# HicrestLaboratory/DLNetBench

Measured on AMD Instinct MI355X. Metric: proxy iter time (ms) + effective GB/s, Llama-3-8B DP/FSDP at 1/2/4/8 MI355X, lower is better.
Workload: dtype bf16

## Files before the change

### csrc/include/dlnb/comm.hpp

```cpp
#pragma once

#include <memory>
#include <string>
#include <vector>

#include "dlnb/bootstrap.hpp"
#include "dlnb/common.hpp"
#include "dlnb/device.hpp"

namespace dlnb {

enum class CollKind : int { AllReduce, AllGather, ReduceScatter, AllToAll, SendRecv };

class Communicator {
 public:
  virtual ~Communicator() = default;
  int rank() const { return rank_; }
  int size() const { return size_; }
  const std::vector<int>& members() const { return members_; }
  const std::string& name() const { return name_; }
  virtual std::string backend_name() const = 0;

  virtual void all_reduce(const void* send, void* recv, size_t count, DType t, Stream& s) = 0;
  virtual void all_gather(const void* send, void* recv, size_t send_count, DType t, Stream& s) = 0;
  virtual void reduce_scatter(const void* send, void* recv, size_t recv_count, DType t, Stream& s) = 0;
  virtual void all_to_all(const void* send, void* recv, size_t count, DType t, Stream& s) = 0;
  virtual void send(const void* buf, size_t count, DType t, int peer, Stream& s) = 0;
  virtual void recv(void* buf, size_t count, DType t, int peer, Stream& s) = 0;
  virtual void group_start() {}
  virtual void group_end() {}
  virtual bool wants_peer_buffers() const { return false; }
  virtual void register_buffer(void* p, size_t bytes) { (void)p, (void)bytes; }
  virtual std::string async_error() { return ""; }
  virtual void abort() {}
  virtual int library_nranks() { return -1; }

 protected:
  int rank_ = 0;
  int size_ = 1;
  std::vector<int> members_;
  std::string name_;
};

class CommFactory {
 public:
  virtual ~CommFactory() = default;
  virtual std::string backend_name() const = 0;
  virtual std::unique_ptr<Communicator> create(const std::string& name, const std::vector<int>& members,
                                               size_t capacity_bytes, bool need_p2p, int max_ctas = 0) = 0;
};

std::unique_ptr<CommFactory> make_rccl_factory(HostGroup& world, Device& dev);
std::unique_ptr<CommFactory> make_shm_factory(HostGroup& world, Device& dev);
std::unique_ptr<CommFactory> make_xgmi_factory(HostGroup& world, Device& dev);
std::unique_ptr<CommFactory> make_mixed_factory(HostGroup& world, Device& dev);

struct LoopbackHub;
std::shared_ptr<LoopbackHub> make_loopback_hub(int ranks, double timeout_s);
void loopback_abort(LoopbackHub& hub, const std::string& why);
AbortFlag loopback_cpu_abort_flag(LoopbackHub& hub);
void loopback_drained(LoopbackHub& hub, bool wait, double timeout_s);
std::unique_ptr<CommFactory> make_loopback_factory(HostGroup& world, Device& dev, std::shared_ptr<LoopbackHub> hub);

std::unique_ptr<CommFactory> wrap_comm_faults(std::unique_ptr<CommFactory> inner, Device& dev, int world_rank);

void host_reduce_sum(DType t, void* dst, const std::vector<const char*>& srcs, size_t count);
void host_copy(void* dst, const void* src, size_t bytes);

double busbw_factor(CollKind k, int n);

}
```

### csrc/include/dlnb/compute.hpp

```cpp
#pragma once

#include <memory>
#include <string>
#include <vector>

#include "dlnb/device.hpp"
#include "dlnb/json.hpp"
#include "dlnb/timers.hpp"

namespace dlnb {

enum class ComputeMode { Sleep, Spin, Gemm, GemmWork, Flops };

ComputeMode parse_compute_mode(const std::string& s, DeviceKind dev);
const char* compute_mode_name(ComputeMode m);

struct ComputeShape {
  int hidden = 4096;
  int ffn = 16384;
  DType dtype = DType::BF16;
  int comm_cus = 32;
  int ranks_on_device = 1;
};

class ComputeEngine {
 public:
  virtual ~ComputeEngine() = default;
  virtual void run(Stream& s, double us, double flops) = 0;
  virtual void run_stamped(Stream& s, double us, double flops, uint64_t* start) {
    (void)start;
    run(s, us, flops);
  }
  virtual bool stamps_task_start() const { return false; }
  virtual void run_chained(Stream& s, double us, double flops, uint64_t* start = nullptr, Event* done = nullptr) {
    run_stamped(s, us, flops, start);
    if (done) s.record(*done);
  }
  virtual uint64_t task_ticks(double us) const { (void)us; return 0; }
  virtual const uint64_t* last_task_end(Stream& s) { (void)s; return nullptr; }
  virtual bool gates_task(double us) const { (void)us; return false; }
  virtual int make_gate() { DLNB_THROW("this compute mode has no device gates"); }
  virtual void signal(Stream& s, int gate) { (void)s; (void)gate; DLNB_THROW("this compute mode has no device gates"); }
  virtual void wait_gate(Stream& s, int gate, double timeout_us) {
    (void)s; (void)gate; (void)timeout_us;
    DLNB_THROW("this compute mode has no device gates");
  }
  virtual void run_gated(Stream& s, double us, double flops, const std::vector<int>& gates, uint64_t* start,
                         bool chain, Event* done = nullptr) {
    (void)s; (void)us; (void)flops; (void)gates; (void)start; (void)chain; (void)done;
    DLNB_THROW("this compute mode has no device gates");
  }
  virtual void set_next_start_slot(uint64_t* slot) { (void)slot; }
  virtual void reset_clocks(Stream& s) { (void)s; }
  virtual void reset_slot(Stream& s) { (void)s; }
  virtual bool begin_program(Stream& s) { (void)s; return false; }
  virtual void end_program(Stream& s, bool join_ok) { (void)s; (void)join_ok; }
  virtual void after_capture() {}
  virtual long programs_on(Stream& s) { (void)s; return 0; }
  virtual bool program_split(Stream& s) { (void)s; return false; }
  virtual void set_lane_join(Stream& s, const std::vector<uint64_t*>& gates, uint32_t tag, uint64_t* host_done) {
    (void)s; (void)gates; (void)tag; (void)host_done;
  }
  virtual bool program_joined(Stream& s) { (void)s; return false; }
  virtual void set_gate_timeout(double s) { (void)s; }
  virtual double lane_task_us(Stream& s) { (void)s; return -1.0; }
  struct ChainCounters {
    double capped_tasks = 0, capped_s = 0, absorbed_tasks = 0, absorbed_s = 0;
    double wait_timeouts = 0, gate_timeouts = 0, aborted = 0, late_blocks = 0;
  };
  virtual void reset_capped(Stream& s) { (void)s; }
  virtual bool chain_counters(ChainCounters& c) { (void)c; return false; }
  virtual void set_task_timers(TimerSet* t) { (void)t; }
  virtual bool product(const void** c, size_t* count, DType* t) const {
    (void)c; (void)count; (void)t;
    return false;
  }
  virtual Json describe() const = 0;
  virtual ComputeMode mode() const = 0;
};

std::unique_ptr<ComputeEngine> make_compute_engine(Device& dev, ComputeMode mode, const ComputeShape& shape,
                                                   double time_scale);

struct TaskMark {
  const uint64_t* slot = nullptr;
  uint64_t ticks = 0;
};
inline TaskMark task_mark(ComputeEngine& ce, Stream& s, const uint64_t* start, double us) {
  if (const uint64_t* e = ce.last_task_end(s)) return {e, 0};
  return {start, ce.task_ticks(us)};
}

}
```

### csrc/include/dlnb/kernels.hpp

```cpp
#pragma once

#include <cstddef>
#include <cstdint>

#include "dlnb/common.hpp"

namespace dlnb {
namespace kernels {

void fill_random(void* p, size_t count, DType t, uint64_t seed, void* stream);

enum DlCounter : int {
  kCappedTasks = 0,
  kCappedTicks = 1,
  kWaitTimeouts = 2,
  kGateTimeouts = 3,
  kAbsorbedTicks = 4,
  kAbsorbedTasks = 5,
  kAborted = 6,
  kLateBlocks = 7,
  kNumCounters = 8
};
constexpr uint64_t kPoisonIter = ~0ull;
struct DlSync {
  uint64_t* tstart[2] = {nullptr, nullptr};
  const uint64_t* gate[2] = {nullptr, nullptr};
  uint32_t tag[2] = {0, 0};
  uint32_t chain = 0;
  uint64_t* counters = nullptr;
  const uint64_t* iter = nullptr;
  uint64_t gate_timeout = 0;
  uint64_t* done_gate = nullptr;
  uint32_t done_tag = 0;
  uint32_t pad = 0;
  const uint64_t* abort = nullptr;
};
constexpr uint32_t kTaskGateOnly = 1;
struct DlTask {
  DlSync sync;
  uint64_t ticks = 0;
  uint32_t epoch = 0;
  uint32_t work_rounds = 0;
  uint32_t tail_kt = 0;
  uint32_t flags = 0;
  uint64_t* tend = nullptr;
};
void gate_signal(uint64_t* gate, const uint64_t* iter, uint32_t tag, void* stream);
void fail_gate_signal(long index);
void gate_wait(const uint64_t* gate, const uint64_t* iter, uint32_t tag, uint64_t timeout_ticks, uint64_t* timeouts,
               void* stream, const uint64_t* abort = nullptr);
void set_word(uint64_t* word, uint64_t value, void* stream);
bool queues_independent(void* a, void* b, uint64_t timeout_ticks);

void idle_wait(uint64_t ticks, void* stream, uint64_t* start = nullptr, uint64_t* start2 = nullptr);
void busy_spin(uint64_t ticks, int blocks, void* stream, uint64_t* start = nullptr, uint64_t* start2 = nullptr);
double wallclock_hz(int device);
double wallclock_hz_nominal(int device);
double wallclock_uncertainty_ppm(int device);
void clock_cal_begin(int device);
void stamp(uint64_t* slot, void* stream);
void host_signal(uint64_t* word, uint64_t value, void* stream);
void lane_done(uint64_t* word, const uint64_t* iter, void* stream);
void host_wait(const uint64_t* word, uint64_t value, uint64_t timeout_ticks, uint64_t* timeouts, void* stream,
               uint64_t* iter_out = nullptr, uint64_t iter_value = 0, const uint64_t* abort = nullptr);
int num_cus(int device);

bool gemm_shape_ok(int M, int N, int K, DType in_t);
void gemm_tn(const void* A, const void* B, void* C, int M, int N, int K, int lda, int ldb, int ldc, DType in_t,
             void* stream, int variant = 0);
bool gemm_8phase_shape_ok(int M, int N, int K, DType in_t);
bool gemm_4wave_fp8_shape_ok(int M, int N, int K, DType in_t);
int gemm_group();
int gemm_narrow_nf(int M, int N, int cus);
bool gemm_tn_narrow(const void* A, const void* B, void* C, int M, int N, int K, int lda, int ldb, int ldc,
                    DType in_t, void* stream);
void gemm_tn_4wave_fp8(const void* A, const void* B, void* C, int M, int N, int K, int lda, int ldb, int ldc,
                       void* stream);
bool gemm_4wave_shape_ok(int M, int N, int K, DType in_t);
void gemm_tn_4wave_bf16(const void* A, const void* B, void* C, int M, int N, int K, int lda, int ldb, int ldc,
                        void* stream);
void gemm_tn_4wave_deadline(const void* A, const void* B, void* C, int M, int N, int K, DType in_t, uint64_t ticks,
                            uint64_t* slot, uint32_t epoch, int grid, void* stream, uint64_t slice_end,
                            const DlSync& sync);
void gemm_tn_4wave_fp8_deadline(const void* A, const void* B, void* C, int M, int N, int K, uint64_t ticks,
                                uint64_t* slot, uint32_t epoch, int grid, void* stream, uint64_t slice_end,
                                const DlSync& sync);
void gemm_tn_8phase(const void* A, const void* B, void* C, int M, int N, int K, int lda, int ldb, int ldc, DType in_t,
                    void* stream);
void gemm_tn_8phase_deadline(const void* A, const void* B, void* C, int M, int N, int K, DType in_t, uint64_t ticks,
                             uint64_t* slot, uint32_t epoch, int grid, void* stream, uint64_t slice_end,
                             const DlSync& sync);

void gemm_tn_deadline(const void* A, const void* B, void* C, int M, int N, int K, DType in_t, uint64_t ticks,
                      uint64_t* slot, uint32_t epoch, int grid, void* stream, uint64_t slice_end = 0,
                      const DlSync& sync = DlSync());

bool deadline_program_ok(int M, int N, int K, DType in_t);
void gemm_tn_deadline_program(const void* A, const void* B, void* C, int M, int N, int K, DType in_t,
                              const DlTask* tasks, int n, uint64_t* slot, int grid, void* stream,
                              uint32_t epoch = 0);
int program_ktiles(int M, int N, int K, DType in_t);
int program_tail_multiple(int M, int N, int K, DType in_t);

void sgd_momentum_bf16(void* param, void* mom, const void* grad, size_t n, float lr, float beta, void* stream,
                       uint64_t* end_stamp = nullptr, uint32_t* done = nullptr);

}
}
```

### csrc/include/dlnb/strategy.hpp

```cpp
#pragma once

#include <memory>
#include <string>
#include <vector>

#include "dlnb/bootstrap.hpp"
#include "dlnb/comm.hpp"
#include "dlnb/compute.hpp"
#include "dlnb/device.hpp"
#include "dlnb/json.hpp"
#include "dlnb/options.hpp"
#include "dlnb/timers.hpp"
#include "dlnb/timeline.hpp"
#include "dlnb/workload.hpp"

namespace dlnb {

struct CommRecord {
  std::string name;
  std::string backend;
  int nranks;
  int library_nranks;
};

struct Context {
  Options opt;
  std::unique_ptr<Bootstrap> boot;
  std::unique_ptr<Device> dev;
  std::unique_ptr<CommFactory> comms;
  std::vector<CommRecord> comm_log;
  std::vector<Communicator*> live_comms;
  std::unique_ptr<ComputeEngine> compute;
  ModelStats stats;
  bool have_arch = false;
  ModelArch arch;
  DType wire = DType::BF16;
  int lane_ctas = 0;
  int ranks_on_device = 1;
  std::unique_ptr<Timeline> timeline;
  int rank() const { return boot->info.rank; }
  int world() const { return boot->info.world_size; }
  HostGroup& hg() { return *boot->world; }
};

struct GridCoords {
  int inner_id, stage_id, dp_id;
};
GridCoords grid_coords(int rank, int inner, int stages);
std::vector<int> inner_group(int rank, int inner, int stages);
std::vector<int> pp_group(int rank, int inner, int stages);
std::vector<int> dp_group(int rank, int inner, int stages, int world);

struct OutputView {
  std::string name;
  const void* data;
  size_t count;
  DType dtype;
};

class Strategy {
 public:
  virtual ~Strategy() = default;
  virtual void setup(Context& ctx) = 0;
  virtual void enqueue_iteration() = 0;
  virtual void synchronize() = 0;
  virtual std::vector<Stream*> streams() = 0;
  virtual bool capturable() const = 0;
  virtual bool lanes_without_program() const { return true; }
  virtual std::string section_id() const = 0;
  virtual std::string section_title() const = 0;
  virtual const char* runtime_key() const { return "runtimes"; }
  virtual Json global_json() const = 0;
  virtual Json rank_json() const = 0;
  virtual Json comm_summary() const = 0;
  virtual double compute_floor_us(const Context& ctx) const {
    return ctx.stats.avg_forward_time_us + ctx.stats.avg_backward_time_us;
  }
  virtual std::string tail_collective_timer() const { return ""; }
  virtual std::vector<OutputView> outputs() const { return {}; }
  TimerSet* timers() { return timers_.get(); }

 protected:
  std::unique_ptr<TimerSet> timers_;
};

std::unique_ptr<Strategy> make_dp();
std::unique_ptr<Strategy> make_fsdp();
std::unique_ptr<Strategy> make_pipeline(StrategyKind kind);
std::unique_ptr<Strategy> make_cp();

int collective_lanes(const Options& o, int world);

std::string select_backend(Context& ctx, const std::string& requested, const std::string& devices);

int commtest_main(int argc, char** argv);
int info_main(int argc, char** argv);

Json run_benchmark(const Options& opt);

int main_for(StrategyKind kind, int argc, char** argv);

void sync_streams(const std::vector<Stream*>& streams, const std::vector<Communicator*>& comms, Device& dev);

void device_failure(const std::string& why);
bool process_poisoned();

class CompletionFlag {
 public:
  CompletionFlag(const uint64_t* flags, size_t n, uint64_t value);
  ~CompletionFlag();
  CompletionFlag(const CompletionFlag&) = delete;
  CompletionFlag& operator=(const CompletionFlag&) = delete;

 private:
  const uint64_t* prev_;
  size_t prev_n_;
  uint64_t prev_value_;
};

struct CommStat {
  std::string name;
  CollKind kind;
  int nranks;
  double bytes_per_op;
  std::string timer;
};
Json comm_stats_json(const std::vector<CommStat>& stats, const TimerSet& t);

void dump_outputs(Context& ctx, const Strategy& strat, const std::string& dir);

void print_topology(Context& ctx);

Json runtime_info();

Json comm_log_json(const std::vector<CommRecord>& log);

void optimizer_step(Context& ctx, Stream& s, void* param, void* mom, const void* grad, size_t n,
                    uint64_t* end_stamp = nullptr, uint32_t* done = nullptr);

}
```

### csrc/include/dlnb/timers.hpp

```cpp
#pragma once

#include <map>
#include <memory>
#include <string>
#include <vector>

#include "dlnb/device.hpp"
#include "dlnb/json.hpp"

namespace dlnb {

class TimerSet {
 public:
  explicit TimerSet(Device& dev);
  ~TimerSet();
  TimerSet(const TimerSet&) = delete;
  TimerSet& operator=(const TimerSet&) = delete;
  int begin(Stream& s);
  const uint64_t* at(int token) const { return token < 0 ? nullptr : stamps_ + token; }
  const uint64_t* end(int token, Stream& s, const std::string& name);
  void stall(Stream& s, Event& e, const std::string& name);
  uint64_t* slot();
  void gap(const uint64_t* prev_start, uint64_t prev_ticks, const uint64_t* next_start, const std::string& name,
           bool clamp = false);
  void set_task_stamps(bool on) { task_stamps_ = on; }
  bool task_stamps() const { return task_stamps_ && enabled_; }
  uint64_t* task_slot(Stream& s);
  void task_started(Stream& s, const uint64_t* start, uint64_t ticks, const uint64_t* end = nullptr);
  const uint64_t* mark(Stream& s);
  void pair(const uint64_t* a, const uint64_t* b, const std::string& name);
  void stall_before_task(Stream& s, Event& e, const std::string& name);
  void stall_after_task(Stream& s, Event& e, const std::string& name);
  void settle(Stream& s, const uint64_t* op_end);
  void stall_until(Stream& s, const uint64_t* end, const std::string& name);
  void iteration_start(Stream& s);
  void finish_stalls();
  void add(const std::string& name, double seconds);
  void ensure(const std::string& name);
  void resolve();
  void clear();
  Json negatives_json() const;
  bool has_negatives() const { return !negatives_.empty(); }
  void begin_capture();
  void end_capture();
  void set_enabled(bool on) { enabled_ = on; }
  bool enabled() const { return enabled_; }
  const std::vector<double>& get(const std::string& name) const;
  double sum(const std::string& name) const;
  Json values_json(const std::string& name) const;

 private:
  Device& dev_;
  uint64_t* stamps_ = nullptr;
  size_t cap_ = 0;
  size_t next_ = 0;
  struct Pending {
    int a, b;
    std::string name;
  };
  std::vector<Pending> pending_;
  struct Gap {
    int prev, next;
    uint64_t prev_ticks;
    std::string name;
    bool clamp;
    int floor;
  };
  std::vector<Gap> gaps_;
  bool owns(const uint64_t* p) const { return p >= stamps_ && p < stamps_ + cap_; }
  struct TaskClock {
    const uint64_t* start = nullptr;
    uint64_t ticks = 0;
    const uint64_t* floor = nullptr;
    std::vector<std::string> pending;
  };
  std::map<Stream*, TaskClock> clocks_;
  Stream* origin_ = nullptr;
  const uint64_t* origin_start_ = nullptr;
  void first_reference(Stream& s, TaskClock& c);
  void close_pending(TaskClock& c, const uint64_t* at, bool clamp = false);
  static void restart(TaskClock& c, const uint64_t* start, uint64_t ticks) {
    c.start = start;
    c.ticks = ticks;
    c.floor = nullptr;
  }
  bool task_stamps_ = false;
  std::map<std::string, std::vector<double>> vals_;
  struct Negative {
    long count = 0;
    double worst_s = 0.0;
  };
  std::map<std::string, Negative> negatives_;
  std::vector<std::pair<std::string, double>> captured_adds_;
  bool capturing_ = false, frozen_ = false;
  bool enabled_ = true;
};

}
```

### csrc/kernels/kernels.hip

```cpp
#include <hip/hip_runtime.h>

#include <cstdio>
#include "dlnb/common.hpp"
#include <thread>
#include <mutex>
#include <cmath>
#include <vector>
#include <algorithm>
#include <atomic>
#include <chrono>

#include "deadline_sync.hpp"
#include "dlnb/kernels.hpp"

#define DLNB_HIP_CHECK(expr)                                                       \
  do {                                                                             \
    hipError_t e_ = (expr);                                                        \
    if (e_ != hipSuccess) DLNB_THROW(#expr << " failed: " << hipGetErrorString(e_)); \
  } while (0)

namespace dlnb {
namespace kernels {

namespace {

typedef __attribute__((ext_vector_type(8))) __bf16 bf16x8;
typedef __attribute__((ext_vector_type(4))) __bf16 bf16x4;
typedef __attribute__((ext_vector_type(4))) float f32x4;
typedef __attribute__((ext_vector_type(8))) int i32x8;
typedef __attribute__((address_space(3))) void* lds_ptr_t;
typedef __attribute__((address_space(1))) void* gbl_ptr_t;

inline hipStream_t S(void* s) { return static_cast<hipStream_t>(s); }


__device__ __forceinline__ uint64_t splitmix64(uint64_t x) {
  x += 0x9E3779B97F4A7C15ull;
  x = (x ^ (x >> 30)) * 0xBF58476D1CE4E5B9ull;
  x = (x ^ (x >> 27)) * 0x94D049BB133111EBull;
  return x ^ (x >> 31);
}

__device__ __forceinline__ float u01(uint64_t h, int part) {
  uint32_t v = static_cast<uint32_t>((h >> (21 * part)) & 0x1fffff);
  return static_cast<float>(v) * (2.0f / 2097152.0f) - 1.0f;
}

__device__ __forceinline__ uint8_t f32_to_e4m3(float f) {
  int r = __builtin_amdgcn_cvt_pk_fp8_f32(f, f, 0, false);
  return static_cast<uint8_t>(r & 0xff);
}

__device__ __forceinline__ uint8_t f32_to_e5m2(float f) {
  int r = __builtin_amdgcn_cvt_pk_bf8_f32(f, f, 0, false);
  return static_cast<uint8_t>(r & 0xff);
}

template <typename Tstore, int KIND>
__global__ void fill_kernel(Tstore* __restrict__ p, size_t n8, size_t n, uint64_t seed) {
  size_t stride = static_cast<size_t>(gridDim.x) * blockDim.x;
  for (size_t i = blockIdx.x * static_cast<size_t>(blockDim.x) + threadIdx.x; i < n8; i += stride) {
    uint64_t h0 = splitmix64(seed ^ (i * 2 + 0));
    uint64_t h1 = splitmix64(seed ^ (i * 2 + 1));
    float f[8];
#pragma unroll
    for (int j = 0; j < 3; ++j) f[j] = u01(h0, j);
#pragma unroll
    for (int j = 0; j < 3; ++j) f[3 + j] = u01(h1, j);
    f[6] = u01(h0 ^ h1, 0);
    f[7] = u01(h0 ^ h1, 1);
    size_t base = i * 8;
    if (KIND == 0) {
      bf16x8 v;
#pragma unroll
      for (int j = 0; j < 8; ++j) v[j] = static_cast<__bf16>(f[j]);
      if (base + 8 <= n) {
        *reinterpret_cast<bf16x8*>(reinterpret_cast<__bf16*>(p) + base) = v;
      } else {
        for (int j = 0; j < 8 && base + j < n; ++j) reinterpret_cast<__bf16*>(p)[base + j] = v[j];
      }
    } else if (KIND == 1) {
      for (int j = 0; j < 8 && base + j < n; ++j) reinterpret_cast<_Float16*>(p)[base + j] = static_cast<_Float16>(f[j]);
    } else if (KIND == 2) {
      for (int j = 0; j < 8 && base + j < n; ++j) reinterpret_cast<float*>(p)[base + j] = f[j];
    } else {
      uint8_t b[8];
#pragma unroll
      for (int j = 0; j < 8; ++j) b[j] = KIND == 3 ? f32_to_e4m3(f[j]) : f32_to_e5m2(f[j]);
      uint8_t* q = reinterpret_cast<uint8_t*>(p);
      if (base + 8 <= n) {
        uint64_t packed = 0;
#pragma unroll
        for (int j = 0; j < 8; ++j) packed |= static_cast<uint64_t>(b[j]) << (8 * j);
        *reinterpret_cast<uint64_t*>(q + base) = packed;
      } else {
        for (int j = 0; j < 8 && base + j < n; ++j) q[base + j] = b[j];
      }
    }
  }
}


__global__ void idle_wait_kernel(uint64_t ticks, uint64_t* start, uint64_t* start2) {
  const uint64_t t0 = __builtin_amdgcn_s_memrealtime();
  if (start) __hip_atomic_store(start, t0, __ATOMIC_RELAXED, __HIP_MEMORY_SCOPE_SYSTEM);
  if (start2) __hip_atomic_store(start2, t0, __ATOMIC_RELAXED, __HIP_MEMORY_SCOPE_SYSTEM);
  while (__builtin_amdgcn_s_memrealtime() - t0 < ticks) __builtin_amdgcn_s_sleep(8);
}

__global__ void stamp_kernel(uint64_t* slot) {
  if (threadIdx.x == 0) {
    const uint64_t t = __builtin_amdgcn_s_memrealtime();
    __hip_atomic_store(slot, t, __ATOMIC_RELAXED, __HIP_MEMORY_SCOPE_SYSTEM);
  }
}

__global__ void gate_signal_kernel(uint64_t* gate, const uint64_t* iter, uint32_t tag) {
  if (threadIdx.x == 0) {
    const uint64_t seq = dl::gate_seq(iter, tag);
    __hip_atomic_store(gate + 1, __builtin_amdgcn_s_memrealtime(), __ATOMIC_RELAXED, __HIP_MEMORY_SCOPE_AGENT);
    __hip_atomic_store(gate, seq, __ATOMIC_RELEASE, __HIP_MEMORY_SCOPE_AGENT);
  }
}

__global__ void gate_wait_kernel(const uint64_t* gate, const uint64_t* iter, uint32_t tag, uint64_t timeout_ticks,
                                 uint64_t* timeouts, const uint64_t* abort) {
  if (threadIdx.x == 0) {
    const uint64_t it = dl::iter_of(iter);
    const uint64_t want = dl::gate_seq_of(it, tag);
    const uint64_t w0 = __builtin_amdgcn_s_memrealtime();
    if (!(iter && it == kPoisonIter)) {
      for (unsigned k = 1; __hip_atomic_load(gate, __ATOMIC_RELAXED, __HIP_MEMORY_SCOPE_AGENT) < want; ++k) {
        __builtin_amdgcn_s_sleep(2);
        if ((k & 63u) == 0 && dl::abort_up(abort)) break;
        if (__builtin_amdgcn_s_memrealtime() - w0 > timeout_ticks) {
          __hip_atomic_fetch_add(timeouts, 1ull, __ATOMIC_RELAXED, __HIP_MEMORY_SCOPE_AGENT);
          break;
        }
      }
    }
    __builtin_amdgcn_fence(__ATOMIC_ACQUIRE, "agent");
  }
}

__global__ void set_word_kernel(uint64_t* word, uint64_t value) {
  if (threadIdx.x == 0) __hip_atomic_store(word, value, __ATOMIC_RELAXED, __HIP_MEMORY_SCOPE_AGENT);
}

__global__ void probe_wait_kernel(const uint64_t* word, uint64_t value, uint64_t timeout_ticks, uint64_t* timed_out) {
  if (threadIdx.x == 0) {
    const uint64_t w0 = __builtin_amdgcn_s_memrealtime();
    while (__hip_atomic_load(word, __ATOMIC_RELAXED, __HIP_MEMORY_SCOPE_SYSTEM) != value) {
      __builtin_amdgcn_s_sleep(2);
      if (__builtin_amdgcn_s_memrealtime() - w0 > timeout_ticks) {
        __hip_atomic_store(timed_out, 1ull, __ATOMIC_RELAXED, __HIP_MEMORY_SCOPE_SYSTEM);
        break;
      }
    }
    __builtin_amdgcn_fence(__ATOMIC_ACQUIRE, "");
  }
}

__global__ void lane_done_kernel(uint64_t* word, const uint64_t* iter) {
  if (threadIdx.x == 0)
    __hip_atomic_store(word, __hip_atomic_load(iter, __ATOMIC_RELAXED, __HIP_MEMORY_SCOPE_AGENT), __ATOMIC_RELAXED,
                       __HIP_MEMORY_SCOPE_SYSTEM);
}

__global__ void host_signal_kernel(uint64_t* word, uint64_t value) {
  if (threadIdx.x == 0) __hip_atomic_store(word, value, __ATOMIC_RELEASE, __HIP_MEMORY_SCOPE_SYSTEM);
}

__global__ void host_wait_kernel(const uint64_t* word, uint64_t value, uint64_t timeout_ticks, uint64_t* timeouts,
                                 uint64_t* iter_out, uint64_t iter_value, uint64_t tight_ticks, const uint64_t* abort) {
  if (threadIdx.x == 0) {
    const uint64_t w0 = __builtin_amdgcn_s_memrealtime();
    bool aborted = false;
    for (unsigned k = 1; __hip_atomic_load(word, __ATOMIC_RELAXED, __HIP_MEMORY_SCOPE_SYSTEM) < value; ++k) {
      const uint64_t el = __builtin_amdgcn_s_memrealtime() - w0;
      if (tight_ticks != 0 && el > tight_ticks)
        __builtin_amdgcn_s_sleep(127);
      else
        __builtin_amdgcn_s_sleep(2);
      if (((k & 63u) == 0 || (tight_ticks != 0 && el > tight_ticks)) && dl::abort_up(abort)) {
        aborted = true;
        break;
      }
      if (__builtin_amdgcn_s_memrealtime() - w0 > timeout_ticks) {
        __hip_atomic_fetch_add(timeouts, 1ull, __ATOMIC_RELAXED, __HIP_MEMORY_SCOPE_SYSTEM);
        break;
      }
    }
    __builtin_amdgcn_fence(__ATOMIC_ACQUIRE, "");
    if (iter_out)
      __hip_atomic_store(iter_out, aborted ? kPoisonIter : iter_value, __ATOMIC_RELAXED, __HIP_MEMORY_SCOPE_AGENT);
  }
}

__global__ void __launch_bounds__(256) busy_spin_kernel(uint64_t ticks, float* sink, uint64_t* start,
                                                        uint64_t* start2) {
  const uint64_t t0 = __builtin_amdgcn_s_memrealtime();
  if (blockIdx.x == 0 && threadIdx.x == 0) {
    if (start) __hip_atomic_store(start, t0, __ATOMIC_RELAXED, __HIP_MEMORY_SCOPE_SYSTEM);
    if (start2) __hip_atomic_store(start2, t0, __ATOMIC_RELAXED, __HIP_MEMORY_SCOPE_SYSTEM);
  }
  float x = static_cast<float>(threadIdx.x) * 1e-3f, y = 0.999f;
  for (;;) {
#pragma unroll
    for (int i = 0; i < 64; ++i) x = __builtin_fmaf(x, y, 1e-3f);
    if (__builtin_amdgcn_s_memrealtime() - t0 >= ticks) break;
  }
  if (x == -1.0f) sink[threadIdx.x] = x;
}


constexpr int kTile = 256;
constexpr int kRowBytes = 128;
constexpr int kTileBytes = kTile * kRowBytes;
constexpr int kStageBytes = 2 * kTileBytes;

__device__ __forceinline__ int swz(int row, int chunk) { return row * kRowBytes + ((chunk ^ ((row >> 1) & 7)) << 4); }

template <int NW>
__device__ __forceinline__ void stage_tile(const char* __restrict__ g, size_t ld_bytes, char* lds_tile, int w,
                                           int lane) {
#pragma unroll
  for (int i = 0; i < 32 / NW; ++i) {
    const int slot = (i * NW + w) * 64 + lane;
    const int r = slot >> 3;
    const int c = (slot & 7) ^ ((r >> 1) & 7);
    const char* src = g + static_cast<size_t>(r) * ld_bytes + (c << 4);
    __builtin_amdgcn_global_load_lds((gbl_ptr_t)src, (lds_ptr_t)(lds_tile + (i * NW + w) * 1024), 16, 0, 0);
  }
}

__device__ __forceinline__ int xcd_remap(int b, int T) {
  const int q = T / 8, r = T % 8, x = b % 8;
  return (x < r ? x * (q + 1) : r * (q + 1) + (x - r) * q) + b / 8;
}

template <bool FP8, bool DEADLINE, int FN, int WTN, bool SWP = false>
__device__ __forceinline__ void ktile_mfma(const char* __restrict__ At, const char* __restrict__ Bt, f32x4 (&acc)[8][FN],
                                           int wm, int wn, int r16, int h) {
  if constexpr (SWP && !FP8 && FN == 4) {
    bf16x8 af[2][8], bfr[2][FN];
#pragma unroll
    for (int i = 0; i < 8; ++i)
      af[0][i] = *reinterpret_cast<const bf16x8*>(At + swz(wm * 128 + i * 16 + r16, h));
#pragma unroll
    for (int j = 0; j < FN; ++j)
      bfr[0][j] = *reinterpret_cast<const bf16x8*>(Bt + swz(wn * WTN + j * 16 + r16, h));
    __builtin_amdgcn_s_setprio(1);
    __builtin_amdgcn_sched_barrier(0);
#pragma unroll
    for (int i = 0; i < 8; ++i)
      af[1][i] = *reinterpret_cast<const bf16x8*>(At + swz(wm * 128 + i * 16 + r16, 4 + h));
#pragma unroll
    for (int j = 0; j < FN; ++j)
      bfr[1][j] = *reinterpret_cast<const bf16x8*>(Bt + swz(wn * WTN + j * 16 + r16, 4 + h));
#pragma unroll
    for (int i = 0; i < 8; ++i)
#pragma unroll
      for (int j = 0; j < FN; ++j)
        acc[i][j] = __builtin_amdgcn_mfma_f32_16x16x32_bf16(bfr[0][j], af[0][i], acc[i][j], 0, 0, 0);
#pragma unroll
    for (int k = 0; k < 12; ++k) {
      __builtin_amdgcn_sched_group_barrier(0x008, 2, 0);
      __builtin_amdgcn_sched_group_barrier(0x100, 1, 0);
    }
    __builtin_amdgcn_sched_group_barrier(0x008, 8, 0);
    __builtin_amdgcn_sched_barrier(0);
#pragma unroll
    for (int i = 0; i < 8; ++i)
#pragma unroll
// ... 92 lines not shown
  constexpr int FN = kTile / WN / 16;
  constexpr int WTN = kTile / WN;
  const int wm = w / WN, wn = w % WN;
  const int nt_m = M / kTile, nt_n = N / kTile, T = nt_m * nt_n;
  constexpr uint64_t kMask48 = dl::kMask48;
  uint64_t t0 = 0;
  if constexpr (DEADLINE) {
    if (tid == 0) t0 = dl::agree_t0(slot, epoch, ticks, sync);
  }
  for (int round = 0;; ++round) {
  const int b = xcd_remap(DEADLINE ? (blockIdx.x + round * gridDim.x) % T : blockIdx.x, T);
  constexpr int GROUP = 8;
  const int per_group = GROUP * nt_n;
  const int first_m = (b / per_group) * GROUP;
  const int gsz = min(nt_m - first_m, GROUP);
  const int tm = first_m + (b % per_group) % gsz;
  const int tn = (b % per_group) / gsz;

  constexpr int esz = FP8 ? 1 : 2;
  const size_t lda_b = static_cast<size_t>(lda) * esz, ldb_b = static_cast<size_t>(ldb) * esz;
  const char* Ab = A + static_cast<size_t>(tm) * kTile * lda_b;
  const char* Bb = B + static_cast<size_t>(tn) * kTile * ldb_b;
  const int nk = (K * esz) / kRowBytes;

  f32x4 acc[8][FN];
#pragma unroll
  for (int i = 0; i < 8; ++i)
#pragma unroll
    for (int j = 0; j < FN; ++j) acc[i][j] = f32x4{0.f, 0.f, 0.f, 0.f};

  stage_tile<NW>(Ab, lda_b, smem, w, lane);
  stage_tile<NW>(Bb, ldb_b, smem + kTileBytes, w, lane);
  asm volatile("s_waitcnt vmcnt(0)" ::: "memory");
  __syncthreads();
  int expired = 0;

  const int r16 = lane & 15, h = lane >> 4;
  for (int kt = 0; kt < nk && !expired; ++kt) {
    const char* cur = smem + (kt & 1) * kStageBytes;
    if (kt + 1 < nk) {
      char* nxt = smem + ((kt + 1) & 1) * kStageBytes;
      stage_tile<NW>(Ab + static_cast<size_t>(kt + 1) * kRowBytes, lda_b, nxt, w, lane);
      stage_tile<NW>(Bb + static_cast<size_t>(kt + 1) * kRowBytes, ldb_b, nxt + kTileBytes, w, lane);
    }
    const char* At = cur;
    const char* Bt = cur + kTileBytes;
    ktile_mfma<FP8, DEADLINE, FN, WTN, SWP>(At, Bt, acc, wm, wn, r16, h);
    asm volatile("s_waitcnt vmcnt(0)" ::: "memory");
    if constexpr (DEADLINE) {
      if (tid == 0) {
        const uint64_t el = (__builtin_amdgcn_s_memrealtime() - t0) & kMask48;
        stop_flag[kt & 1] = el >= ticks || el >= slice_end;
      }
      __syncthreads();
      expired = __builtin_amdgcn_readfirstlane(stop_flag[kt & 1]);
    } else {
      __syncthreads();
    }
  }
  if (expired) {
    if constexpr (DEADLINE) dl::task_done(sync);
    return;
  }

  store_tile<FN, WTN>(C, ldc, tm, tn, wm, wn, r16, h, acc);
  if constexpr (!DEADLINE) return;
  }
}



__global__ void sgd_momentum_kernel(__bf16* __restrict__ p, __bf16* __restrict__ m, const __bf16* __restrict__ g,
                                    size_t n, float lr, float beta, uint64_t* end_stamp, uint32_t* done) {
  size_t stride = static_cast<size_t>(gridDim.x) * blockDim.x * 8;
  for (size_t i = (blockIdx.x * static_cast<size_t>(blockDim.x) + threadIdx.x) * 8; i < n; i += stride) {
    if (i + 8 <= n) {
      bf16x8 pv = *reinterpret_cast<bf16x8*>(p + i);
      bf16x8 mv = *reinterpret_cast<bf16x8*>(m + i);
      bf16x8 gv = *reinterpret_cast<const bf16x8*>(g + i);
#pragma unroll
      for (int j = 0; j < 8; ++j) {
        float mm = beta * static_cast<float>(mv[j]) + static_cast<float>(gv[j]);
        mv[j] = static_cast<__bf16>(mm);
        pv[j] = static_cast<__bf16>(static_cast<float>(pv[j]) - lr * mm);
      }
      *reinterpret_cast<bf16x8*>(p + i) = pv;
      *reinterpret_cast<bf16x8*>(m + i) = mv;
    } else {
      for (size_t k = i; k < n; ++k) {
        float mm = beta * static_cast<float>(m[k]) + static_cast<float>(g[k]);
        m[k] = static_cast<__bf16>(mm);
        p[k] = static_cast<__bf16>(static_cast<float>(p[k]) - lr * mm);
      }
    }
  }
  if (end_stamp) {
    __syncthreads();
    if (threadIdx.x == 0) {
      const uint64_t t = __builtin_amdgcn_s_memrealtime();
      if (__hip_atomic_fetch_add(done, 1u, __ATOMIC_ACQ_REL, __HIP_MEMORY_SCOPE_AGENT) == gridDim.x - 1) {
        __hip_atomic_store(end_stamp, t, __ATOMIC_RELAXED, __HIP_MEMORY_SCOPE_SYSTEM);
        __hip_atomic_store(done, 0u, __ATOMIC_RELAXED, __HIP_MEMORY_SCOPE_AGENT);
      }
    }
  }
}

int grid_for(size_t work_items, int block) {
  size_t g = (work_items + block - 1) / block;
  if (g > 8192) g = 8192;
  if (g < 1) g = 1;
  return static_cast<int>(g);
}

}

void fill_random(void* p, size_t count, DType t, uint64_t seed, void* stream) {
  if (count == 0) return;
  size_t n8 = (count + 7) / 8;
  int grid = grid_for(n8, 256);
  seed = seed * 0xD1B54A32D192ED03ull + 0x632BE59BD9B4E019ull;
  switch (t) {
    case DType::BF16: hipLaunchKernelGGL((fill_kernel<uint16_t, 0>), grid, 256, 0, S(stream), static_cast<uint16_t*>(p), n8, count, seed); break;
    case DType::FP16: hipLaunchKernelGGL((fill_kernel<uint16_t, 1>), grid, 256, 0, S(stream), static_cast<uint16_t*>(p), n8, count, seed); break;
    case DType::FP32: hipLaunchKernelGGL((fill_kernel<float, 2>), grid, 256, 0, S(stream), static_cast<float*>(p), n8, count, seed); break;
    case DType::FP8_E4M3: hipLaunchKernelGGL((fill_kernel<uint8_t, 3>), grid, 256, 0, S(stream), static_cast<uint8_t*>(p), n8, count, seed); break;
    case DType::FP8_E5M2: hipLaunchKernelGGL((fill_kernel<uint8_t, 4>), grid, 256, 0, S(stream), static_cast<uint8_t*>(p), n8, count, seed); break;
  }
  DLNB_HIP_CHECK(hipGetLastError());
}

void idle_wait(uint64_t ticks, void* stream, uint64_t* start, uint64_t* start2) {
  hipLaunchKernelGGL(idle_wait_kernel, 1, 64, 0, S(stream), ticks, start, start2);
  DLNB_HIP_CHECK(hipGetLastError());
}

namespace {
std::atomic<long> g_gate_signals{0};
std::atomic<long> g_gate_fault{-1};
}

void fail_gate_signal(long index) { g_gate_fault.store(index); }

void gate_signal(uint64_t* gate, const uint64_t* iter, uint32_t tag, void* stream) {
  DLNB_REQUIRE(gate != nullptr && tag > 0 && reinterpret_cast<uintptr_t>(gate) % 16 == 0, "gate_signal: bad gate/tag");
  const long k = g_gate_signals.fetch_add(1);
  const long f = g_gate_fault.load();
  if (f >= 0 && k == f) {
    std::fprintf(stderr, "[dlnb] fault injection: gate signal %ld of this process is not raised\n", k);
    std::fflush(stderr);
    return;
  }
  hipLaunchKernelGGL(gate_signal_kernel, 1, 64, 0, S(stream), gate, iter, tag);
  DLNB_HIP_CHECK(hipGetLastError());
}

void gate_wait(const uint64_t* gate, const uint64_t* iter, uint32_t tag, uint64_t timeout_ticks, uint64_t* timeouts,
               void* stream, const uint64_t* abort) {
  DLNB_REQUIRE(gate != nullptr && timeouts != nullptr && tag > 0 && reinterpret_cast<uintptr_t>(gate) % 16 == 0,
               "gate_wait: bad gate/tag");
  hipLaunchKernelGGL(gate_wait_kernel, 1, 64, 0, S(stream), gate, iter, tag, timeout_ticks, timeouts, abort);
  DLNB_HIP_CHECK(hipGetLastError());
}

void set_word(uint64_t* word, uint64_t value, void* stream) {
  DLNB_REQUIRE(word != nullptr, "set_word: null word");
  hipLaunchKernelGGL(set_word_kernel, 1, 64, 0, S(stream), word, value);
  DLNB_HIP_CHECK(hipGetLastError());
}

bool queues_independent(void* a, void* b, uint64_t timeout_ticks) {
  void* p = nullptr;
  DLNB_HIP_CHECK(hipHostMalloc(&p, 2 * sizeof(uint64_t), hipHostMallocMapped | hipHostMallocCoherent));
  uint64_t* w = static_cast<uint64_t*>(p);
  w[0] = 0;
  w[1] = 0;
  hipLaunchKernelGGL(probe_wait_kernel, 1, 64, 0, S(a), w, 1ull, timeout_ticks, w + 1);
  hipLaunchKernelGGL(host_signal_kernel, 1, 64, 0, S(b), w, 1ull);
  hipError_t e = hipGetLastError();
  const hipError_t ea = hipStreamSynchronize(S(a)), eb = hipStreamSynchronize(S(b));
  const bool ok = __atomic_load_n(w + 1, __ATOMIC_ACQUIRE) == 0;
  (void)hipHostFree(p);
  DLNB_HIP_CHECK(e);
  DLNB_HIP_CHECK(ea);
  DLNB_HIP_CHECK(eb);
  return ok;
}

void lane_done(uint64_t* word, const uint64_t* iter, void* stream) {
  DLNB_REQUIRE(word != nullptr && iter != nullptr, "lane_done: null word");
  hipLaunchKernelGGL(lane_done_kernel, 1, 64, 0, S(stream), word, iter);
  DLNB_HIP_CHECK(hipGetLastError());
}

void host_signal(uint64_t* word, uint64_t value, void* stream) {
  DLNB_REQUIRE(word != nullptr, "host_signal: null word");
  hipLaunchKernelGGL(host_signal_kernel, 1, 64, 0, S(stream), word, value);
  DLNB_HIP_CHECK(hipGetLastError());
}

void host_wait(const uint64_t* word, uint64_t value, uint64_t timeout_ticks, uint64_t* timeouts, void* stream,
               uint64_t* iter_out, uint64_t iter_value, const uint64_t* abort) {
  DLNB_REQUIRE(word != nullptr && timeouts != nullptr, "host_wait: null word");
  static const long tight_us = env_int("DLNB_HOST_WAIT_TIGHT_US", 50);
  const uint64_t tight = tight_us > 0 ? static_cast<uint64_t>(tight_us) * 100ull : 0ull;
  hipLaunchKernelGGL(host_wait_kernel, 1, 64, 0, S(stream), word, value, timeout_ticks, timeouts, iter_out, iter_value,
                     tight, abort);
  DLNB_HIP_CHECK(hipGetLastError());
}

void stamp(uint64_t* slot, void* stream) {
  hipLaunchKernelGGL(stamp_kernel, 1, 64, 0, S(stream), slot);
  DLNB_HIP_CHECK(hipGetLastError());
}

void busy_spin(uint64_t ticks, int blocks, void* stream, uint64_t* start, uint64_t* start2) {
  hipLaunchKernelGGL(busy_spin_kernel, blocks, 256, 0, S(stream), ticks, static_cast<float*>(nullptr), start, start2);
  DLNB_HIP_CHECK(hipGetLastError());
}

double wallclock_hz_nominal(int device) {
  int khz = 0;
  if (hipDeviceGetAttribute(&khz, hipDeviceAttributeWallClockRate, device) != hipSuccess || khz <= 0) khz = 100000;
  return static_cast<double>(khz) * 1e3;
}

__global__ void clock_pingpong_kernel(uint64_t* slot, int n, uint64_t idle_ticks) {
  if (threadIdx.x == 0) {
    for (int k = 1; k <= n; ++k) {
      const uint64_t w0 = __builtin_amdgcn_s_memrealtime();
      bool live = true;
      while (__hip_atomic_load(slot, __ATOMIC_RELAXED, __HIP_MEMORY_SCOPE_SYSTEM) < static_cast<uint64_t>(k)) {
        if (__builtin_amdgcn_s_memrealtime() - w0 > idle_ticks) {
          live = false;
          break;
        }
      }
      if (!live) break;
      const uint64_t t = __builtin_amdgcn_s_memrealtime();
      __hip_atomic_store(slot + 1, t, __ATOMIC_RELAXED, __HIP_MEMORY_SCOPE_SYSTEM);
      __hip_atomic_store(slot + 2, static_cast<uint64_t>(k), __ATOMIC_RELEASE, __HIP_MEMORY_SCOPE_SYSTEM);
    }
  }
}

namespace {
struct ClockCal {
  std::mutex mu;
  bool begun = false, done = false;
  double hz = 0.0, host_us = 0.0, err_us = 0.0;
  double uncertainty_ppm = -1.0;
  uint64_t tick = 0;
};
ClockCal& clock_cal(int device) {
  static ClockCal c[64];
  return c[device & 63];
}
double steady_us() {
  return std::chrono::duration<double, std::micro>(std::chrono::steady_clock::now().time_since_epoch()).count();
}
bool read_clock(int device, double* host_us, uint64_t* tick, double* err_us) {
  int prev = 0;
  DLNB_HIP_CHECK(hipGetDevice(&prev));
  DLNB_HIP_CHECK(hipSetDevice(device));
  hipStream_t s{};
  DLNB_HIP_CHECK(hipStreamCreateWithFlags(&s, hipStreamNonBlocking));
  void* p = nullptr;
  DLNB_HIP_CHECK(hipHostMalloc(&p, 64, hipHostMallocMapped | hipHostMallocCoherent));
  uint64_t* slot = static_cast<uint64_t*>(p);
  slot[0] = slot[1] = slot[2] = 0;
  const double nominal = wallclock_hz_nominal(device);
  const int n = 2048;
  hipLaunchKernelGGL(clock_pingpong_kernel, 1, 64, 0, s, slot, n, static_cast<uint64_t>(1.0 * nominal));
  const hipError_t le = hipGetLastError();
  struct Rt {
    double h0, h1;
    uint64_t t;
  };
  std::vector<Rt> rs;
  rs.reserve(n);
  const double start = steady_us();
  for (int k = 1; k <= n; ++k) {
    const double h0 = steady_us();
    __atomic_store_n(slot, static_cast<uint64_t>(k), __ATOMIC_RELEASE);
    bool got = true;
    while (__atomic_load_n(slot + 2, __ATOMIC_ACQUIRE) < static_cast<uint64_t>(k)) {
      if (steady_us() - start > 2e6) {
        got = false;
        break;
      }
    }
    if (!got) break;
    const double h1 = steady_us();
    rs.push_back({h0, h1, __atomic_load_n(slot + 1, __ATOMIC_ACQUIRE)});
  }
  __atomic_store_n(slot, static_cast<uint64_t>(n), __ATOMIC_RELEASE);
  const hipError_t se = hipStreamSynchronize(s);
  (void)hipHostFree(p);
  (void)hipStreamDestroy(s);
  DLNB_HIP_CHECK(hipSetDevice(prev));
  DLNB_HIP_CHECK(le);
  DLNB_HIP_CHECK(se);
  if (rs.size() < 64) return false;
  const double b = nominal * 1e-6;
  const uint64_t tref = rs[rs.size() / 2].t;
  std::vector<size_t> idx(rs.size());
// ... 220 lines not shown
```

### csrc/src/capi.cpp

```cpp
#include <hip/hip_runtime.h>

#include <cstdlib>
#include <cstring>
#include <string>
#include <vector>

#include "dlnb/compute.hpp"
#include "dlnb/kernels.hpp"
#include "dlnb/strategy.hpp"
#include "dlnb/workload.hpp"

namespace {
thread_local std::string g_err;

char* dup(const std::string& s) {
  char* p = static_cast<char*>(std::malloc(s.size() + 1));
  std::memcpy(p, s.c_str(), s.size() + 1);
  return p;
}

template <typename F>
int guard(F f) {
  try {
    f();
    return 0;
  } catch (const std::exception& e) {
    g_err = e.what();
    return 1;
  }
}
}

extern "C" {

const char* dlnb_version() { return "dlnetbench_amd 0.1.0 (gfx950)"; }

const char* dlnb_last_error() { return g_err.c_str(); }

void dlnb_free(char* p) { std::free(p); }

int dlnb_gpu_count() { return dlnb::gpu_device_count(); }

int dlnb_run(const char* strategy, int argc, const char** argv, char** out) {
  return guard([&] {
    dlnb::StrategyKind k = dlnb::parse_strategy(strategy);
    std::vector<const char*> av;
    av.push_back(strategy);
    for (int i = 0; i < argc; ++i) av.push_back(argv[i]);
    dlnb::Options o = dlnb::parse_options(k, static_cast<int>(av.size()), av.data());
    dlnb::Json doc = dlnb::run_benchmark(o);
    if (out) *out = dup(doc.dump());
  });
}

int dlnb_parse_stats(const char* path, char** out) {
  return guard([&] {
    dlnb::ModelStats s = dlnb::parse_model_stats(path);
    if (out) *out = dup(s.to_json().dump());
  });
}

int dlnb_fill_random(void* p, size_t n, int dtype, unsigned long long seed, void* stream) {
  return guard([&] { dlnb::kernels::fill_random(p, n, static_cast<dlnb::DType>(dtype), seed, stream); });
}

int dlnb_gemm_tn(const void* A, const void* B, void* C, int M, int N, int K, int lda, int ldb, int ldc, int dtype,
                 void* stream) {
  return guard([&] {
    dlnb::kernels::gemm_tn(A, B, C, M, N, K, lda, ldb, ldc, static_cast<dlnb::DType>(dtype), stream);
  });
}

int dlnb_gemm_tn_waves(const void* A, const void* B, void* C, int M, int N, int K, int lda, int ldb, int ldc, int dtype,
                       int waves, void* stream) {
  return guard([&] {
    dlnb::kernels::gemm_tn(A, B, C, M, N, K, lda, ldb, ldc, static_cast<dlnb::DType>(dtype), stream, waves);
  });
}

int dlnb_gemm_deadline_us(const void* A, const void* B, void* C, int M, int N, int K, int dtype, double us,
                          int device, void* stamp_slot, int grid, void* stream) {
  static uint32_t epoch = 0;
  return guard([&] {
    epoch = epoch % 65535 + 1;
    double hz = dlnb::kernels::wallclock_hz(device);
    if (grid <= 0) grid = dlnb::kernels::num_cus(device);
    dlnb::kernels::gemm_tn_deadline(A, B, C, M, N, K, static_cast<dlnb::DType>(dtype),
                                    static_cast<unsigned long long>(us * 1e-6 * hz), static_cast<uint64_t*>(stamp_slot),
                                    epoch, grid, stream);
  });
}

int dlnb_gemm_deadline_ex(const void* A, const void* B, void* C, int M, int N, int K, int dtype, double us, int device,
                          void* slot, int grid, void* stream, unsigned epoch, double chain_us, void* gate0, unsigned tag0,
                          void* gate1, unsigned tag1, void* tstart, void* counters) {
  return guard([&] {
    double hz = dlnb::kernels::wallclock_hz(device);
    if (grid <= 0) grid = dlnb::kernels::num_cus(device);
    dlnb::kernels::DlSync sync;
    sync.chain = chain_us > 0 ? static_cast<uint32_t>(std::max(1.0, chain_us * 1e-6 * hz + 0.5)) : 0u;
    sync.gate[0] = static_cast<const uint64_t*>(gate0);
    sync.gate[1] = static_cast<const uint64_t*>(gate1);
    sync.tag[0] = tag0;
    sync.tag[1] = tag1;
    sync.tstart[0] = static_cast<uint64_t*>(tstart);
    sync.counters = static_cast<uint64_t*>(counters);
    dlnb::kernels::gemm_tn_deadline(A, B, C, M, N, K, static_cast<dlnb::DType>(dtype),
                                    static_cast<unsigned long long>(us * 1e-6 * hz), static_cast<uint64_t*>(slot),
                                    epoch, grid, stream, 0, sync);
  });
}

int dlnb_gate_signal(void* gate, unsigned tag, void* stream) {
  return guard([&] { dlnb::kernels::gate_signal(static_cast<uint64_t*>(gate), nullptr, tag, stream); });
}

int dlnb_gate_signal_iter(void* gate, const void* iter, unsigned tag, void* stream) {
  return guard([&] {
    dlnb::kernels::gate_signal(static_cast<uint64_t*>(gate), static_cast<const uint64_t*>(iter), tag, stream);
  });
}

struct dlnb_task_desc {
  unsigned long long ticks;
  unsigned long long chain_ticks;
  void* gate0;
  void* gate1;
  unsigned tag0, tag1;
  void* tstart0;
  void* tstart1;
  void* done_gate;
  unsigned done_tag;
  unsigned work_rounds;
  unsigned tail_kt;
  unsigned epoch;
  void* tend;
  unsigned flags;
};

int dlnb_task_size() { return static_cast<int>(sizeof(dlnb::kernels::DlTask)); }

int dlnb_gemm_program(const void* A, const void* B, void* C, int M, int N, int K, int dtype, const dlnb_task_desc* d,
                      int n, const void* iter, void* counters, const void* abort, double gate_timeout_s, int device,
                      void* slot, void* task_buf, int grid, void* stream, unsigned epoch) {
  return guard([&] {
    DLNB_REQUIRE(n > 0 && d && task_buf && slot, "dlnb_gemm_program: bad arguments");
    if (grid <= 0) grid = dlnb::kernels::num_cus(device);
    const double hz = dlnb::kernels::wallclock_hz_nominal(device);
    std::vector<dlnb::kernels::DlTask> ts(static_cast<size_t>(n));
    for (int i = 0; i < n; ++i) {
      dlnb::kernels::DlTask& t = ts[static_cast<size_t>(i)];
      t.ticks = d[i].ticks;
      t.epoch = d[i].epoch;
      t.work_rounds = d[i].work_rounds;
      t.tail_kt = d[i].tail_kt;
      t.flags = d[i].flags;
      t.tend = static_cast<uint64_t*>(d[i].tend);
      t.sync.chain = static_cast<uint32_t>(d[i].chain_ticks);
      t.sync.gate[0] = static_cast<const uint64_t*>(d[i].gate0);
      t.sync.gate[1] = static_cast<const uint64_t*>(d[i].gate1);
      t.sync.tag[0] = d[i].tag0;
      t.sync.tag[1] = d[i].tag1;
      t.sync.tstart[0] = static_cast<uint64_t*>(d[i].tstart0);
      t.sync.tstart[1] = static_cast<uint64_t*>(d[i].tstart1);
      t.sync.done_gate = static_cast<uint64_t*>(d[i].done_gate);
      t.sync.done_tag = d[i].done_tag;
      t.sync.iter = static_cast<const uint64_t*>(iter);
      t.sync.counters = static_cast<uint64_t*>(counters);
      t.sync.abort = static_cast<const uint64_t*>(abort);
      t.sync.gate_timeout = static_cast<uint64_t>(gate_timeout_s * hz);
    }
    hipStream_t st = static_cast<hipStream_t>(stream);
    if (hipStreamSynchronize(st) != hipSuccess) DLNB_THROW("dlnb_gemm_program: stream synchronize failed");
    if (hipMemcpy(task_buf, ts.data(), ts.size() * sizeof(dlnb::kernels::DlTask), hipMemcpyHostToDevice) != hipSuccess)
      DLNB_THROW("dlnb_gemm_program: task list copy failed");
    dlnb::kernels::gemm_tn_deadline_program(A, B, C, M, N, K, static_cast<dlnb::DType>(dtype),
                                            static_cast<const dlnb::kernels::DlTask*>(task_buf), n,
                                            static_cast<uint64_t*>(slot), grid, stream, epoch);
  });
}

int dlnb_program_ktiles(int M, int N, int K, int dtype) {
  return dlnb::kernels::program_ktiles(M, N, K, static_cast<dlnb::DType>(dtype));
}

void* dlnb_host_words(int n, void** dev) {
  void* p = nullptr;
  if (hipHostMalloc(&p, static_cast<size_t>(n) * 8, hipHostMallocMapped | hipHostMallocCoherent) != hipSuccess)
    return nullptr;
  std::memset(p, 0, static_cast<size_t>(n) * 8);
  if (dev && hipHostGetDevicePointer(dev, p, 0) != hipSuccess) *dev = p;
  return p;
}
void dlnb_host_words_free(void* p) { (void)hipHostFree(p); }

int dlnb_gemm_narrow_nf(int M, int N, int cus) { return dlnb::kernels::gemm_narrow_nf(M, N, cus); }

int dlnb_gemm_shape_ok(int M, int N, int K, int dtype) {
  return dlnb::kernels::gemm_shape_ok(M, N, K, static_cast<dlnb::DType>(dtype)) ? 1 : 0;
}

int dlnb_idle_wait_us(double us, int device, void* stream) {
  return guard([&] {
    double hz = dlnb::kernels::wallclock_hz(device);
    dlnb::kernels::idle_wait(static_cast<unsigned long long>(us * 1e-6 * hz), stream);
  });
}

int dlnb_busy_spin_us(double us, int device, void* stream) {
  return guard([&] {
    double hz = dlnb::kernels::wallclock_hz(device);
    dlnb::kernels::busy_spin(static_cast<unsigned long long>(us * 1e-6 * hz), dlnb::kernels::num_cus(device), stream);
  });
}

int dlnb_sgd_momentum_bf16(void* p, void* m, const void* g, size_t n, float lr, float beta, void* stream) {
  return guard([&] { dlnb::kernels::sgd_momentum_bf16(p, m, g, n, lr, beta, stream); });
}

double dlnb_wallclock_hz(int device) { return dlnb::kernels::wallclock_hz(device); }

int dlnb_stamp(void* slot, void* stream) {
  return guard([&] { dlnb::kernels::stamp(static_cast<uint64_t*>(slot), stream); });
}

float dlnb_bf16_to_float(unsigned short v) { return dlnb::bf16_to_float(v); }
unsigned short dlnb_float_to_bf16(float f) { return dlnb::float_to_bf16(f); }
float dlnb_fp8e4m3_to_float(unsigned char v) { return dlnb::fp8e4m3_to_float(v); }
unsigned char dlnb_float_to_fp8e4m3(float f) { return dlnb::float_to_fp8e4m3(f); }

}
```

### csrc/src/comm_rccl.cpp

```cpp
#include <hip/hip_runtime.h>
#include <rccl/rccl.h>

#include <dlfcn.h>

#include <cstring>
#include <sstream>

#include "dlnb/comm.hpp"
#include "dlnb/json.hpp"

#define DLNB_NCCL_CHECK(expr)                                                            \
  do {                                                                                   \
    ncclResult_t r_ = (expr);                                                            \
    if (r_ != ncclSuccess) DLNB_THROW(#expr << " failed: " << ncclGetErrorString(r_));   \
  } while (0)

namespace dlnb {

namespace {

ncclDataType_t to_nccl(DType t) {
  switch (t) {
    case DType::BF16: return ncclBfloat16;
    case DType::FP16: return ncclFloat16;
    case DType::FP32: return ncclFloat32;
    case DType::FP8_E4M3: return static_cast<ncclDataType_t>(10);
    case DType::FP8_E5M2: return static_cast<ncclDataType_t>(11);
  }
  return ncclBfloat16;
}

hipStream_t hs(Stream& s) { return static_cast<hipStream_t>(s.native()); }

class RcclComm : public Communicator {
 public:
  RcclComm(const std::string& name, const std::vector<int>& members, int my_world_rank, HostGroup& world,
           int max_ctas) {
    name_ = name;
    members_ = members;
    size_ = static_cast<int>(members.size());
    rank_ = -1;
    for (int i = 0; i < size_; ++i)
      if (members[i] == my_world_rank) rank_ = i;
    DLNB_REQUIRE(rank_ >= 0, "rank " << my_world_rank << " is not a member of group " << name);
    std::ostringstream key;
    key << "rccl/" << name << "/";
    for (int m : members) key << m << ",";
    key << "/uid";
    ncclUniqueId id;
    if (rank_ == 0) {
      DLNB_NCCL_CHECK(ncclGetUniqueId(&id));
      world.store().set(key.str(), std::string(reinterpret_cast<const char*>(&id), sizeof(id)));
    } else {
      std::string v = world.store().get(key.str());
      DLNB_REQUIRE(v.size() == sizeof(id), "bad unique id size for " << name);
      std::memcpy(&id, v.data(), sizeof(id));
    }
    ncclConfig_t cfg = NCCL_CONFIG_INITIALIZER;
    if (max_ctas > 0) cfg.maxCTAs = max_ctas;
    cfg.commName = name_.c_str();
    DLNB_NCCL_CHECK(ncclCommInitRankConfig(&comm_, size_, id, rank_, &cfg));
  }
  ~RcclComm() override {
    if (comm_) (void)ncclCommDestroy(comm_);
  }
  std::string backend_name() const override { return "RCCL"; }

  void all_reduce(const void* send, void* recv, size_t count, DType t, Stream& s) override {
    DLNB_NCCL_CHECK(ncclAllReduce(send, recv, count, to_nccl(t), ncclSum, comm_, hs(s)));
  }
  void all_gather(const void* send, void* recv, size_t send_count, DType t, Stream& s) override {
    DLNB_NCCL_CHECK(ncclAllGather(send, recv, send_count, to_nccl(t), comm_, hs(s)));
  }
  void reduce_scatter(const void* send, void* recv, size_t recv_count, DType t, Stream& s) override {
    DLNB_NCCL_CHECK(ncclReduceScatter(send, recv, recv_count, to_nccl(t), ncclSum, comm_, hs(s)));
  }
  void all_to_all(const void* send, void* recv, size_t count, DType t, Stream& s) override {
    DLNB_NCCL_CHECK(ncclAllToAll(send, recv, count, to_nccl(t), comm_, hs(s)));
  }
  void send(const void* buf, size_t count, DType t, int peer, Stream& s) override {
    DLNB_NCCL_CHECK(ncclSend(buf, count, to_nccl(t), peer, comm_, hs(s)));
  }
  void recv(void* buf, size_t count, DType t, int peer, Stream& s) override {
    DLNB_NCCL_CHECK(ncclRecv(buf, count, to_nccl(t), peer, comm_, hs(s)));
  }
  void group_start() override { DLNB_NCCL_CHECK(ncclGroupStart()); }
  void group_end() override { DLNB_NCCL_CHECK(ncclGroupEnd()); }
  std::string async_error() override {
    ncclResult_t r = ncclSuccess;
    if (ncclCommGetAsyncError(comm_, &r) != ncclSuccess) return "ncclCommGetAsyncError failed";
    if (r != ncclSuccess && r != ncclInProgress) return std::string("RCCL async error in ") + name_ + ": " + ncclGetErrorString(r);
    return "";
  }
  void abort() override {
    if (comm_) {
      (void)ncclCommAbort(comm_);
      comm_ = nullptr;
    }
  }
  int library_nranks() override {
    int n = -1;
    if (comm_ && ncclCommCount(comm_, &n) != ncclSuccess) n = -1;
    return n;
  }

 private:
  ncclComm_t comm_ = nullptr;
};

class RcclFactory : public CommFactory {
 public:
  RcclFactory(HostGroup& world, Device& dev) : world_(world), dev_(dev) {
    DLNB_REQUIRE(dev.kind() == DeviceKind::GPU, "the RCCL backend needs a GPU device");
  }
  std::string backend_name() const override { return "RCCL"; }
  std::unique_ptr<Communicator> create(const std::string& name, const std::vector<int>& members, size_t,
                                       bool, int max_ctas) override {
    (void)hipSetDevice(dev_.index());
    return std::unique_ptr<Communicator>(new RcclComm(name, members, world_.rank(), world_, max_ctas));
  }

 private:
  HostGroup& world_;
  Device& dev_;
};

}

std::unique_ptr<CommFactory> make_rccl_factory(HostGroup& world, Device& dev) {
  return std::unique_ptr<CommFactory>(new RcclFactory(world, dev));
}

namespace {
std::string lib_of(const void* sym) {
  Dl_info info;
  if (dladdr(sym, &info) && info.dli_fname) return info.dli_fname;
  return "?";
}
}

Json runtime_info() {
  Json j = Json::object();
  int v = 0;
  if (ncclGetVersion(&v) == ncclSuccess) {
    j["rccl_version_code"] = v;
    std::ostringstream s;
    s << v / 10000 << "." << (v / 100) % 100 << "." << v % 100;
    j["rccl_version"] = s.str();
  }
  j["librccl"] = lib_of(reinterpret_cast<const void*>(&ncclGetVersion));
  int hv = 0;
  if (hipRuntimeGetVersion(&hv) == hipSuccess) j["hip_runtime_version"] = hv;
  j["libamdhip64"] = lib_of(reinterpret_cast<const void*>(&hipRuntimeGetVersion));
  return j;
}

double busbw_factor(CollKind k, int n) {
  if (n <= 1) return 0.0;
  switch (k) {
    case CollKind::AllReduce: return 2.0 * (n - 1) / n;
    case CollKind::AllGather:
    case CollKind::ReduceScatter:
    case CollKind::AllToAll: return static_cast<double>(n - 1) / n;
    case CollKind::SendRecv: return 1.0;
  }
  return 1.0;
}

}
```

### csrc/src/compute.cpp

```cpp
#include "dlnb/compute.hpp"

#include <algorithm>
#include <cmath>
#include <exception>
#include <map>
#include <set>

#include "dlnb/kernels.hpp"
#include "dlnb/timers.hpp"

namespace dlnb {

ComputeMode parse_compute_mode(const std::string& s, DeviceKind dev) {
  if (s == "auto") return dev == DeviceKind::GPU ? ComputeMode::Gemm : ComputeMode::Sleep;
  if (s == "sleep") return ComputeMode::Sleep;
  if (s == "spin") return ComputeMode::Spin;
  if (s == "gemm") return ComputeMode::Gemm;
  if (s == "gemm-work" || s == "gemm_work") return ComputeMode::GemmWork;
  if (s == "flops") return ComputeMode::Flops;
  DLNB_THROW("unknown compute mode '" << s << "' (auto, sleep, spin, gemm, flops)");
}

const char* compute_mode_name(ComputeMode m) {
  switch (m) {
// ... 104 lines not shown

  void reset_clocks(Stream& s) override {
    if (slots_.data()) dev_.memset_async(slots_.data(), 0, kSlots * 64, s);
  }
  void reset_slot(Stream& s) override {
    if (!slots_.data()) return;
    auto it = slot_of_.find(&s);
    if (it != slot_of_.end()) dev_.memset_async(slots_.as<uint64_t>() + it->second * 8, 0, 64, s);
  }
  void reset_capped(Stream& s) override {
    if (!counters_.data()) return;
    uint64_t* c = counters_.as<uint64_t>();
    dev_.memset_async(c + kernels::kCappedTasks, 0, 2 * sizeof(uint64_t), s);
    dev_.memset_async(c + kernels::kAbsorbedTicks, 0, 2 * sizeof(uint64_t), s);
  }
  bool begin_program(Stream& s) override {
    if ((mode_ != ComputeMode::Gemm && !fixed_) || slice_us_ > 0 || env_int("DLNB_COMPUTE_PROGRAMS", 1) == 0 ||
        !kernels::deadline_program_ok(kMmax, N_, K_, dtype_))
      return false;
    Program& p = programs_[&s];
    DLNB_REQUIRE(!p.open, "begin_program: a program is already open on this stream");
    p.open = true;
    p.index = 0;
    p.tasks.clear();
    p.pending.clear();
    p.done_free = false;
    p.split = false;
    if (dev_.gate_events()) {
      p.fold.e = this;
      p.fold.s = &s;
      dev_.set_stream_fold(s, &p.fold);
    }
    return true;
  }
  void end_program(Stream& s, bool join_ok) override {
    auto it = programs_.find(&s);
    if (it == programs_.end() || !it->second.open) return;
    Program& p = it->second;
    dev_.set_stream_fold(s, nullptr);
    emit_pending(s, p, nullptr, 0);
    auto j = joins_.find(&s);
    if (j != joins_.end() && !p.tasks.empty() && join_ok) {
      const Join& jn = j->second;
      size_t g = 0;
      do {
        kernels::DlTask t;
        t.sync.iter = dev_.iter_word();
        t.sync.counters = counters_.as<uint64_t>();
        t.sync.gate_timeout = gate_timeout_ticks_;
        t.sync.abort = dev_.abort_word();
        for (int i = 0; i < 2 && g < jn.gates.size(); ++i, ++g) {
          t.sync.gate[i] = jn.gates[g];
          t.sync.tag[i] = jn.tag;
        }
        if (g >= jn.gates.size()) t.sync.tstart[0] = jn.host_done;
        t.ticks = 0;
        p.tasks.push_back(t);
      } while (g < jn.gates.size());
      joins_.erase(j);
      joined_.insert(&s);
    }
    flush_program(s);
    p.open = false;
  }
  void set_lane_join(Stream& s, const std::vector<uint64_t*>& gates, uint32_t tag, uint64_t* host_done) override {
    if (mode_ != ComputeMode::Gemm && !fixed_) return;
    joins_[&s] = Join{gates, tag, host_done};
    joined_.erase(&s);
    lane_stats_.clear();
  }
  bool program_joined(Stream& s) override { return joined_.count(&s) != 0; }
  bool program_split(Stream& s) override {
    auto it = programs_.find(&s);
    return it != programs_.end() && it->second.split;
  }
  long programs_on(Stream& s) override {
    auto it = program_count_.find(&s);
    return it == program_count_.end() ? 0 : it->second;
  }
  void set_gate_timeout(double s) override {
    gate_timeout_ticks_ = static_cast<uint64_t>(s * kernels::wallclock_hz_nominal(dev_.index()));
  }
  double lane_task_us(Stream& s) override {
    auto it = lane_stats_.find(&s);
    if (it == lane_stats_.end() || it->second.n == 0 || !it->second.single) return -1.0;
    return it->second.us / static_cast<double>(it->second.n);
  }
  void after_capture() override {
    joins_.clear();
    if (uploads_.empty()) return;
    auto st = dev_.create_stream(false);
    for (const auto& u : uploads_)
      dev_.copy_async(u.dst, u.tasks.data(), u.tasks.size() * sizeof(kernels::DlTask), *st);
    st->synchronize();
    uploads_.clear();
  }

  bool chain_counters(ChainCounters& out) override {
    if (!counters_.data()) return false;
    uint64_t v[kernels::kNumCounters] = {};
    auto st = dev_.create_stream(false);
    dev_.copy_async(v, counters_.data(), sizeof(v), *st);
    st->synchronize();
    out.capped_tasks = static_cast<double>(v[kernels::kCappedTasks]);
    out.capped_s = static_cast<double>(v[kernels::kCappedTicks]) / hz();
    out.absorbed_tasks = static_cast<double>(v[kernels::kAbsorbedTasks]);
    out.absorbed_s = static_cast<double>(v[kernels::kAbsorbedTicks]) / hz();
    out.wait_timeouts = static_cast<double>(v[kernels::kWaitTimeouts]);
    out.gate_timeouts = static_cast<double>(v[kernels::kGateTimeouts]);
    out.aborted = static_cast<double>(v[kernels::kAborted]);
    out.late_blocks = static_cast<double>(v[kernels::kLateBlocks]);
    return true;
  }

  bool stamps_task_start() const override { return true; }
  uint64_t task_ticks(double us) const override { return fixed_ ? 0 : ticks(us * scale_); }
  const uint64_t* last_task_end(Stream& s) override {
    auto it = last_end_.find(&s);
    return it == last_end_.end() ? nullptr : it->second;
  }
  void run(Stream& s, double us, double flops) override { run_stamped(s, us, flops, nullptr); }

  void run_chained(Stream& s, double us, double flops, uint64_t* start, Event* done) override {
    if (fixed_) {
      fixed_task(s, us, flops, start, {}, done);
      return;
    }
    if (mode_ == ComputeMode::Gemm && us * scale_ >= 20.0 && chain_live_[slot_for(s)]) {
      note_task(s, us * scale_);
      if (stall_timers_ && !start) start = stall_timers_->task_slot(s);
      StartNote note{stall_timers_, s, start, ticks(us * scale_), nullptr};
      kernels::DlSync sync;
      sync.tstart[0] = start;
      sync.tstart[1] = extra_start_;
      extra_start_ = nullptr;
      deadline_task(s, us * scale_, sync, true, done);
      ++chained_;
      return;
    }
    run_stamped(s, us, flops, start);
    if (done) s.record(*done);
  }

  bool gates_task(double us) const override { return fixed_ || (mode_ == ComputeMode::Gemm && us * scale_ >= 20.0); }

  int make_gate() override {
    DLNB_REQUIRE(mode_ == ComputeMode::Gemm || fixed_, "gates need the gemm (deadline) or fixed-work GPU compute");
    gates_.push_back(dev_.alloc_gate());
    gate_tag_.push_back(0);
    return static_cast<int>(gates_.size()) - 1;
  }

  void signal(Stream& s, int gate) override {
    uint32_t& tag = gate_tag_.at(gate);
    tag = tag == 0xffffffffu ? 1u : tag + 1;
    kernels::gate_signal(gates_.at(gate), dev_.iter_word(), tag, s.native());
  }
  void wait_gate(Stream& s, int gate, double timeout_us) override {
    const uint32_t tag = gate_tag_.at(gate);
    DLNB_REQUIRE(tag != 0, "wait_gate: gate " << gate << " was never signalled");
    kernels::gate_wait(gates_.at(gate), dev_.iter_word(), tag, ticks(timeout_us),
                       counters_.as<uint64_t>() + kernels::kWaitTimeouts, s.native(), dev_.abort_word());
  }

  void run_gated(Stream& s, double us, double flops, const std::vector<int>& gates, uint64_t* start,
                 bool chain, Event* done) override {
    DLNB_REQUIRE(gates_task(us), "run_gated: the task cannot wait on gates (see gates_task)");
    DLNB_REQUIRE(gates.size() <= 2, "run_gated: at most 2 gates per task");
    kernels::DlSync sync;
    for (size_t i = 0; i < gates.size(); ++i) {
      sync.gate[i] = gates_.at(gates[i]);
      sync.tag[i] = gate_tag_.at(gates[i]);
      DLNB_REQUIRE(sync.tag[i] != 0, "run_gated: gate " << gates[i] << " was never signalled");
    }
    if (fixed_) {
      fixed_task(s, us, flops, start, sync, done);
      ++gated_;
      return;
    }
    note_task(s, us * scale_);
    if (stall_timers_ && !start) start = stall_timers_->task_slot(s);
    StartNote note{stall_timers_, s, start, ticks(us * scale_), nullptr};
    sync.tstart[0] = start;
    sync.tstart[1] = extra_start_;
    extra_start_ = nullptr;
    const bool chained = chain && chain_live_[slot_for(s)];
    deadline_task(s, us * scale_, sync, chained, done);
    if (chained) ++chained_;
    ++gated_;
  }

  void set_next_start_slot(uint64_t* slot) override { extra_start_ = slot; }

  void flush_program(Stream& s) {
    auto it = programs_.find(&s);
    if (it == programs_.end()) return;
    if (it->second.open) emit_pending(s, it->second, nullptr, 0);
    if (it->second.tasks.empty()) return;
    it->second.done_free = false;
    std::vector<kernels::DlTask>& ts = it->second.tasks;
    for (int i = 0; i < 2; ++i)
      if (ts[0].sync.gate[i])
        kernels::gate_wait(ts[0].sync.gate[i], dev_.iter_word(), ts[0].sync.tag[i], gate_timeout_ticks_,
                           counters_.as<uint64_t>() + kernels::kWaitTimeouts, s.native(), dev_.abort_word());
    const kernels::DlTask* dst = place_tasks(s, ts);
    kernels::gemm_tn_deadline_program(A_.data(), B_.data(), C_.data(), kMmax, N_, K_, dtype_, dst,
                                      static_cast<int>(ts.size()), slot_for(s), grid_, s.native(), 0u);
    ++programs_launched_;
    ++program_count_[&s];
    program_tasks_ += static_cast<long>(ts.size());
    ts.clear();
  }

  void run_stamped(Stream& s, double us, double flops, uint64_t* start) override {
    if (fixed_) {
      fixed_task(s, us, flops, start, {}, nullptr);
      return;
    }
    note_task(s, us * scale_);
    if (stall_timers_ && !start) start = stall_timers_->task_slot(s);
    StartNote note{stall_timers_, s, start, ticks(std::max(0.0, us * scale_)), nullptr};
    double d = us * scale_;
    if (mode_ == ComputeMode::Gemm && d < 20.0) {
      auto pit = programs_.find(&s);
      if (pit != programs_.end() && pit->second.open) pit->second.split = true;
      flush_program(s);
    }
    if (mode_ == ComputeMode::Gemm) chain_live_[slot_for(s)] = false;
    if (mode_ == ComputeMode::Sleep || mode_ == ComputeMode::Spin) {
      uint64_t* extra = extra_start_;
      extra_start_ = nullptr;
      if (d <= 0) {
        if (start) dev_.stamp(s, start);
        if (extra) dev_.stamp(s, extra);
      } else if (mode_ == ComputeMode::Sleep) {
        kernels::idle_wait(ticks(d), s.native(), start, extra);
      } else {
        kernels::busy_spin(ticks(d), cus_, s.native(), start, extra);
      }
      return;
    }
    if (d <= 0) {
      if (start) dev_.stamp(s, start);
      if (extra_start_) dev_.stamp(s, extra_start_);
      extra_start_ = nullptr;
      return;
    }
    if (d < 20.0) {
      kernels::busy_spin(ticks(d), cus_, s.native(), start, extra_start_);
      extra_start_ = nullptr;
      return;
    }
    kernels::DlSync sync;
    sync.tstart[0] = start;
    sync.tstart[1] = extra_start_;
    extra_start_ = nullptr;
    deadline_task(s, d, sync, false);
  }

  void set_task_timers(TimerSet* t) override {
    task_timers_ = fixed_ ? t : nullptr;
    if (t && env_int("DLNB_TASK_STAMP_TIMERS", 1) != 0) {
      stall_timers_ = t;
      t->set_task_stamps(true);
    } else if (fixed_) {
      stall_timers_ = t;
    }
  }

  Json describe() const override {
    Json j = Json::object();
    j["mode"] = compute_mode_name(mode_);
    j["time_scale"] = scale_;
    j["wallclock_hz"] = hz();
    j["wallclock_hz_nominal"] = kernels::wallclock_hz_nominal(dev_.index());
    j["wallclock_uncertainty_ppm"] = kernels::wallclock_uncertainty_ppm(dev_.index());
    j["num_cus"] = cus_;
    if (mode_ == ComputeMode::Gemm || fixed_) {
      j["deadline_grid"] = grid_;
      j["comm_reserved_cus"] = cus_ - grid_;
      j["deadline_slice_us"] = slice_us_;
      j["chained_tasks"] = chained_;
      j["chain_absorb_us"] = absorb_ticks_ / hz() * 1e6;
      j["gated_tasks"] = gated_;
      j["programs"] = programs_launched_;
      j["program_tasks"] = program_tasks_;
    }
    if (A_.data()) {
      j["gemm_dtype"] = dtype_name(dtype_);
      j["gemm_N"] = N_;
      j["gemm_K"] = K_;
    }
    if (fixed_) {
      Json f = Json::object();
      f["round_us"] = cal_.round_us;
      f["ktile_us"] = cal_.ktile_us;
      f["grid"] = grid_;
      f["ktiles_per_tile"] = nk_;
      f["tflops"] = round_flops() / (cal_.round_us * 1e-6) / 1e12;
      f["tasks"] = fixed_tasks_;
      f["calibration"] = cal_given_ ? "DLNB_FIXED_WORK_CAL" : "measured";
      j["fixed_work"] = f;
    }
    return j;
  }
  ComputeMode mode() const override { return mode_; }
  bool product(const void** c, size_t* count, DType* t) const override {
    if (!C_.data()) return false;
    *c = C_.data();
// ... 411 lines not shown
```

### csrc/src/device_gpu.cpp

```cpp
#include <hip/hip_runtime.h>
#include <hsa/hsa_ext_amd.h>

#include <chrono>
#include <cstdio>
#include <cstring>
#include <map>
#include <mutex>
#include <set>
#include <string>
#include <thread>
#include <vector>

#include "dlnb/device.hpp"
#include "dlnb/kernels.hpp"

#define DLNB_HIP_CHECK(expr)                                                       \
  do {                                                                             \
    hipError_t e_ = (expr);                                                        \
    if (e_ != hipSuccess) DLNB_THROW(#expr << " failed: " << hipGetErrorString(e_)); \
  } while (0)

namespace dlnb {

namespace {
// ... 124 lines not shown
class GpuDevice : public Device {
 public:
  explicit GpuDevice(int idx) : idx_(idx) {
    DLNB_HIP_CHECK(hipSetDevice(idx_));
    hipDeviceProp_t prop;
    DLNB_HIP_CHECK(hipGetDeviceProperties(&prop, idx_));
    name_ = prop.name;
    arch_ = prop.gcnArchName;
    total_ = prop.totalGlobalMem;
    kernels::clock_cal_begin(idx_);
    ensure_pool();
    void* a = nullptr;
    DLNB_HIP_CHECK(hipHostMalloc(&a, 64, hipHostMallocMapped | hipHostMallocCoherent));
    abort_host_ = static_cast<uint64_t*>(a);
    std::memset(abort_host_, 0, 64);
    void* ad = nullptr;
    DLNB_HIP_CHECK(hipHostGetDevicePointer(&ad, a, 0));
    abort_dev_ = static_cast<uint64_t*>(ad);
  }
  ~GpuDevice() override {
    if (pool_) (void)hipFree(pool_);
    if (abort_host_ && !abort_raised()) (void)hipHostFree(abort_host_);
  }
  DeviceKind kind() const override { return DeviceKind::GPU; }
  std::string name() const override { return name_ + " (" + arch_ + ")"; }
  int index() const override { return idx_; }
  std::unique_ptr<Stream> create_stream(bool high_priority) override {
    static const bool high_ok = env_int("DLNB_HIGH_PRIORITY_STREAMS", 1) != 0;
    return std::unique_ptr<Stream>(new GpuStream(idx_, high_priority && high_ok, streams_));
  }
  std::unique_ptr<Event> create_event(bool timing) override {
    return std::unique_ptr<Event>(new GpuEvent(timing, this));
  }
  double elapsed_ms(Event& a, Event& b) override {
    float ms = 0;
    DLNB_HIP_CHECK(hipEventSynchronize(static_cast<GpuEvent&>(b).ev));
    DLNB_HIP_CHECK(hipEventElapsedTime(&ms, static_cast<GpuEvent&>(a).ev, static_cast<GpuEvent&>(b).ev));
    return ms;
  }
  void* raw_alloc(size_t bytes) override {
    void* p = nullptr;
    hipError_t e = hipMalloc(&p, bytes);
    if (e != hipSuccess)
      DLNB_THROW("hipMalloc(" << bytes << " B) failed on device " << idx_ << ": " << hipGetErrorString(e));
    DLNB_HIP_CHECK(hipMemset(p, 0, bytes));
    DLNB_HIP_CHECK(hipStreamSynchronize(nullptr));
    return p;
  }
  void* raw_alloc_peer(size_t bytes) override {
    void* p = nullptr;
    hipError_t e = hipExtMallocWithFlags(&p, bytes, hipDeviceMallocUncached);
    if (e != hipSuccess)
      DLNB_THROW("hipExtMallocWithFlags(" << bytes << " B, uncached) failed on device " << idx_ << ": "
                                          << hipGetErrorString(e));
    DLNB_HIP_CHECK(hipMemset(p, 0, bytes));
    DLNB_HIP_CHECK(hipStreamSynchronize(nullptr));
    return p;
  }
  void raw_free(void* p, size_t) override { (void)hipFree(p); }
  void fill_random(void* p, size_t count, DType t, uint64_t seed, Stream& s) override {
    kernels::fill_random(p, count, t, seed, s.native());
  }
  void memset_async(void* p, int v, size_t bytes, Stream& s) override {
    DLNB_HIP_CHECK(hipMemsetAsync(p, v, bytes, static_cast<hipStream_t>(s.native())));
  }
  void copy_async(void* dst, const void* src, size_t bytes, Stream& s) override {
    DLNB_HIP_CHECK(hipMemcpyAsync(dst, src, bytes, hipMemcpyDefault, static_cast<hipStream_t>(s.native())));
  }
  void host_task(Stream& s, std::function<void()> fn) override {
    auto* heap = new std::function<void()>(std::move(fn));
    DLNB_HIP_CHECK(hipLaunchHostFunc(static_cast<hipStream_t>(s.native()), host_trampoline, heap));
  }
  void synchronize() override { DLNB_HIP_CHECK(hipDeviceSynchronize()); }
  const uint64_t* abort_word() override { return abort_dev_; }
  void raise_abort() override { __atomic_store_n(abort_host_, 1ull, __ATOMIC_SEQ_CST); }
  bool abort_raised() const override { return __atomic_load_n(abort_host_, __ATOMIC_ACQUIRE) != 0; }
  bool abort_and_drain() override {
    raise_abort();
    const double limit = static_cast<double>(env_int("DLNB_ABORT_DRAIN_S", 20));
    const double t0 = now_s();
    for (;;) {
      bool idle = true;
      {
        std::lock_guard<std::mutex> g(streams_->mu);
        for (hipStream_t s : streams_->live) {
          const hipError_t e = hipStreamQuery(s);
          if (e == hipErrorNotReady) {
            idle = false;
            break;
          }
        }
      }
      if (idle) return true;
      if (now_s() - t0 > limit) return false;
      std::this_thread::sleep_for(std::chrono::milliseconds(1));
    }
  }
  void idle(Stream& s, double us) override {
    kernels::idle_wait(static_cast<uint64_t>(us * 1e-6 * stamp_hz() + 0.5), s.native());
  }
  uint64_t* alloc_stamps(size_t n) override {
    void* p = nullptr;
    DLNB_HIP_CHECK(hipHostMalloc(&p, n * sizeof(uint64_t), hipHostMallocMapped | hipHostMallocCoherent));
    std::memset(p, 0, n * sizeof(uint64_t));
    return static_cast<uint64_t*>(p);
  }
  void free_stamps(uint64_t* p, size_t) override { (void)hipHostFree(p); }
  void stamp(Stream& s, uint64_t* slot) override { kernels::stamp(slot, s.native()); }
  void host_signal(Stream& s, uint64_t* word, uint64_t value) override { kernels::host_signal(word, value, s.native()); }
  void host_wait(Stream& s, const uint64_t* word, uint64_t value, double timeout_s, uint64_t* timeouts,
                 uint64_t iter_value) override {
    kernels::host_wait(word, value, static_cast<uint64_t>(timeout_s * stamp_hz()), timeouts, s.native(),
                       iter_value ? iter_word() : nullptr, iter_value, abort_dev_);
  }

  uint64_t* alloc_gate() override {
    ensure_pool();
    DLNB_REQUIRE(next_gate_ < kPoolGates, "device gate pool exhausted (" << kPoolGates << " gates)");
    return pool_ + 8 + 2 * next_gate_++;
  }
  uint64_t* iter_word() override {
    ensure_pool();
    return pool_;
  }
  void set_iteration(Stream& s, uint64_t it) override { kernels::set_word(iter_word(), it, s.native()); }
  void lane_done(Stream& s, uint64_t* host_word) override { kernels::lane_done(host_word, iter_word(), s.native()); }
  void pad(Stream& s) override { kernels::set_word(pool_ + 2, 0, s.native()); }
  void signal_gate(Stream& s, uint64_t* gate, uint32_t tag) override {
    kernels::gate_signal(gate, iter_word(), tag, s.native());
  }
  void set_gate_events(bool on) override {
    if (on) ensure_pool();
    gate_events_ = on;
  }
  bool gate_events() const override { return gate_events_; }
  bool capturing(Stream& s) override {
    hipStreamCaptureStatus st = hipStreamCaptureStatusNone;
    DLNB_HIP_CHECK(hipStreamIsCapturing(static_cast<hipStream_t>(s.native()), &st));
    return st != hipStreamCaptureStatusNone;
  }
  uint64_t gate_event_timeouts() override {
    if (!pool_) return 0;
    uint64_t v = 0;
    DLNB_HIP_CHECK(hipMemcpy(&v, pool_ + 1, sizeof(v), hipMemcpyDeviceToHost));
    return v;
  }
  uint64_t gate_timeout_ticks() {
    static const double s = static_cast<double>(env_int("DLNB_GATE_TIMEOUT_S", 60));
    return static_cast<uint64_t>((gate_timeout_s_ > 0 ? gate_timeout_s_ : s) * stamp_hz());
  }
  void set_gate_timeout(double s) override { gate_timeout_s_ = s; }
  double gate_timeout_s_ = 0.0;
  void gate_mark(GpuEvent& e, hipStream_t s) {
    if (!e.gate) e.gate = alloc_gate();
    e.tag = e.tag == 0xffffffffu ? 1u : e.tag + 1;
    e.on = s;
    e.gen = gen_;
  }
  void gate_record(GpuEvent& e, hipStream_t s) {
    gate_mark(e, s);
    kernels::gate_signal(e.gate, iter_word(), e.tag, s);
  }
  bool arm_gate_record(Event& ev, Stream& s, uint64_t** gate, uint32_t* tag) override {
    auto& e = static_cast<GpuEvent&>(ev);
    if (!gate_events_ || !e.dev) return false;
    gate_mark(e, static_cast<hipStream_t>(s.native()));
    *gate = e.gate;
    *tag = e.tag;
    return true;
  }
  bool gate_needed(const GpuEvent& e, hipStream_t s) const {
    if (e.tag == 0) return false;
    if (e.on == s) return false;
    return e.gen == gen_;
  }
  void gate_wait(GpuEvent& e, GpuStream& st) {
    if (!gate_needed(e, st.s)) return;
    if (st.fold) {
      st.fold->fold_wait(e.gate, e.tag);
      return;
    }
    kernels::gate_wait(e.gate, iter_word(), e.tag, gate_timeout_ticks(), pool_ + 1, st.s, abort_dev_);
  }
  void set_stream_fold(Stream& s, StreamFold* f) override { static_cast<GpuStream&>(s).fold = f; }
  bool queues_independent(const std::vector<Stream*>& ss, double timeout_s, std::string* detail) override {
    const uint64_t t = static_cast<uint64_t>(timeout_s * stamp_hz());
    bool ok = true;
    for (size_t a = 0; a < ss.size(); ++a)
      for (size_t b = 0; b < ss.size(); ++b) {
        if (a == b) continue;
        if (!kernels::queues_independent(ss[a]->native(), ss[b]->native(), t)) {
          ok = false;
          if (detail) *detail += (detail->empty() ? "" : ", ") + std::to_string(a) + " waits behind " + std::to_string(b);
        }
      }
    return ok;
  }
  double stamp_hz() const override { return kernels::wallclock_hz(idx_); }
  size_t total_memory() const override { return total_; }
  size_t free_memory() const override {
    size_t f = 0, t = 0;
    if (hipMemGetInfo(&f, &t) != hipSuccess) return 0;
    return f;
  }
  std::unique_ptr<GraphExec> capture(Stream& origin, const std::vector<Stream*>& others,
                                     const std::function<void()>& enqueue,
                                     const std::function<void()>& head) override {
    auto fork = create_event(false);
    std::vector<std::unique_ptr<Event>> joins;
    for (size_t i = 0; i < others.size(); ++i) joins.push_back(create_event(false));
    hipStream_t o = static_cast<hipStream_t>(origin.native());
    DLNB_HIP_CHECK(hipStreamBeginCapture(o, hipStreamCaptureModeThreadLocal));
    try {
      if (head) head();
      origin.record(*fork);
      for (Stream* s : others) s->wait(*fork);
      enqueue();
      for (size_t i = 0; i < others.size(); ++i) {
        others[i]->record(*joins[i]);
        origin.wait(*joins[i]);
      }
    } catch (...) {
      hipGraph_t g = nullptr;
      (void)hipStreamEndCapture(o, &g);
      if (g) (void)hipGraphDestroy(g);
      throw;
    }
    hipGraph_t g = nullptr;
    DLNB_HIP_CHECK(hipStreamEndCapture(o, &g));
    return instantiate(g);
  }

  std::vector<std::unique_ptr<GraphExec>> capture_lanes(const std::vector<Stream*>& lanes,
                                                        const std::function<void()>& enqueue,
                                                        const std::function<void(size_t)>& tail) override {
    ++gen_;
    size_t begun = 0;
    auto end_all = [&] {
      for (size_t i = 0; i < begun; ++i) {
        hipGraph_t g = nullptr;
        (void)hipStreamEndCapture(static_cast<hipStream_t>(lanes[i]->native()), &g);
        if (g) (void)hipGraphDestroy(g);
      }
    };
    try {
      for (; begun < lanes.size(); ++begun)
        DLNB_HIP_CHECK(hipStreamBeginCapture(static_cast<hipStream_t>(lanes[begun]->native()),
                                             hipStreamCaptureModeThreadLocal));
      enqueue();
      if (tail)
        for (size_t i = 0; i < lanes.size(); ++i) tail(i);
    } catch (...) {
      end_all();
      throw;
    }
    std::vector<hipGraph_t> gs(lanes.size(), nullptr);
    hipError_t first = hipSuccess;
    for (size_t i = 0; i < lanes.size(); ++i) {
      hipError_t e = hipStreamEndCapture(static_cast<hipStream_t>(lanes[i]->native()), &gs[i]);
      if (e != hipSuccess && first == hipSuccess) first = e;
    }
    if (first != hipSuccess) {
      for (hipGraph_t g : gs)
        if (g) (void)hipGraphDestroy(g);
      DLNB_THROW("lane capture failed: " << hipGetErrorString(first)
                                         << " (a cross-stream dependency that is not a gate event?)");
    }
    std::vector<std::unique_ptr<GraphExec>> out;
    for (hipGraph_t g : gs) out.push_back(instantiate(g));
    return out;
  }

 private:
  static constexpr size_t kPoolGates = 65536;
  void ensure_pool() {
    if (pool_) return;
    const size_t bytes = 64 + kPoolGates * 16;
    DLNB_HIP_CHECK(hipMalloc(reinterpret_cast<void**>(&pool_), bytes));
    DLNB_HIP_CHECK(hipMemset(pool_, 0, bytes));
    DLNB_HIP_CHECK(hipStreamSynchronize(nullptr));
  }
  uint64_t* pool_ = nullptr;
  uint64_t* abort_host_ = nullptr;
  uint64_t* abort_dev_ = nullptr;
  std::shared_ptr<GpuStreamSet> streams_ = std::make_shared<GpuStreamSet>();
  size_t next_gate_ = 0;
  uint64_t gen_ = 0;
  bool gate_events_ = false;
  int idx_;
  std::string name_, arch_;
  size_t total_ = 0;
};

}

void GpuStream::record(Event& e) {
  auto& g = static_cast<GpuEvent&>(e);
  if (g.dev && g.dev->gate_events()) {
    if (fold)
      fold->fold_record(e);
    else
      g.dev->gate_record(g, s);
    return;
  }
  DLNB_HIP_CHECK(hipEventRecord(g.ev, s));
}
// ... 63 lines not shown
```

### csrc/src/runner.cpp

```cpp
#include <algorithm>
#include <exception>
#include <atomic>
#include <chrono>
#include <condition_variable>
#include <cstdlib>
#include <cmath>
#include <cstdio>
#include <fstream>
#include <iostream>
#include <map>
#include <mutex>
#include <sstream>
#include <thread>

#include <sys/prctl.h>

extern char** environ;

#include "dlnb/aux.hpp"
#include "dlnb/kernels.hpp"
#include "dlnb/strategy.hpp"
#include "dlnb/xgmi.hpp"

namespace dlnb {

namespace {
thread_local const uint64_t* t_done_flag = nullptr;
thread_local size_t t_done_n = 0;
thread_local uint64_t t_done_value = 0;

struct FailGuard {
  Device* dev = nullptr;
  std::vector<Communicator*>* comms = nullptr;
  bool cli_exit = false;
  int rank = 0;
  bool fired = false;
};
thread_local FailGuard* t_fail = nullptr;
std::atomic<bool> g_poisoned{false};
}

void device_failure(const std::string& why) {
  FailGuard* f = t_fail;
  if (!f || f->fired) return;
  f->fired = true;
  if (f->dev) f->dev->raise_abort();
  if (f->cli_exit && f->dev) {
    std::fprintf(stderr,
                 "[dlnb] rank %d error: %s\n[dlnb] rank %d: device waits aborted; exiting without teardown (the "
                 "driver reclaims the GPU queues)\n",
                 f->rank, why.c_str(), f->rank);
    std::fflush(stdout);
    std::fflush(stderr);
    std::_Exit(3);
  }
  if (f->comms)
    for (Communicator* c : *f->comms)
      if (c) c->abort();
}

bool process_poisoned() { return g_poisoned.load(); }

CompletionFlag::CompletionFlag(const uint64_t* flags, size_t n, uint64_t value)
    : prev_(t_done_flag), prev_n_(t_done_n), prev_value_(t_done_value) {
  t_done_flag = flags;
  t_done_n = n;
  t_done_value = value;
}
CompletionFlag::~CompletionFlag() {
  t_done_flag = prev_;
  t_done_n = prev_n_;
  t_done_value = prev_value_;
}

void sync_streams(const std::vector<Stream*>& streams, const std::vector<Communicator*>& comms, Device& dev) {
  (void)dev;
  thread_local const bool slack_set = [] {
    prctl(PR_SET_TIMERSLACK, 1000UL, 0, 0, 0);
    return true;
  }();
  (void)slack_set;
  const double timeout = static_cast<double>(env_int("DLNB_TIMEOUT", 900));
  const double t0 = now_s();
  int polls = 0;
  const uint64_t* flag = t_done_flag;
  const size_t nflags = t_done_n;
  const uint64_t want = t_done_value;
  auto done = [&](Stream* s) {
    if (!flag) return s->query();
    for (size_t i = 0; i < nflags; ++i)
      if (__atomic_load_n(flag + i, __ATOMIC_ACQUIRE) < want) return false;
    return true;
  };
  for (Stream* s : streams) {
    while (!done(s)) {
      if (++polls % 64 == 0) {
        for (Communicator* c : comms) {
          if (!c) continue;
          std::string err = c->async_error();
          if (!err.empty()) {
            device_failure("communication failure: " + err);
            for (Communicator* a : comms)
              if (a) a->abort();
            DLNB_THROW("communication failure: " << err);
          }
        }
        if (now_s() - t0 > timeout) {
          std::ostringstream m;
          m << "iteration did not complete within DLNB_TIMEOUT=" << timeout << " s (hung collective or dead peer)";
          if (flag) {
            m << "; lane done words (want " << want << "):";
            for (size_t i = 0; i < nflags; ++i) m << " " << __atomic_load_n(flag + i, __ATOMIC_ACQUIRE);
          }
          device_failure(m.str());
          for (Communicator* a : comms)
            if (a) a->abort();
          DLNB_THROW(m.str());
        }
      }
      std::this_thread::sleep_for(std::chrono::microseconds(5));
    }
  }
}

Json comm_stats_json(const std::vector<CommStat>& stats, const TimerSet& t) {
  Json out = Json::object();
  for (const auto& s : stats) {
    const auto& v = t.get(s.timer);
    Json e = Json::object();
    e["kind"] = s.name;
    e["nranks"] = s.nranks;
    e["bytes_per_op"] = s.bytes_per_op;
    e["ops"] = static_cast<long long>(v.size());
    double tot = 0;
    for (double x : v) tot += x;
    e["total_s"] = tot;
    e["transport"] = s.nranks > 1 ? "link" : "local-copy";
    if (!v.empty() && tot > 0) {
      double algbw = s.bytes_per_op * v.size() / tot / 1e9;
      e["algbw_GBps"] = algbw;
      e["busbw_GBps"] = algbw * busbw_factor(s.kind, s.nranks);
    }
    out[s.name] = e;
  }
  return out;
}

void optimizer_step(Context& ctx, Stream& s, void* param, void* mom, const void* grad, size_t n, uint64_t* end_stamp,
                    uint32_t* done) {
  if (ctx.dev->kind() == DeviceKind::GPU) {
    kernels::sgd_momentum_bf16(param, mom, grad, n, 1e-4f, 0.9f, s.native(), end_stamp, done);
    return;
  }
  if (end_stamp) {
    ctx.dev->host_task(s, [param, mom, grad, n] {
      auto* p = static_cast<uint16_t*>(param);
      auto* m = static_cast<uint16_t*>(mom);
      auto* g = static_cast<const uint16_t*>(grad);
      for (size_t i = 0; i < n; ++i) {
        float mv = 0.9f * bf16_to_float(m[i]) + bf16_to_float(g[i]);
        m[i] = float_to_bf16(mv);
        p[i] = float_to_bf16(bf16_to_float(p[i]) - 1e-4f * mv);
      }
    });
    ctx.dev->stamp(s, end_stamp);
    return;
  }
  ctx.dev->host_task(s, [param, mom, grad, n] {
    auto* p = static_cast<uint16_t*>(param);
    auto* m = static_cast<uint16_t*>(mom);
    auto* g = static_cast<const uint16_t*>(grad);
    for (size_t i = 0; i < n; ++i) {
      float mv = 0.9f * bf16_to_float(m[i]) + bf16_to_float(g[i]);
      m[i] = float_to_bf16(mv);
      p[i] = float_to_bf16(bf16_to_float(p[i]) - 1e-4f * mv);
    }
  });
}


void print_topology(Context& ctx) {
  std::string addr = env_or("SLURM_TOPOLOGY_ADDR", "");
  if (addr.empty()) addr = "root." + ctx.boot->info.hostname;
  std::ostringstream me;
  me << addr << "|" << ctx.boot->info.hostname << "|" << ctx.dev->name() << "|" << ctx.dev->index();
  auto all = ctx.hg().allgather(me.str());
  if (ctx.rank() != 0) return;
  std::map<std::string, std::vector<int>> leaves;
  std::map<std::string, std::string> dev_of;
  for (size_t r = 0; r < all.size(); ++r) {
    auto f = split(all[r], '|');
    leaves[f[0]].push_back(static_cast<int>(r));
    dev_of[f[0]] = f.size() > 2 ? f[2] : "?";
  }
  std::ostringstream os;
  os << "=== topology: " << all.size() << " ranks on " << leaves.size() << " node(s) ===\n";
  std::vector<std::string> prev;
  for (const auto& kv : leaves) {
    auto parts = split(kv.first, '.');
    size_t common = 0;
    while (common < prev.size() && common < parts.size() - 1 && prev[common] == parts[common]) ++common;
    for (size_t d = common; d < parts.size(); ++d) {
      os << std::string(2 * d, ' ') << (d ? "└─ " : "") << parts[d];
      if (d + 1 == parts.size()) {
        os << "  ranks [";
        for (size_t i = 0; i < kv.second.size(); ++i) os << (i ? "," : "") << kv.second[i];
        os << "]  " << dev_of[kv.first];
      }
      os << "\n";
    }
    prev = parts;
  }
  if (ctx.dev->kind() == DeviceKind::GPU) os << describe_gpu_links();
  std::cout << os.str() << std::flush;
}

namespace {

std::vector<int> parse_device_list(const std::string& s) {
  std::vector<int> v;
  if (s.empty()) return v;
  for (auto& p : split(s, ',')) {
    std::string t = trim(p);
    if (!t.empty()) v.push_back(std::stoi(t));
  }
  return v;
}

double percentile(std::vector<double> v, double q) {
  if (v.empty()) return 0;
  std::sort(v.begin(), v.end());
  double pos = q * (v.size() - 1);
  size_t lo = static_cast<size_t>(std::floor(pos)), hi = static_cast<size_t>(std::ceil(pos));
  return v[lo] + (v[hi] - v[lo]) * (pos - lo);
}

std::unique_ptr<Strategy> make_strategy(StrategyKind k) {
  switch (k) {
    case StrategyKind::DP: return make_dp();
    case StrategyKind::FSDP: return make_fsdp();
    case StrategyKind::HybridCP: return make_cp();
    default: return make_pipeline(k);
  }
}

bool file_exists(const std::string& p) {
  std::ifstream f(p);
  return static_cast<bool>(f);
}

}

namespace {

class RecordingFactory : public CommFactory {
 public:
  RecordingFactory(std::unique_ptr<CommFactory> inner, std::vector<CommRecord>* log, std::vector<Communicator*>* live)
      : inner_(std::move(inner)), log_(log), live_(live) {}
  std::string backend_name() const override { return inner_->backend_name(); }
  std::unique_ptr<Communicator> create(const std::string& name, const std::vector<int>& members,
                                       size_t capacity_bytes, bool need_p2p, int max_ctas) override {
    auto c = inner_->create(name, members, capacity_bytes, need_p2p, max_ctas);
    log_->push_back({name, c->backend_name(), c->size(), c->library_nranks()});
    return c;
  }
  void add_live(Communicator* c) { live_->push_back(c); }

 private:
  std::unique_ptr<CommFactory> inner_;
  std::vector<CommRecord>* log_;
  std::vector<Communicator*>* live_;
};

class LiveFactory : public CommFactory {
 public:
// ... 954 lines not shown
```

### csrc/src/strategy_dp.cpp

```cpp
#include <cmath>

#include "dlnb/strategy.hpp"

namespace dlnb {

std::vector<uint64_t> dp_bucket_sizes(uint64_t P, int nb, double ratio) {
  std::vector<uint64_t> s;
  if (ratio >= 1.0) {
    const uint64_t base = P / nb, rem = P % nb;
    for (int i = 0; i < nb; ++i) s.push_back(base + (static_cast<uint64_t>(i) < rem ? 1 : 0));
    return s;
  }
  std::vector<double> w(static_cast<size_t>(nb));
  double x = 1.0, tot = 0.0;
  for (int i = 0; i < nb; ++i) {
    w[static_cast<size_t>(i)] = x;
    x *= ratio;
  }
  for (double v : w) tot += v;
  uint64_t sum = 0;
  for (double v : w) {
    s.push_back(static_cast<uint64_t>(std::floor(static_cast<double>(P) * v / tot)));
    sum += s.back();
  }
  s[0] += P - sum;
  for (uint64_t v : s) DLNB_REQUIRE(v > 0, "--dp-bucket-ratio " << ratio << " leaves an empty bucket of " << nb);
  return s;
}

namespace {

class DataParallel : public Strategy {
 public:
  void setup(Context& ctx) override {
    ctx_ = &ctx;
    const auto& o = ctx.opt;
    const auto& st = ctx.stats;
    nb_ = o.num_buckets;
    P_ = st.model_size;
    DLNB_REQUIRE(P_ >= static_cast<uint64_t>(nb_), "num_buckets (" << nb_ << ") exceeds the parameter count");
    ratio_ = o.dp_bucket_ratio;
    sizes_ = dp_bucket_sizes(P_, nb_, ratio_);
    fwd_us_ = st.avg_forward_time_us;
    bwd_us_per_bucket_ = st.avg_backward_time_us / nb_;
    for (uint64_t sz : sizes_) {
      const double share = ratio_ >= 1.0 ? 1.0 / nb_ : static_cast<double>(sz) / static_cast<double>(P_);
      bwd_us_.push_back(ratio_ >= 1.0 ? bwd_us_per_bucket_ : st.avg_backward_time_us * share);
      bwd_flops_.push_back(st.backward_flops * share);
    }
    fwd_flops_ = st.forward_flops;
    bwd_flops_per_bucket_ = st.backward_flops / nb_;

    Device& dev = *ctx.dev;
    es_ = dtype_size(ctx.wire);
    zero_ = o.zero;
    W_ = ctx.world();
    for (uint64_t sz : sizes_) shard_.push_back((sz + W_ - 1) / W_);
    std::vector<int> all;
    for (int r = 0; r < ctx.world(); ++r) all.push_back(r);
    comm_ = ctx.comms->create("dp/world", all, (zero_ ? shard_[0] * W_ : sizes_[0]) * es_, false, ctx.lane_ctas);
    compute_ = dev.create_stream(false);
    comm_stream_ = dev.create_stream(true);
    ComputeEngine& ce0 = *ctx.compute;
    comm_gates_ = !zero_ && o.schedule != "reference" && env_int("DLNB_DP_COMM_GATES", 0) != 0 &&
                  ce0.gates_task(fwd_us_);
    if (comm_gates_)
      for (int i = 0; i < nb_; ++i) g_ready_.push_back(ce0.make_gate());
    size_t need = static_cast<size_t>(P_) * es_ * 2;
    in_place_ = o.in_place || (dev.kind() == DeviceKind::GPU && need > dev.free_memory() * 0.85);
    if (zero_ == 2) in_place_ = false;
    in_place_ = ctx.hg().allreduce_max(in_place_ ? 1.0 : 0.0) > 0.5;
    const bool peer = comm_->wants_peer_buffers();
    auto buf = [&](size_t bytes, bool reg) {
      Buffer b = peer && reg ? dev.alloc_peer(bytes) : dev.alloc(bytes);
      if (peer && reg) comm_->register_buffer(b.data(), bytes);
      return b;
    };
    for (int i = 0; i < nb_; ++i) {
      const uint64_t n = zero_ ? shard_[i] * W_ : sizes_[i];
      grads_.push_back(buf(n * es_, true));
      if (!in_place_) sums_.push_back(buf((zero_ == 2 ? shard_[i] : n) * es_, zero_ != 2));
      ready_.push_back(dev.create_event());
      dev.fill_random(grads_.back().data(), n, ctx.wire, 1000 + i, *compute_);
      if (zero_) {
        pshard_.push_back(dev.alloc(shard_[i] * es_));
        mshard_.push_back(dev.alloc(shard_[i] * es_));
        pfull_.push_back(buf(shard_[i] * W_ * es_, true));
        dev.fill_random(pshard_.back().data(), shard_[i], ctx.wire, 2000 + i, *compute_);
        opt_done_.push_back(dev.create_event());
      }
    }
    if (zero_) opt_done_word_ = dev.alloc(64);
    done_ = dev.create_event();
    ag_done_ = dev.create_event();
    if (o.optimizer && !zero_) {
      DLNB_REQUIRE(ctx.wire == DType::BF16, "--optimizer needs --wire-dtype bf16");
      params_ = dev.alloc(P_ * es_);
      mom_ = dev.alloc(P_ * es_);
    }
    compute_->synchronize();
    timers_.reset(new TimerSet(dev));
    timers_->ensure("barrier_time");
    timers_->ensure("allreduce_time");
    double op_bytes = 0, shard_bytes = 0;
    for (int i = 0; i < nb_; ++i) {
      op_bytes += static_cast<double>((zero_ ? shard_[i] * W_ : sizes_[i]) * es_) / nb_;
      shard_bytes += static_cast<double>(shard_[i] * W_ * es_) / nb_;
    }
    if (ratio_ >= 1.0) {
      op_bytes = static_cast<double>((zero_ ? shard_[0] * W_ : sizes_[0]) * es_);
      shard_bytes = static_cast<double>(shard_[0] * W_ * es_);
    }
    if (zero_ == 2)
      stats_ = {{"reduce_scatter", CollKind::ReduceScatter, W_, shard_bytes, "reduce_scatter_time"}};
    else
      stats_ = {{"allreduce", CollKind::AllReduce, W_, op_bytes, "allreduce_time"}};
    if (zero_) {
      for (const char* k : {"reduce_scatter_time", "param_allgather_time", "param_allgather_exposed"}) timers_->ensure(k);
      stats_.push_back({"param_allgather", CollKind::AllGather, W_, shard_bytes, "param_allgather_time"});
    }
  }

  void enqueue_zero() {
    Context& ctx = *ctx_;
    ComputeEngine& ce = *ctx.compute;
    const int me = comm_->rank();
    const bool prog = ctx.dev->gate_events() && ce.begin_program(*compute_);
    ce.run(*compute_, fwd_us_, fwd_flops_);
    for (int i = 0; i < nb_; ++i) {
      ce.run_chained(*compute_, bwd_us_[i], bwd_flops_[i]);
      compute_->record(*ready_[i]);
      comm_stream_->wait(*ready_[i]);
      const uint64_t n = shard_[i] * W_;
      if (zero_ == 2) {
        int t = timers_->begin(*comm_stream_);
        comm_->reduce_scatter(grads_[i].data(), sums_[i].data(), shard_[i], ctx.wire, *comm_stream_);
        timers_->end(t, *comm_stream_, "reduce_scatter_time");
      } else {
        int t = timers_->begin(*comm_stream_);
        void* out = in_place_ ? grads_[i].data() : sums_[i].data();
        comm_->all_reduce(grads_[i].data(), out, n, ctx.wire, *comm_stream_);
        timers_->end(t, *comm_stream_, "allreduce_time");
      }
    }
    if (prog) ce.end_program(*compute_, false);
    comm_stream_->record(*done_);
    timers_->stall_after_task(*compute_, *done_, "barrier_time");
    const uint64_t* ag_end = nullptr;
    uint64_t* opt_end = nullptr;
    for (int i = 0; i < nb_; ++i) {
      const void* g = zero_ == 2 ? sums_[i].data()
                                 : (in_place_ ? grads_[i].at(me * shard_[i] * es_) : sums_[i].at(me * shard_[i] * es_));
      uint64_t* end = i == nb_ - 1 && timers_->enabled() ? timers_->slot() : nullptr;
      if (ctx.wire == DType::BF16) {
        optimizer_step(ctx, *compute_, pshard_[i].data(), mshard_[i].data(), g, shard_[i], end,
                       end ? opt_done_word_.as<uint32_t>() : nullptr);
        opt_end = end;
      }
      compute_->record(*opt_done_[i]);
      comm_stream_->wait(*opt_done_[i]);
      int t = timers_->begin(*comm_stream_);
      comm_->all_gather(pshard_[i].data(), pfull_[i].data(), shard_[i], ctx.wire, *comm_stream_);
      ag_end = timers_->end(t, *comm_stream_, "param_allgather_time");
    }
    const uint64_t* opt_mark = opt_end ? opt_end : timers_->mark(*compute_);
    comm_stream_->record(*ag_done_);
    compute_->wait(*ag_done_);
    if (opt_mark && ag_end) timers_->gap(opt_mark, 0, ag_end, "param_allgather_exposed", true);
  }

  void enqueue_iteration() override {
    if (zero_) {
      enqueue_zero();
      return;
    }
    Context& ctx = *ctx_;
    ComputeEngine& ce = *ctx.compute;
    const bool stamped = ce.stamps_task_start();
    TaskMark last;
    const uint64_t* tail_end = nullptr;
    uint64_t* fwd_start = stamped ? timers_->slot() : nullptr;
    const bool prog = ctx.dev->gate_events() && !comm_gates_ && ce.begin_program(*compute_);
    ce.run_stamped(*compute_, fwd_us_, fwd_flops_, fwd_start);
    for (int i = 0; i < nb_; ++i) {
      uint64_t* st = stamped && i == nb_ - 1 ? timers_->slot() : nullptr;
      ce.run_chained(*compute_, bwd_us_[i], bwd_flops_[i], st, comm_gates_ ? nullptr : ready_[i].get());
      if (st) last = task_mark(ce, *compute_, st, bwd_us_[i]);
      if (comm_gates_) {
        ce.signal(*compute_, g_ready_[i]);
        double ahead = fwd_us_;
        for (int j = 0; j <= i; ++j) ahead += bwd_us_[j];
        ce.wait_gate(*comm_stream_, g_ready_[i], ahead * ctx.opt.time_scale * 4 + 1e6);
      } else {
        comm_stream_->wait(*ready_[i]);
      }
      int t = timers_->begin(*comm_stream_);
      void* out = in_place_ ? grads_[i].data() : sums_[i].data();
      comm_->all_reduce(grads_[i].data(), out, sizes_[i], ctx.wire, *comm_stream_);
      const uint64_t* e = timers_->end(t, *comm_stream_, "allreduce_time");
      if (e) tail_end = e;
    }
    const bool tail_gap = last.slot && tail_end && !ctx.opt.optimizer;
    if (prog) ce.end_program(*compute_, tail_gap);
    if (tail_gap) {
      timers_->gap(last.slot, last.ticks, tail_end, "barrier_time");
      timers_->gap(fwd_start, 0, tail_end, "device_span_time");
    } else {
      comm_stream_->record(*done_);
      timers_->stall_after_task(*compute_, *done_, "barrier_time");
    }
    if (ctx.opt.optimizer) {
      size_t off = 0;
      for (int i = 0; i < nb_; ++i) {
        const void* g = in_place_ ? grads_[i].data() : sums_[i].data();
        optimizer_step(ctx, *compute_, params_.at(off * es_), mom_.at(off * es_), g, sizes_[i]);
        off += sizes_[i];
      }
    }
  }

  std::vector<Stream*> streams() override { return {compute_.get(), comm_stream_.get()}; }
  bool capturable() const override { return true; }

  void synchronize() override {
    sync_streams({compute_.get(), comm_stream_.get()}, {comm_.get()}, *ctx_->dev);
    timers_->resolve();
  }

  std::string tail_collective_timer() const override {
    return zero_ ? "param_allgather_time" : "allreduce_time";
  }
  std::string section_id() const override { return "dp"; }
  std::string section_title() const override { return "Data Parallelism"; }

  Json global_json() const override {
    const Context& ctx = *ctx_;
    double avg = 0, sd = 0;
    for (uint64_t s : sizes_) avg += static_cast<double>(s);
    avg /= nb_;
    for (uint64_t s : sizes_) sd += (s - avg) * (s - avg);
    sd = std::sqrt(sd / nb_);
    Json g = Json::object();
    g["comm_gates"] = comm_gates_;
    g["model_name"] = ctx.opt.model;
    g["num_buckets"] = nb_;
    g["local_batch_size"] = ctx.stats.batch_size;
    g["world_size"] = ctx.world();
    g["fwd_rt_whole_model"] = fwd_us_;
    g["bwd_rt_per_bucket"] = bwd_us_per_bucket_;
    g["total_model_size_params"] = P_;
    g["msg_size_avg_bytes"] = avg * es_;
    g["msg_size_std_bytes"] = sd * es_;
    g["device"] = ctx.dev->kind() == DeviceKind::CPU ? "CPU" : "GPU";
    g["backend"] = comm_->backend_name();
    g["in_place"] = in_place_;
    g["bucket_ratio"] = ratio_;
    if (ratio_ < 1.0) {
      g["bucket_policy"] = "geometric";
      g["bucket_sizes"] = Json(sizes_);
      g["bwd_us_per_bucket"] = Json(bwd_us_);
      g["bwd_flops_per_bucket"] = Json(bwd_flops_);
    } else {
      g["bucket_policy"] = "even";
    }
    g["zero_stage"] = zero_;
    if (zero_) {
      g["shard_size_params"] = shard_[0];
      g["param_allgather_msg_size_bytes"] = static_cast<double>(shard_[0] * W_ * es_);
    }
    return g;
  }

  Json rank_json() const override {
    Json r = Json::object();
    r["runtimes"] = timers_->values_json("runtimes");
    r["barrier_time"] = timers_->values_json("barrier_time");
    r["allreduce_time"] = timers_->values_json("allreduce_time");
    if (!timers_->get("device_span_time").empty()) r["device_span_time"] = timers_->values_json("device_span_time");
    if (zero_) {
      r["reduce_scatter_time"] = timers_->values_json("reduce_scatter_time");
      r["param_allgather_time"] = timers_->values_json("param_allgather_time");
      r["param_allgather_exposed"] = timers_->values_json("param_allgather_exposed");
    }
    return r;
  }

  Json comm_summary() const override { return comm_stats_json(stats_, *timers_); }

 private:
  Context* ctx_ = nullptr;
  int nb_ = 1;
  uint64_t P_ = 0;
  size_t es_ = 2;
  std::vector<uint64_t> sizes_;
  std::vector<double> bwd_us_;
  bool comm_gates_ = false;
  std::vector<int> g_ready_;
  std::vector<double> bwd_flops_;
  double ratio_ = 1.0;
  double fwd_us_ = 0, bwd_us_per_bucket_ = 0, fwd_flops_ = 0, bwd_flops_per_bucket_ = 0;
  bool in_place_ = false;
  int zero_ = 0, W_ = 1;
  std::vector<uint64_t> shard_;
  std::vector<Buffer> pshard_, mshard_, pfull_;
  std::vector<std::unique_ptr<Event>> opt_done_;
  Buffer opt_done_word_;
  std::unique_ptr<Event> ag_done_;
  std::unique_ptr<Communicator> comm_;
  std::unique_ptr<Stream> compute_, comm_stream_;
  std::vector<Buffer> grads_, sums_;
  std::vector<std::unique_ptr<Event>> ready_;
  std::unique_ptr<Event> done_;
  Buffer params_, mom_;
  std::vector<CommStat> stats_;
};

}

std::unique_ptr<Strategy> make_dp() { return std::unique_ptr<Strategy>(new DataParallel()); }

}
```

### csrc/src/strategy_fsdp.cpp

```cpp
#include <cstdio>

#include "dlnb/strategy.hpp"

namespace dlnb {

namespace {

class Fsdp : public Strategy {
 public:
  void setup(Context& ctx) override {
    ctx_ = &ctx;
    const auto& o = ctx.opt;
    const auto& st = ctx.stats;
    U_ = o.num_units;
    F_ = o.sharding_factor;
    const int W = ctx.world();
    DLNB_REQUIRE(W % F_ == 0, "world size " << W << " must be divisible by sharding_factor " << F_);
    R_ = W / F_;
    P_ = st.model_size;
    DLNB_REQUIRE(P_ >= static_cast<uint64_t>(U_), "num_units exceeds the parameter count");
    uint64_t base = P_ / U_, rem = P_ % U_;
    for (int u = 0; u < U_; ++u) {
      uint64_t pu = base + (static_cast<uint64_t>(u) < rem ? 1 : 0);
      shard_.push_back(pu / F_ + (pu % F_ ? 1 : 0));
    }
    max_shard_ = shard_[0];
    fwd_us_ = st.avg_forward_time_us / U_;
    bwd_us_ = st.avg_backward_time_us / U_;
    fwd_flops_ = st.forward_flops / U_;
    bwd_flops_ = st.backward_flops / U_;
    reference_ = o.schedule == "reference";

    Device& dev = *ctx.dev;
    es_ = dtype_size(ctx.wire);
    const int rank = ctx.rank();
    std::vector<int> unit_members, rep_members;
    for (int r = 0; r < W; ++r) {
      if (r / F_ == rank / F_) unit_members.push_back(r);
      if (r % F_ == rank % F_) rep_members.push_back(r);
    }
    const size_t unit_bytes = max_shard_ * F_ * es_;
    const bool split = o.comm_lanes == "split";
    auto own_comm = [&](std::unique_ptr<Communicator> c) {
      comms_.push_back(std::move(c));
      return comms_.back().get();
    };
    auto own_stream = [&](std::unique_ptr<Stream> s) {
      lanes_.push_back(std::move(s));
      return lanes_.back().get();
    };
    ag_comm_ = own_comm(ctx.comms->create("fsdp/unit/" + std::to_string(rank / F_), unit_members, unit_bytes, false, ctx.lane_ctas));
    rs_comm_ = split ? own_comm(ctx.comms->create("fsdp/unit_rs/" + std::to_string(rank / F_), unit_members,
                                                  unit_bytes, false, ctx.lane_ctas))
                     : ag_comm_;
    if (R_ > 1)
      ar_comm_ = own_comm(
          ctx.comms->create("fsdp/replica/" + std::to_string(rank % F_), rep_members, max_shard_ * es_, false, ctx.lane_ctas));

    compute_ = dev.create_stream(false);
    ag_stream_ = own_stream(dev.create_stream(true));
    rs_stream_ = split ? own_stream(dev.create_stream(true)) : ag_stream_;
    if (R_ > 1) ar_stream_ = split ? own_stream(dev.create_stream(true)) : ag_stream_;

    for (int u = 0; u < U_; ++u) {
      params_.push_back(dev.alloc(shard_[u] * es_));
      grads_.push_back(dev.alloc(shard_[u] * es_));
      dev.fill_random(params_.back().data(), shard_[u], ctx.wire, 2000 + u, *compute_);
    }
    const bool ag_peer = ag_comm_->wants_peer_buffers(), rs_peer = rs_comm_->wants_peer_buffers();
    for (int b = 0; b < 2; ++b) {
      gathered_[b] = ag_peer ? dev.alloc_peer(unit_bytes) : dev.alloc(unit_bytes);
      full_grad_[b] = rs_peer ? dev.alloc_peer(unit_bytes) : dev.alloc(unit_bytes);
      dev.fill_random(full_grad_[b].data(), max_shard_ * F_, ctx.wire, 3000 + b, *compute_);
      if (ag_peer) ag_comm_->register_buffer(gathered_[b].data(), unit_bytes);
      if (rs_peer) rs_comm_->register_buffer(full_grad_[b].data(), unit_bytes);
    }
    auto mk = [&](std::vector<std::unique_ptr<Event>>& v) {
      for (int u = 0; u < U_; ++u) v.push_back(dev.create_event());
    };
    mk(ag_f_);
    mk(fwd_done_);
    mk(ag_b_);
    mk(bwd_done_);
    mk(rs_done_);
    mk(ar_done_);
    ComputeEngine& ce = *ctx.compute;
    gated_ = !reference_ && env_int("DLNB_DEVICE_GATES", 1) != 0 && ce.gates_task(fwd_us_) && ce.gates_task(bwd_us_);
    if (gated_) {
      for (int u = 0; u < U_; ++u) {
        g_ag_f_.push_back(ce.make_gate());
        g_ag_b_.push_back(ce.make_gate());
        g_rs_.push_back(ce.make_gate());
      }
    }
    if (o.optimizer) {
      DLNB_REQUIRE(ctx.wire == DType::BF16, "--optimizer needs --wire-dtype bf16");
      for (int u = 0; u < U_; ++u) mom_.push_back(dev.alloc(shard_[u] * es_));
    }
    compute_->synchronize();
    timers_.reset(new TimerSet(dev));
    for (const char* k : {"allgather", "allgather_wait_fwd", "allgather_wait_bwd", "reduce_scatter", "barrier",
                          "allgather_time", "allreduce_time"})
      timers_->ensure(k);
    stats_.push_back({"allgather", CollKind::AllGather, F_, static_cast<double>(unit_bytes), "allgather_time"});
    stats_.push_back({"reduce_scatter", CollKind::ReduceScatter, F_, static_cast<double>(unit_bytes), "reduce_scatter"});
    if (R_ > 1)
      stats_.push_back({"allreduce", CollKind::AllReduce, R_, static_cast<double>(max_shard_ * es_), "allreduce_time"});
  }

  void compute_after(Event* dep, const char* timer, double us, double flops) {
    ComputeEngine& ce = *ctx_->compute;
    if (ce.stamps_task_start()) {
      if (dep) compute_->wait(*dep);
      uint64_t* st = timers_->slot();
      ce.run_stamped(*compute_, us, flops, st);
      if (timer && prev_.slot) timers_->gap(prev_.slot, prev_.ticks, st, timer);
      prev_ = task_mark(ce, *compute_, st, us);
      return;
    }
    if (dep) {
      if (timer)
        timers_->stall_before_task(*compute_, *dep, timer);
      else
        compute_->wait(*dep);
    }
    ce.run(*compute_, us, flops);
  }
  void compute_after(Event& dep, const char* timer, double us, double flops) { compute_after(&dep, timer, us, flops); }

  void compute_gated(std::vector<int> gates, const char* timer, double us, double flops, Event* done) {
    ComputeEngine& ce = *ctx_->compute;
    uint64_t* st = timers_->slot();
    ce.run_gated(*compute_, us, flops, gates, st, prev_.slot != nullptr, done);
    if (timer && prev_.slot) timers_->gap(prev_.slot, prev_.ticks, st, timer);
    prev_ = task_mark(ce, *compute_, st, us);
  }

  void enqueue_iteration() override {
    Context& ctx = *ctx_;
    const DType t = ctx.wire;
    prev_ = TaskMark();
    tail_end_ = nullptr;

    ComputeEngine& ce = *ctx.compute;
    const bool lane = gated_ && ctx.dev->gate_events();
    const bool prog = lane && ce.begin_program(*compute_);
    auto gather = [&](int u, Event& done, bool first, int gate) {
      int tk = timers_->begin(*ag_stream_);
      ag_comm_->all_gather(params_[u].data(), gathered_[u & 1].data(), shard_[u], t, *ag_stream_);
      timers_->end(tk, *ag_stream_, first ? "allgather" : "allgather_time");
      if (gated_) ce.signal(*ag_stream_, gate);
      if (!lane) ag_stream_->record(done);
    };

    gather(0, *ag_f_[0], true, gated_ ? g_ag_f_[0] : -1);
    if (reference_) ag_stream_->synchronize();
    for (int u = 0; u < U_; ++u) {
      if (u + 1 < U_) {
        if (u >= 1) ag_stream_->wait(*fwd_done_[u - 1]);
        gather(u + 1, *ag_f_[u + 1], false, gated_ ? g_ag_f_[u + 1] : -1);
      }
      if (gated_) {
        if (!lane) compute_->wait(*ag_f_[u]);
        compute_gated({g_ag_f_[u]}, u == 0 ? nullptr : "allgather_wait_fwd", fwd_us_, fwd_flops_,
                      fwd_done_[u].get());
      } else {
        compute_after(*ag_f_[u], u == 0 ? nullptr : "allgather_wait_fwd", fwd_us_, fwd_flops_);
        compute_->record(*fwd_done_[u]);
      }
    }

    for (int u = U_ - 1; u >= 0; --u) {
      if (u - 1 >= 0) {
        ag_stream_->wait(u + 1 <= U_ - 1 ? *bwd_done_[u + 1] : *fwd_done_[u - 1]);
        gather(u - 1, *ag_b_[u - 1], false, gated_ ? g_ag_b_[u - 1] : -1);
      }
      if (gated_) {
        std::vector<int> gates;
        if (u < U_ - 1) {
          if (!lane) compute_->wait(*ag_b_[u]);
          gates.push_back(g_ag_b_[u]);
        }
        if (u + 2 <= U_ - 1) {
          if (!lane) compute_->wait(*rs_done_[u + 2]);
          gates.push_back(g_rs_[u + 2]);
        }
        compute_gated(gates, u < U_ - 1 ? "allgather_wait_bwd" : nullptr, bwd_us_, bwd_flops_, bwd_done_[u].get());
      } else {
        if (u + 2 <= U_ - 1) compute_->wait(*rs_done_[u + 2]);
        if (u < U_ - 1)
          compute_after(*ag_b_[u], "allgather_wait_bwd", bwd_us_, bwd_flops_);
        else
          compute_after(nullptr, nullptr, bwd_us_, bwd_flops_);
        compute_->record(*bwd_done_[u]);
      }

      rs_stream_->wait(*bwd_done_[u]);
      int tk = timers_->begin(*rs_stream_);
      rs_comm_->reduce_scatter(full_grad_[u & 1].data(), grads_[u].data(), shard_[u], t, *rs_stream_);
      tail_end_ = timers_->end(tk, *rs_stream_, "reduce_scatter");
      if (gated_ && u >= 2) ce.signal(*rs_stream_, g_rs_[u]);
      if (!lane || R_ > 1 || u == 0) rs_stream_->record(*rs_done_[u]);
      if (reference_) compute_->wait(*rs_done_[u]);
      if (R_ > 1) {
        ar_stream_->wait(*rs_done_[u]);
        int ta = timers_->begin(*ar_stream_);
        ar_comm_->all_reduce(grads_[u].data(), grads_[u].data(), shard_[u], t, *ar_stream_);
        tail_end_ = timers_->end(ta, *ar_stream_, "allreduce_time");
        ar_stream_->record(*ar_done_[u]);
      }
    }
    const bool tail_gap = gated_ && !ctx.opt.optimizer && tail_end_ && prev_.slot;
    if (prog) ce.end_program(*compute_, tail_gap);
    Event& tail = R_ > 1 ? *ar_done_[0] : *rs_done_[0];
    if (tail_gap) {
      timers_->gap(prev_.slot, prev_.ticks, tail_end_, "barrier");
    } else {
      timers_->stall_after_task(*compute_, tail, "barrier");
    }
    if (ctx.opt.optimizer) {
      if (R_ > 1)
        for (int u = 1; u < U_; ++u) compute_->wait(*ar_done_[u]);
      for (int u = 0; u < U_; ++u)
        optimizer_step(ctx, *compute_, params_[u].data(), mom_[u].data(), grads_[u].data(), shard_[u]);
    }
  }

  std::vector<Stream*> streams() override {
    std::vector<Stream*> ss = {compute_.get()};
    for (auto& s : lanes_) ss.push_back(s.get());
    return ss;
  }
  bool capturable() const override { return !reference_; }

  void synchronize() override {
    std::vector<Stream*> ss = {compute_.get()};
    std::vector<Communicator*> cs;
    for (auto& s : lanes_) ss.push_back(s.get());
    for (auto& c : comms_) cs.push_back(c.get());
    sync_streams(ss, cs, *ctx_->dev);
    timers_->resolve();
  }

  std::vector<OutputView> outputs() const override {
    std::vector<OutputView> v;
    auto name = [](const char* stem, int i) {
      char b[48];
      std::snprintf(b, sizeof b, "%s_%03d", stem, i);
      return std::string(b);
    };
    for (int u = 0; u < U_; ++u) v.push_back({name("grad_shard", u), grads_[u].data(), shard_[u], ctx_->wire});
    for (int b = 0; b < 2 && b < U_; ++b)
      v.push_back({name("gathered_params", b), gathered_[b].data(), shard_[b] * F_, ctx_->wire});
    if (ctx_->opt.optimizer)
      for (int u = 0; u < U_; ++u) v.push_back({name("param_shard", u), params_[u].data(), shard_[u], ctx_->wire});
    return v;
  }

  std::string tail_collective_timer() const override { return R_ > 1 ? "allreduce_time" : "reduce_scatter"; }
  std::string section_id() const override { return "fsdp"; }
  std::string section_title() const override { return "FSDP metrics"; }
  const char* runtime_key() const override { return "runtime"; }

  Json global_json() const override {
    const Context& ctx = *ctx_;
    Json g = Json::object();
    g["model_size_bytes"] = P_ * es_;
    g["model_name"] = ctx.opt.model;
    g["world_size"] = ctx.world();
    g["num_units"] = U_;
    g["sharding_factor"] = F_;
    g["num_replicas"] = R_;
    g["local_batch_size"] = ctx.stats.batch_size;
    g["device"] = ctx.dev->kind() == DeviceKind::CPU ? "CPU" : "GPU";
    g["backend"] = ag_comm_->backend_name();
    g["comm_lanes"] = ctx.opt.comm_lanes;
    g["device_gates"] = gated_;
    g["fwd_time_per_unit_us"] = fwd_us_;
    g["bwd_time_per_unit_us"] = bwd_us_;
    g["allgather_msg_size_bytes"] = max_shard_ * F_ * es_;
    g["reducescatter_msg_size_bytes"] = max_shard_ * es_;
    if (R_ > 1) g["allreduce_msg_size_bytes"] = max_shard_ * es_;
    return g;
  }

  Json rank_json() const override {
    Json r = Json::object();
    for (const char* k : {"runtime", "allgather", "allgather_wait_fwd", "allgather_wait_bwd", "reduce_scatter",
                          "barrier", "allgather_time", "allreduce_time"})
      r[k] = timers_->values_json(k);
    r["rank"] = ctx_->rank();
    return r;
  }

  Json comm_summary() const override { return comm_stats_json(stats_, *timers_); }

 private:
  Context* ctx_ = nullptr;
  int U_ = 1, F_ = 1, R_ = 1;
  uint64_t P_ = 0, max_shard_ = 0;
  size_t es_ = 2;
  bool reference_ = false;
  bool gated_ = false;
  std::vector<int> g_ag_f_, g_ag_b_, g_rs_;
  std::vector<uint64_t> shard_;
  double fwd_us_ = 0, bwd_us_ = 0, fwd_flops_ = 0, bwd_flops_ = 0;
  std::vector<std::unique_ptr<Communicator>> comms_;
  std::vector<std::unique_ptr<Stream>> lanes_;
  Communicator *ag_comm_ = nullptr, *rs_comm_ = nullptr, *ar_comm_ = nullptr;
  std::unique_ptr<Stream> compute_;
  Stream *ag_stream_ = nullptr, *rs_stream_ = nullptr, *ar_stream_ = nullptr;
  std::vector<Buffer> params_, grads_, mom_;
  Buffer gathered_[2], full_grad_[2];
  std::vector<std::unique_ptr<Event>> ag_f_, fwd_done_, ag_b_, bwd_done_, rs_done_, ar_done_;
  std::vector<CommStat> stats_;
  TaskMark prev_;
  const uint64_t* tail_end_ = nullptr;
};

}

std::unique_ptr<Strategy> make_fsdp() { return std::unique_ptr<Strategy>(new Fsdp()); }

}
```

### csrc/src/timeline.cpp

```cpp
#include "dlnb/timeline.hpp"

#include <algorithm>
#include <cstdio>
#include <fstream>
#include <limits>

#include "dlnb/common.hpp"

namespace dlnb {

Timeline::Timeline(Device& dev, size_t cap, size_t max_events) : dev_(dev), cap_(cap), max_events_(max_events) {
  stamps_ = dev_.alloc_stamps(cap_);
}

Timeline::~Timeline() {
  if (stamps_) dev_.free_stamps(stamps_, cap_);
}

int Timeline::lane_of(Stream& s) {
  auto it = lanes_.find(&s);
  if (it != lanes_.end()) return it->second;
  const int id = static_cast<int>(lane_names_.size());
  lanes_[&s] = id;
  lane_names_.push_back("stream " + std::to_string(id));
// ... 224 lines not shown
      x["pid"] = pid;
      x["tid"] = static_cast<int>(e.at(1).as_int());
      x["cat"] = e.at(2).as_string();
      x["name"] = e.at(3).as_string();
      x["ts"] = base_us(r) + e.at(4).as_double() - t0;
      x["dur"] = e.at(5).as_double();
      Json args = e.at(6);
      args["iter"] = e.at(0).as_int();
      x["args"] = args;
      out.push_back(x);
    }
  }
  Json doc = Json::object();
  doc["traceEvents"] = out;
  doc["displayTimeUnit"] = "ms";
  Json other = meta;
  Json cal = Json::object();
  for (const auto& r : ranks) cal[std::to_string(r.at("rank").as_int())] = r.at("calibration_error_us");
  other["calibration_error_us"] = cal;
  other["time_origin_host_ns"] = o0 + static_cast<long long>(t0 * 1e3);
  doc["otherData"] = other;
  std::ofstream f(path);
  DLNB_REQUIRE(f.good(), "cannot write the timeline to " << path);
  f << doc.dump() << "\n";
}

namespace {

Json op_args(size_t count, DType t, int n) {
  Json a = Json::object();
  a["count"] = static_cast<double>(count);
  a["bytes"] = static_cast<double>(count * dtype_size(t));
  a["dtype"] = dtype_name(t);
  a["ranks"] = n;
  return a;
}

class TracingCommunicator : public Communicator {
 public:
  TracingCommunicator(std::unique_ptr<Communicator> in, Timeline* tl) : in_(std::move(in)), tl_(tl) {
    rank_ = in_->rank();
    size_ = in_->size();
    members_ = in_->members();
    name_ = in_->name();
  }
  std::string backend_name() const override { return in_->backend_name(); }

  void all_reduce(const void* send, void* recv, size_t count, DType t, Stream& s) override {
    traced(s, "all_reduce", count, t, [&] { in_->all_reduce(send, recv, count, t, s); });
  }
  void all_gather(const void* send, void* recv, size_t count, DType t, Stream& s) override {
    traced(s, "all_gather", count * static_cast<size_t>(size_), t, [&] { in_->all_gather(send, recv, count, t, s); });
  }
  void reduce_scatter(const void* send, void* recv, size_t count, DType t, Stream& s) override {
    traced(s, "reduce_scatter", count * static_cast<size_t>(size_), t,
           [&] { in_->reduce_scatter(send, recv, count, t, s); });
  }
  void all_to_all(const void* send, void* recv, size_t count, DType t, Stream& s) override {
    traced(s, "all_to_all", count * static_cast<size_t>(size_), t, [&] { in_->all_to_all(send, recv, count, t, s); });
  }
  void send(const void* buf, size_t count, DType t, int peer, Stream& s) override {
    p2p(s, "send", count, t, peer);
    in_->send(buf, count, t, peer, s);
    if (depth_ == 0) p2p_close();
  }
  void recv(void* buf, size_t count, DType t, int peer, Stream& s) override {
    p2p(s, "recv", count, t, peer);
    in_->recv(buf, count, t, peer, s);
    if (depth_ == 0) p2p_close();
  }
  void group_start() override {
    ++depth_;
    in_->group_start();
  }
  void group_end() override {
    in_->group_end();
    if (--depth_ == 0) p2p_close();
  }
  bool wants_peer_buffers() const override { return in_->wants_peer_buffers(); }
  void register_buffer(void* p, size_t bytes) override { in_->register_buffer(p, bytes); }
  std::string async_error() override { return in_->async_error(); }
  void abort() override { in_->abort(); }
  int library_nranks() override { return in_->library_nranks(); }

 private:
  template <class F>
  void traced(Stream& s, const char* op, size_t count, DType t, F&& fn) {
    tl_->label(s, "comm: " + name_);
    const int tok = tl_->begin(s);
    fn();
    tl_->end(tok, s, "comm", std::string(op) + " " + name_, op_args(count, t, size_));
  }
  void p2p(Stream& s, const char* op, size_t count, DType t, int peer) {
    if (!open_) {
      tl_->label(s, "comm: " + name_);
      open_ = true;
      stream_ = &s;
      tok_ = tl_->begin(s);
      ops_.clear();
      bytes_ = 0;
    }
    if (!ops_.empty()) ops_ += ",";
    ops_ += std::string(op) + "(" + std::to_string(peer) + ")";
    bytes_ += static_cast<double>(count * dtype_size(t));
  }
  void p2p_close() {
    if (!open_) return;
    open_ = false;
    Json a = Json::object();
    a["bytes"] = bytes_;
    a["ops"] = ops_;
    tl_->end(tok_, *stream_, "p2p", "p2p " + name_, a);
  }
  std::unique_ptr<Communicator> in_;
  Timeline* tl_;
  int depth_ = 0, tok_ = -1;
  bool open_ = false;
  Stream* stream_ = nullptr;
  std::string ops_;
  double bytes_ = 0;
};

class TracingFactory : public CommFactory {
 public:
  TracingFactory(std::unique_ptr<CommFactory> in, Timeline* tl) : in_(std::move(in)), tl_(tl) {}
  std::string backend_name() const override { return in_->backend_name(); }
  std::unique_ptr<Communicator> create(const std::string& name, const std::vector<int>& members,
                                       size_t capacity_bytes, bool need_p2p, int max_ctas) override {
    return std::make_unique<TracingCommunicator>(in_->create(name, members, capacity_bytes, need_p2p, max_ctas), tl_);
  }

 private:
  std::unique_ptr<CommFactory> in_;
  Timeline* tl_;
};

class TracingCompute : public ComputeEngine {
 public:
  TracingCompute(std::unique_ptr<ComputeEngine> in, Timeline* tl) : in_(std::move(in)), tl_(tl) {}
  void run(Stream& s, double us, double flops) override {
    traced(s, "compute", us, [&] { in_->run(s, us, flops); });
  }
  void run_stamped(Stream& s, double us, double flops, uint64_t* start) override {
    traced(s, "compute", us, [&] { in_->run_stamped(s, us, flops, start); });
  }
  bool stamps_task_start() const override { return in_->stamps_task_start(); }
  void run_chained(Stream& s, double us, double flops, uint64_t* start, Event* done) override {
    traced(s, "compute (chained)", us, [&] { in_->run_chained(s, us, flops, start, done); });
  }
  uint64_t task_ticks(double us) const override { return in_->task_ticks(us); }
  bool gates_task(double us) const override { return in_->gates_task(us); }
  int make_gate() override { return in_->make_gate(); }
  void signal(Stream& s, int gate) override { in_->signal(s, gate); }
  void wait_gate(Stream& s, int gate, double timeout_us) override { in_->wait_gate(s, gate, timeout_us); }
  void run_gated(Stream& s, double us, double flops, const std::vector<int>& gates, uint64_t* start,
                 bool chain, Event* done) override {
    Json a = Json::object();
    a["gates"] = static_cast<int>(gates.size());
    traced(s, chain ? "compute (chained)" : "compute", us,
           [&] { in_->run_gated(s, us, flops, gates, start, chain, done); }, a);
  }
  void set_next_start_slot(uint64_t* slot) override { in_->set_next_start_slot(slot); }
  void reset_clocks(Stream& s) override { in_->reset_clocks(s); }
  void reset_slot(Stream& s) override { in_->reset_slot(s); }
  bool begin_program(Stream& s) override { return in_->begin_program(s); }
  void end_program(Stream& s, bool join_ok) override { in_->end_program(s, join_ok); }
  long programs_on(Stream& s) override { return in_->programs_on(s); }
  bool program_split(Stream& s) override { return in_->program_split(s); }
  const uint64_t* last_task_end(Stream& s) override { return in_->last_task_end(s); }
  void after_capture() override { in_->after_capture(); }
  void set_lane_join(Stream& s, const std::vector<uint64_t*>& gates, uint32_t tag, uint64_t* host_done) override {
    in_->set_lane_join(s, gates, tag, host_done);
  }
  bool program_joined(Stream& s) override { return in_->program_joined(s); }
  void set_gate_timeout(double s) override { in_->set_gate_timeout(s); }
  double lane_task_us(Stream& s) override { return in_->lane_task_us(s); }
  void reset_capped(Stream& s) override { in_->reset_capped(s); }
  bool chain_counters(ChainCounters& c) override { return in_->chain_counters(c); }
  void set_task_timers(TimerSet* t) override { in_->set_task_timers(t); }
  bool product(const void** c, size_t* count, DType* t) const override { return in_->product(c, count, t); }
  Json describe() const override { return in_->describe(); }
  ComputeMode mode() const override { return in_->mode(); }

 private:
  template <class F>
  void traced(Stream& s, const char* name, double us, F&& fn, Json a = Json::object()) {
    tl_->label(s, "compute");
    int tok;
    if (in_->stamps_task_start()) {
      uint64_t* first = nullptr;
      tok = tl_->begin_external(&first);
      in_->set_next_start_slot(first);
    } else {
      tok = tl_->begin(s);
    }
    fn();
    a["table_us"] = us;
    if (!in_->stamps_task_start())
      tl_->end(tok, s, "compute", name, a);
    else if (const uint64_t* e = in_->last_task_end(s))
      tl_->end_at(tok, s, e, "compute", name, a);
    else
      tl_->end_after(tok, s, in_->task_ticks(us), "compute", name, a);
  }
  std::unique_ptr<ComputeEngine> in_;
  Timeline* tl_;
};

}

std::unique_ptr<CommFactory> make_tracing_factory(std::unique_ptr<CommFactory> inner, Timeline* tl) {
  return std::make_unique<TracingFactory>(std::move(inner), tl);
}

std::unique_ptr<ComputeEngine> make_tracing_compute(std::unique_ptr<ComputeEngine> inner, Timeline* tl) {
  return std::make_unique<TracingCompute>(std::move(inner), tl);
}

}
```

### csrc/src/timers.cpp

```cpp
#include "dlnb/timers.hpp"

#include <algorithm>
#include "dlnb/common.hpp"

namespace dlnb {

TimerSet::TimerSet(Device& dev) : dev_(dev) {
  cap_ = 1 << 16;
  stamps_ = dev_.alloc_stamps(cap_);
}

TimerSet::~TimerSet() {
  if (stamps_) dev_.free_stamps(stamps_, cap_);
}

int TimerSet::begin(Stream& s) {
  if (!enabled_) return -1;
  DLNB_REQUIRE(next_ < cap_, "too many timer stamps in one iteration");
  int idx = static_cast<int>(next_++);
  dev_.stamp(s, stamps_ + idx);
  if (task_stamps()) {
    auto it = clocks_.find(&s);
    if (it != clocks_.end() && !it->second.pending.empty()) close_pending(it->second, stamps_ + idx);
  }
  return idx;
}

const uint64_t* TimerSet::end(int token, Stream& s, const std::string& name) {
  if (!enabled_ || token < 0) return nullptr;
  DLNB_REQUIRE(next_ < cap_, "too many timer stamps in one iteration");
  int idx = static_cast<int>(next_++);
  dev_.stamp(s, stamps_ + idx);
  pending_.push_back(Pending{token, idx, name});
  if (task_stamps()) {
    auto it = clocks_.find(&s);
    if (it != clocks_.end()) restart(it->second, stamps_ + idx, 0);
  }
  return stamps_ + idx;
}

void TimerSet::stall(Stream& s, Event& e, const std::string& name) {
  static const bool timed = env_int("DLNB_STALL_TIMERS", 1) != 0;
  if (!timed) {
    s.wait(e);
    return;
  }
  DLNB_REQUIRE(!capturing_ || !task_stamps_, "TimerSet::stall(" << name << ") inside a graph capture");
  int t = begin(s);
  s.wait(e);
  end(t, s, name);
}

uint64_t* TimerSet::task_slot(Stream& s) {
  (void)s;
  if (!task_stamps()) return nullptr;
  return slot();
}

void TimerSet::task_started(Stream& s, const uint64_t* start, uint64_t ticks, const uint64_t* end) {
  if (!task_stamps() || !owns(start)) return;
  TaskClock& c = clocks_[&s];
  close_pending(c, start);
  if (end && owns(end))
    restart(c, end, 0);
  else
    restart(c, start, ticks);
}

const uint64_t* TimerSet::mark(Stream& s) {
  if (!enabled_) return nullptr;
  uint64_t* st = slot();
  dev_.stamp(s, st);
  return st;
}

void TimerSet::pair(const uint64_t* a, const uint64_t* b, const std::string& name) {
  if (!enabled_ || !owns(a) || !owns(b)) return;
  pending_.push_back(Pending{static_cast<int>(a - stamps_), static_cast<int>(b - stamps_), name});
}

void TimerSet::stall_before_task(Stream& s, Event& e, const std::string& name) {
  if (!task_stamps()) {
    stall(s, e, name);
    return;
  }
  TaskClock& c = clocks_[&s];
  if (!c.start) {
    first_reference(s, c);
  }
  s.wait(e);
  c.pending.push_back(name);
}

void TimerSet::stall_after_task(Stream& s, Event& e, const std::string& name) {
  if (!task_stamps()) {
    stall(s, e, name);
    return;
  }
  TaskClock& c = clocks_[&s];
  if (!c.start) first_reference(s, c);
  s.wait(e);
  DLNB_REQUIRE(next_ < cap_, "too many timer stamps in one iteration");
  uint64_t* st = stamps_ + next_++;
  dev_.stamp(s, st);
  c.pending.push_back(name);
  close_pending(c, st);
  restart(c, st, 0);
}

void TimerSet::stall_until(Stream& s, const uint64_t* end, const std::string& name) {
  if (!enabled_) return;
  DLNB_REQUIRE(task_stamps() && owns(end), "TimerSet::stall_until(" << name << ") needs task stamps");
  TaskClock& c = clocks_[&s];
  DLNB_REQUIRE(c.start, "TimerSet::stall_until(" << name << "): no task before it on the stream");
  c.pending.push_back(name);
  close_pending(c, end, true);
}

void TimerSet::iteration_start(Stream& s) {
  if (!task_stamps()) return;
  origin_ = &s;
  origin_start_ = mark(s);
}

void TimerSet::first_reference(Stream& s, TaskClock& c) {
  if (&s == origin_ && origin_start_)
    restart(c, origin_start_, 0);
  else
    restart(c, mark(s), 0);
}

void TimerSet::settle(Stream& s, const uint64_t* op_end) {
  if (!task_stamps() || !owns(op_end)) return;
  auto it = clocks_.find(&s);
  if (it == clocks_.end() || !it->second.start || it->second.pending.empty()) return;
  close_pending(it->second, op_end, true);
  it->second.floor = op_end;
}

void TimerSet::close_pending(TaskClock& c, const uint64_t* at, bool clamp) {
  for (size_t i = 0; i < c.pending.size(); ++i) {
    if (i == 0) {
      gap(c.start, c.ticks, at, c.pending[i], clamp);
      if (c.floor && enabled_ && c.start && at) gaps_.back().floor = static_cast<int>(c.floor - stamps_);
    } else
      gap(at, 0, at, c.pending[i]);
  }
  c.pending.clear();
}

void TimerSet::finish_stalls() {
  for (auto& kv : clocks_) {
    TaskClock& c = kv.second;
    if (c.pending.empty() || !enabled_) continue;
    uint64_t* st = slot();
    dev_.stamp(*kv.first, st);
    close_pending(c, st);
  }
  clocks_.clear();
  origin_ = nullptr;
  origin_start_ = nullptr;
}

uint64_t* TimerSet::slot() {
  DLNB_REQUIRE(next_ < cap_, "too many timer stamps in one iteration");
  return stamps_ + next_++;
}

void TimerSet::gap(const uint64_t* prev_start, uint64_t prev_ticks, const uint64_t* next_start,
                   const std::string& name, bool clamp) {
  if (!enabled_ || !prev_start || !next_start) return;
  gaps_.push_back(
      Gap{static_cast<int>(prev_start - stamps_), static_cast<int>(next_start - stamps_), prev_ticks, name, clamp, -1});
}

void TimerSet::add(const std::string& name, double seconds) {
  if (capturing_) {
    captured_adds_.emplace_back(name, seconds);
    return;
  }
  if (enabled_) vals_[name].push_back(seconds);
}

void TimerSet::begin_capture() {
  clocks_.clear();
// ... 81 lines not shown
```

### dlnetbench_amd/_native.py

```python
from __future__ import annotations

import ctypes
import json
import os
from typing import List, Optional

_LIB: Optional[ctypes.CDLL] = None
LIB_PATH = os.path.join(os.path.dirname(os.path.abspath(__file__)), "_lib", "libdlnb.so")

DTYPES = {"bf16": 0, "fp16": 1, "fp32": 2, "fp8": 3, "fp8_e4m3": 3, "fp8_e5m2": 4}


class NativeError(RuntimeError):
    pass


class TaskDesc(ctypes.Structure):
    _fields_ = [("ticks", ctypes.c_ulonglong), ("chain_ticks", ctypes.c_ulonglong),
                ("gate0", ctypes.c_void_p), ("gate1", ctypes.c_void_p),
                ("tag0", ctypes.c_uint), ("tag1", ctypes.c_uint),
                ("tstart0", ctypes.c_void_p), ("tstart1", ctypes.c_void_p),
                ("done_gate", ctypes.c_void_p), ("done_tag", ctypes.c_uint),
                ("work_rounds", ctypes.c_uint), ("tail_kt", ctypes.c_uint), ("epoch", ctypes.c_uint),
                ("tend", ctypes.c_void_p), ("flags", ctypes.c_uint)]


def lib() -> ctypes.CDLL:
    global _LIB
    if _LIB is not None:
        return _LIB
    if os.environ.get("DLNB_NO_TORCH", "0") != "1":
        try:
            import torch
        except ImportError:
            pass
    if not os.path.exists(LIB_PATH):
        raise NativeError(f"{LIB_PATH} is missing: build it with `make` (or __graft_entry__.build())")
    L = ctypes.CDLL(LIB_PATH, mode=ctypes.RTLD_LOCAL)
    c_int, c_size, c_vp, c_dbl, c_float = ctypes.c_int, ctypes.c_size_t, ctypes.c_void_p, ctypes.c_double, ctypes.c_float
    L.dlnb_version.restype = ctypes.c_char_p
    L.dlnb_last_error.restype = ctypes.c_char_p
    L.dlnb_free.argtypes = [c_vp]
    L.dlnb_gpu_count.restype = c_int
    L.dlnb_run.argtypes = [ctypes.c_char_p, c_int, ctypes.POINTER(ctypes.c_char_p), ctypes.POINTER(c_vp)]
    L.dlnb_run.restype = c_int
    L.dlnb_parse_stats.argtypes = [ctypes.c_char_p, ctypes.POINTER(c_vp)]
    L.dlnb_parse_stats.restype = c_int
    L.dlnb_fill_random.argtypes = [c_vp, c_size, c_int, ctypes.c_ulonglong, c_vp]
    L.dlnb_gemm_tn.argtypes = [c_vp, c_vp, c_vp, c_int, c_int, c_int, c_int, c_int, c_int, c_int, c_vp]
    L.dlnb_gemm_tn_waves.argtypes = [c_vp, c_vp, c_vp, c_int, c_int, c_int, c_int, c_int, c_int, c_int, c_int, c_vp]
    L.dlnb_gemm_deadline_us.argtypes = [c_vp, c_vp, c_vp, c_int, c_int, c_int, c_int, c_dbl, c_int, c_vp, c_int, c_vp]
    L.dlnb_gemm_deadline_ex.argtypes = [c_vp, c_vp, c_vp, c_int, c_int, c_int, c_int, c_dbl, c_int, c_vp, c_int, c_vp,
                                        ctypes.c_uint, c_dbl, c_vp, ctypes.c_uint, c_vp, ctypes.c_uint, c_vp, c_vp]
    L.dlnb_gate_signal.argtypes = [c_vp, ctypes.c_uint, c_vp]
    L.dlnb_gate_signal_iter.argtypes = [c_vp, c_vp, ctypes.c_uint, c_vp]
    L.dlnb_task_size.restype = c_int
    L.dlnb_gemm_program.argtypes = [c_vp, c_vp, c_vp, c_int, c_int, c_int, c_int, ctypes.POINTER(TaskDesc), c_int,
                                    c_vp, c_vp, c_vp, c_dbl, c_int, c_vp, c_vp, c_int, c_vp, ctypes.c_uint]
    L.dlnb_program_ktiles.argtypes = [c_int, c_int, c_int, c_int]
    L.dlnb_host_words.argtypes = [c_int, ctypes.POINTER(c_vp)]
    L.dlnb_host_words.restype = c_vp
    L.dlnb_host_words_free.argtypes = [c_vp]
    L.dlnb_gemm_shape_ok.argtypes = [c_int, c_int, c_int, c_int]
    L.dlnb_gemm_narrow_nf.argtypes = [c_int, c_int, c_int]
    L.dlnb_idle_wait_us.argtypes = [c_dbl, c_int, c_vp]
    L.dlnb_busy_spin_us.argtypes = [c_dbl, c_int, c_vp]
    L.dlnb_sgd_momentum_bf16.argtypes = [c_vp, c_vp, c_vp, c_size, c_float, c_float, c_vp]
    L.dlnb_stamp.argtypes = [c_vp, c_vp]
    L.dlnb_wallclock_hz.argtypes = [c_int]
    L.dlnb_wallclock_hz.restype = c_dbl
    L.dlnb_bf16_to_float.argtypes = [ctypes.c_ushort]
    L.dlnb_bf16_to_float.restype = c_float
    L.dlnb_float_to_bf16.argtypes = [c_float]
    L.dlnb_float_to_bf16.restype = ctypes.c_ushort
    L.dlnb_fp8e4m3_to_float.argtypes = [ctypes.c_ubyte]
    L.dlnb_fp8e4m3_to_float.restype = c_float
    L.dlnb_float_to_fp8e4m3.argtypes = [c_float]
    L.dlnb_float_to_fp8e4m3.restype = ctypes.c_ubyte
    _LIB = L
    return L


def check(rc: int) -> None:
    if rc != 0:
        raise NativeError(lib().dlnb_last_error().decode())


def _take_string(ptr: ctypes.c_void_p) -> str:
    s = ctypes.cast(ptr, ctypes.c_char_p).value.decode()
    lib().dlnb_free(ptr)
    return s


def version() -> str:
    return lib().dlnb_version().decode()


def run_raw(strategy: str, args: List[str]) -> dict:
    L = lib()
    argv = (ctypes.c_char_p * len(args))(*[a.encode() for a in args])
    out = ctypes.c_void_p()
    check(L.dlnb_run(strategy.encode(), len(args), argv, ctypes.byref(out)))
    return json.loads(_take_string(out)) if out.value else {}


def parse_stats(path: str) -> dict:
    out = ctypes.c_void_p()
    check(lib().dlnb_parse_stats(path.encode(), ctypes.byref(out)))
    return json.loads(_take_string(out))
```

### dlnetbench_amd/ops/gemm.py

```python
from __future__ import annotations

from .. import _native


def _stream(t):
    import torch
    return torch.cuda.current_stream(t.device).cuda_stream


def gemm_tn(a, b, out=None, waves: int = 0):
    import torch
    if a.dtype != b.dtype:
        raise TypeError("a and b must have the same dtype")
    if a.dtype == torch.bfloat16:
        dt = _native.DTYPES["bf16"]
    elif a.dtype == getattr(torch, "float8_e4m3fn", None):
        dt = _native.DTYPES["fp8_e4m3"]
    else:
        raise TypeError(f"unsupported dtype {a.dtype}")
    M, K = a.shape
    N, K2 = b.shape
    if K != K2:
        raise ValueError("K mismatch")
    if a.stride(1) != 1 or b.stride(1) != 1:
        raise ValueError("a and b must be K-contiguous (row-major)")
    L = _native.lib()
    if not L.dlnb_gemm_shape_ok(M, N, K, dt):
        raise ValueError(f"unsupported shape M={M} N={N} K={K} (M,N % 256, K bytes % 128)")
    if out is None:
        out = torch.empty((M, N), device=a.device, dtype=torch.bfloat16)
    if out.stride(1) != 1:
        raise ValueError("out must be row-major")
    lda, ldb, ldc = a.stride(0), b.stride(0), out.stride(0)
    _native.check(L.dlnb_gemm_tn_waves(a.data_ptr(), b.data_ptr(), out.data_ptr(), M, N, K, lda, ldb, ldc, dt, waves,
                                       _stream(a)))
    return out


def gemm_deadline_us(a, b, c, us: float, stamp=None, grid: int = 0):
    import torch
    dt = _native.DTYPES["bf16"] if a.dtype == torch.bfloat16 else _native.DTYPES["fp8_e4m3"]
    M, K = a.shape
    N = b.shape[0]
    if stamp is None:
        stamp = torch.zeros(8, dtype=torch.int64, device=a.device)
    if stamp.numel() < 8 or stamp.dtype != torch.int64:
        raise ValueError("stamp must be an int64 tensor of >= 8 elements")
    _native.check(_native.lib().dlnb_gemm_deadline_us(a.data_ptr(), b.data_ptr(), c.data_ptr(), M, N, K, dt, us,
                                                      a.device.index or 0, stamp.data_ptr(), grid, _stream(a)))
    return c


def gemm_deadline_ex(a, b, c, us: float, slot, epoch: int, chain=False, gates=(), tstart=None,
                     grid: int = 0, counters=None):
    import torch
    dt = _native.DTYPES["bf16"] if a.dtype == torch.bfloat16 else _native.DTYPES["fp8_e4m3"]
    M, K = a.shape
    N = b.shape[0]
    if slot.numel() < 8 or slot.dtype != torch.int64:
        raise ValueError("slot must be an int64 tensor of >= 8 elements")
    g = [(t.data_ptr() + 16 * i, tag) for t, i, tag in gates] + [(None, 0)] * (2 - len(gates))
    ts = tstart[0].data_ptr() + 8 * tstart[1] if tstart is not None else None
    if counters is not None and (counters.numel() < 8 or counters.dtype != torch.int64):
        raise ValueError("counters must be an int64 tensor of >= 8 elements")
    cp = counters.data_ptr() if counters is not None else None
    _native.check(_native.lib().dlnb_gemm_deadline_ex(a.data_ptr(), b.data_ptr(), c.data_ptr(), M, N, K, dt, us,
                                                      a.device.index or 0, slot.data_ptr(), grid, _stream(a), epoch,
                                                      30.0 if chain is True else float(chain or 0), g[0][0],
                                                      g[0][1], g[1][0], g[1][1], ts, cp))
    return c


def gate_signal_(gate, index: int, tag: int):
    import torch
    if gate.numel() < 2 * index + 2 or gate.dtype != torch.int64:
        raise ValueError("gate must be an int64 tensor with two words per gate")
    _native.check(_native.lib().dlnb_gate_signal(gate.data_ptr() + 16 * index, tag, _stream(gate)))
    return gate


def fill_random_(t, seed: int = 0):
    import torch
    m = {torch.bfloat16: "bf16", torch.float16: "fp16", torch.float32: "fp32"}
    f8 = getattr(torch, "float8_e4m3fn", None)
    if f8 is not None:
        m[f8] = "fp8_e4m3"
    f85 = getattr(torch, "float8_e5m2", None)
    if f85 is not None:
        m[f85] = "fp8_e5m2"
    dt = _native.DTYPES[m[t.dtype]]
    _native.check(_native.lib().dlnb_fill_random(t.data_ptr(), t.numel(), dt, seed, _stream(t)))
    return t


def sgd_momentum_(param, mom, grad, lr: float = 1e-4, beta: float = 0.9):
    _native.check(_native.lib().dlnb_sgd_momentum_bf16(param.data_ptr(), mom.data_ptr(), grad.data_ptr(),
                                                       param.numel(), lr, beta, _stream(param)))
    return param


def idle_wait_us(us: float, device: int = 0):
    import torch
    _native.check(_native.lib().dlnb_idle_wait_us(us, device, torch.cuda.current_stream(device).cuda_stream))


def busy_spin_us(us: float, device: int = 0):
    import torch
    _native.check(_native.lib().dlnb_busy_spin_us(us, device, torch.cuda.current_stream(device).cuda_stream))


def stamp_(slot, index: int = 0):
    _native.check(_native.lib().dlnb_stamp(slot.data_ptr() + 8 * index, _stream(slot)))
    return slot


def gate_signal_iter_(gate, index: int, tag: int, iter_word):
    _native.check(_native.lib().dlnb_gate_signal_iter(gate.data_ptr() + 16 * index, iter_word.data_ptr(), tag,
                                                      _stream(gate)))
    return gate


def task_size() -> int:
    return int(_native.lib().dlnb_task_size())


def program_ktiles(M: int, N: int, K: int, dtype) -> int:
    import torch
    dt = _native.DTYPES["bf16"] if dtype == torch.bfloat16 else _native.DTYPES["fp8_e4m3"]
    return int(_native.lib().dlnb_program_ktiles(M, N, K, dt))


def ptr(t, index: int = 0, words: int = 1) -> int:
    if isinstance(t, HostWords):
        return t.dev + 8 * index
    return t.data_ptr() + 8 * index


class HostWords:

    def __init__(self, n: int):
        import ctypes
        dev = ctypes.c_void_p()
        self.host = _native.lib().dlnb_host_words(n, ctypes.byref(dev))
        if not self.host:
            raise _native.NativeError("hipHostMalloc failed")
        self.dev = dev.value
        self.n = n
        self._arr = (ctypes.c_uint64 * n).from_address(self.host)

    def __getitem__(self, i: int) -> int:
        return int(self._arr[i])

    def __setitem__(self, i: int, v: int) -> None:
        self._arr[i] = v

    def free(self) -> None:
        if self.host:
            _native.lib().dlnb_host_words_free(self.host)
            self.host = None


def gemm_program(a, b, c, tasks, slot, task_buf, iter_word=None, counters=None, abort=None,
                 gate_timeout_s: float = 60.0, grid: int = 0, epoch: int = 0):
    import torch
    dt = _native.DTYPES["bf16"] if a.dtype == torch.bfloat16 else _native.DTYPES["fp8_e4m3"]
    M, K = a.shape
    N = b.shape[0]
    if slot.numel() < 8 or slot.dtype != torch.int64:
        raise ValueError("slot must be an int64 tensor of >= 8 elements")
    if task_buf.numel() * task_buf.element_size() < len(tasks) * task_size():
        raise ValueError("task_buf too small")
    arr = (_native.TaskDesc * len(tasks))(*tasks)
    _native.check(_native.lib().dlnb_gemm_program(
        a.data_ptr(), b.data_ptr(), c.data_ptr(), M, N, K, dt, arr, len(tasks),
        iter_word.data_ptr() if iter_word is not None else None,
        counters.data_ptr() if counters is not None else None,
        abort.dev if abort is not None else None, gate_timeout_s, a.device.index or 0, slot.data_ptr(),
        task_buf.data_ptr(), grid, _stream(a), epoch))
    return c
```

Measured before the change: 2815.

## Fuse timer stamps and gate signal into single-rank collective copy kernel

For one-rank RCCL communicators, collectives and self send/recv are replaced with a custom nontemporal vectorized copy kernel instead of calling RCCL. The kernel also writes the begin/end timer stamps and raises the gate signal from its last finishing block, so the separate stamp and gate-signal kernel launches around each collective go away. This is meant to cut launch overhead and RCCL's self-collective cost in the 1-GPU case. It adds a per-stream completion counter and new hook plumbing through the timers, compute engine and strategies.

```diff
diff --git a/csrc/include/dlnb/comm.hpp b/csrc/include/dlnb/comm.hpp
--- a/csrc/include/dlnb/comm.hpp
+++ b/csrc/include/dlnb/comm.hpp
@@ -11,6 +11,14 @@
 namespace dlnb {
 
 enum class CollKind : int { AllReduce, AllGather, ReduceScatter, AllToAll, SendRecv };
+
+struct CollHooks {
+  uint64_t* begin_slot = nullptr;
+  uint64_t* end_slot = nullptr;
+  uint64_t* gate = nullptr;
+  const uint64_t* iter = nullptr;
+  uint32_t tag = 0;
+};
 
 class Communicator {
  public:
@@ -29,6 +37,11 @@
   virtual void recv(void* buf, size_t count, DType t, int peer, Stream& s) = 0;
   virtual void group_start() {}
   virtual void group_end() {}
+  virtual bool collective_hooked(CollKind kind, const void* send, void* recv, size_t count, DType t, Stream& s,
+                                 const CollHooks& h) {
+    (void)kind, (void)send, (void)recv, (void)count, (void)t, (void)s, (void)h;
+    return false;
+  }
   virtual bool wants_peer_buffers() const { return false; }
   virtual void register_buffer(void* p, size_t bytes) { (void)p, (void)bytes; }
   virtual std::string async_error() { return ""; }
diff --git a/csrc/include/dlnb/compute.hpp b/csrc/include/dlnb/compute.hpp
--- a/csrc/include/dlnb/compute.hpp
+++ b/csrc/include/dlnb/compute.hpp
@@ -41,6 +41,10 @@
   virtual bool gates_task(double us) const { (void)us; return false; }
   virtual int make_gate() { DLNB_THROW("this compute mode has no device gates"); }
   virtual void signal(Stream& s, int gate) { (void)s; (void)gate; DLNB_THROW("this compute mode has no device gates"); }
+  virtual void arm_signal(int gate, uint64_t** words, uint32_t* tag) {
+    (void)gate; (void)words; (void)tag;
+    DLNB_THROW("this compute mode has no device gates");
+  }
   virtual void wait_gate(Stream& s, int gate, double timeout_us) {
     (void)s; (void)gate; (void)timeout_us;
     DLNB_THROW("this compute mode has no device gates");
diff --git a/csrc/include/dlnb/kernels.hpp b/csrc/include/dlnb/kernels.hpp
--- a/csrc/include/dlnb/kernels.hpp
+++ b/csrc/include/dlnb/kernels.hpp
@@ -47,6 +47,10 @@
 };
 void gate_signal(uint64_t* gate, const uint64_t* iter, uint32_t tag, void* stream);
 void fail_gate_signal(long index);
+void copy_stamped(void* dst, const void* src, size_t bytes, uint64_t* begin_slot, uint64_t* end_slot, uint64_t* gate,
+                  const uint64_t* iter, uint32_t tag, uint32_t* done, int blocks, void* stream);
+int copy_stamped_blocks_per_cu();
+int copy_stamped_grid(size_t bytes, int max_blocks);
 void gate_wait(const uint64_t* gate, const uint64_t* iter, uint32_t tag, uint64_t timeout_ticks, uint64_t* timeouts,
                void* stream, const uint64_t* abort = nullptr);
 void set_word(uint64_t* word, uint64_t value, void* stream);
diff --git a/csrc/include/dlnb/strategy.hpp b/csrc/include/dlnb/strategy.hpp
--- a/csrc/include/dlnb/strategy.hpp
+++ b/csrc/include/dlnb/strategy.hpp
@@ -127,6 +127,10 @@
 };
 Json comm_stats_json(const std::vector<CommStat>& stats, const TimerSet& t);
 
+const uint64_t* hooked_collective(Context& ctx, TimerSet& timers, Communicator& comm, CollKind kind, const void* send,
+                                  void* recv, size_t count, DType t, Stream& s, const std::string& timer,
+                                  uint64_t* gate = nullptr, uint32_t tag = 0);
+
 void dump_outputs(Context& ctx, const Strategy& strat, const std::string& dir);
 
 void print_topology(Context& ctx);
diff --git a/csrc/include/dlnb/timers.hpp b/csrc/include/dlnb/timers.hpp
--- a/csrc/include/dlnb/timers.hpp
+++ b/csrc/include/dlnb/timers.hpp
@@ -19,6 +19,9 @@
   int begin(Stream& s);
   const uint64_t* at(int token) const { return token < 0 ? nullptr : stamps_ + token; }
   const uint64_t* end(int token, Stream& s, const std::string& name);
+  int begin_slot(Stream& s, uint64_t** slot);
+  const uint64_t* end_slot(int token, Stream& s, const std::string& name, uint64_t** slot);
+  void stamp(Stream& s, uint64_t* slot);
   void stall(Stream& s, Event& e, const std::string& name);
   uint64_t* slot();
   void gap(const uint64_t* prev_start, uint64_t prev_ticks, const uint64_t* next_start, const std::string& name,
diff --git a/csrc/kernels/kernels.hip b/csrc/kernels/kernels.hip
--- a/csrc/kernels/kernels.hip
+++ b/csrc/kernels/kernels.hip
@@ -28,6 +28,7 @@
 typedef __attribute__((ext_vector_type(4))) __bf16 bf16x4;
 typedef __attribute__((ext_vector_type(4))) float f32x4;
 typedef __attribute__((ext_vector_type(8))) int i32x8;
+typedef __attribute__((ext_vector_type(4))) uint32_t u32x4;
 typedef __attribute__((address_space(3))) void* lds_ptr_t;
 typedef __attribute__((address_space(1))) void* gbl_ptr_t;
 
@@ -120,6 +121,68 @@
     const uint64_t seq = dl::gate_seq(iter, tag);
     __hip_atomic_store(gate + 1, __builtin_amdgcn_s_memrealtime(), __ATOMIC_RELAXED, __HIP_MEMORY_SCOPE_AGENT);
     __hip_atomic_store(gate, seq, __ATOMIC_RELEASE, __HIP_MEMORY_SCOPE_AGENT);
+  }
+}
+
+
+constexpr int kCopyThreads = 1024;
+constexpr int kCopyUnroll = 8;
+
+template <typename V>
+__device__ __forceinline__ void copy_units(V* __restrict__ dst, const V* __restrict__ src, size_t n) {
+  constexpr size_t tile = static_cast<size_t>(kCopyThreads) * kCopyUnroll;
+  const size_t step = static_cast<size_t>(gridDim.x) * tile;
+  size_t base = static_cast<size_t>(blockIdx.x) * tile;
+  for (; base + tile <= n; base += step) {
+    const size_t i = base + threadIdx.x;
+    V v[kCopyUnroll];
+#pragma unroll
+    for (int j = 0; j < kCopyUnroll; ++j) v[j] = __builtin_nontemporal_load(src + i + j * kCopyThreads);
+#pragma unroll
+    for (int j = 0; j < kCopyUnroll; ++j) __builtin_nontemporal_store(v[j], dst + i + j * kCopyThreads);
+  }
+  for (size_t i = base + threadIdx.x; i < n; i += kCopyThreads)
+    __builtin_nontemporal_store(__builtin_nontemporal_load(src + i), dst + i);
+}
+
+template <typename V>
+__device__ __forceinline__ void copy_bytes(char* dst, const char* src, size_t bytes) {
+  size_t head = (sizeof(V) - reinterpret_cast<uintptr_t>(dst) % sizeof(V)) % sizeof(V);
+  if (head > bytes) head = bytes;
+  const size_t n = (bytes - head) / sizeof(V);
+  const size_t tail = head + n * sizeof(V);
+  if (blockIdx.x == 0 && threadIdx.x < 16) {
+    if (threadIdx.x < head) dst[threadIdx.x] = src[threadIdx.x];
+    if (tail + threadIdx.x < bytes) dst[tail + threadIdx.x] = src[tail + threadIdx.x];
+  }
+  copy_units(reinterpret_cast<V*>(dst + head), reinterpret_cast<const V*>(src + head), n);
+}
+
+__global__ void __launch_bounds__(kCopyThreads)
+    copy_stamped_kernel(char* dst, const char* src, size_t bytes, int vec_log2, uint64_t* begin_slot,
+                        uint64_t* end_slot, uint64_t* gate, const uint64_t* iter, uint32_t tag, uint32_t* done) {
+  if (begin_slot && blockIdx.x == 0 && threadIdx.x == 0)
+    __hip_atomic_store(begin_slot, __builtin_amdgcn_s_memrealtime(), __ATOMIC_RELAXED, __HIP_MEMORY_SCOPE_SYSTEM);
+  switch (vec_log2) {
+    case 4: copy_bytes<u32x4>(dst, src, bytes); break;
+    case 3: copy_bytes<uint64_t>(dst, src, bytes); break;
+    case 2: copy_bytes<uint32_t>(dst, src, bytes); break;
+    case 1: copy_bytes<uint16_t>(dst, src, bytes); break;
+    default: copy_bytes<uint8_t>(dst, src, bytes); break;
+  }
+  asm volatile("s_waitcnt vmcnt(0)" ::: "memory");
+  __syncthreads();
+  if (threadIdx.x == 0) {
+    if (__hip_atomic_fetch_add(done, 1u, __ATOMIC_RELEASE, __HIP_MEMORY_SCOPE_AGENT) == gridDim.x - 1) {
+      const uint64_t t = __builtin_amdgcn_s_memrealtime();
+      __hip_atomic_store(done, 0u, __ATOMIC_RELAXED, __HIP_MEMORY_SCOPE_AGENT);
+      if (end_slot) __hip_atomic_store(end_slot, t, __ATOMIC_RELAXED, __HIP_MEMORY_SCOPE_SYSTEM);
+      if (gate) {
+        const uint64_t seq = dl::gate_seq(iter, tag);
+        __hip_atomic_store(gate + 1, t, __ATOMIC_RELAXED, __HIP_MEMORY_SCOPE_AGENT);
+        __hip_atomic_store(gate, seq, __ATOMIC_RELEASE, __HIP_MEMORY_SCOPE_AGENT);
+      }
+    }
   }
 }
 
@@ -518,6 +581,43 @@
     return;
   }
   hipLaunchKernelGGL(gate_signal_kernel, 1, 64, 0, S(stream), gate, iter, tag);
+  DLNB_HIP_CHECK(hipGetLastError());
+}
+
+int copy_stamped_blocks_per_cu() {
+  static const int per_cu = [] {
+    int n = 0;
+    DLNB_HIP_CHECK(hipOccupancyMaxActiveBlocksPerMultiprocessor(&n, copy_stamped_kernel, kCopyThreads, 0));
+    return std::max(1, n);
+  }();
+  return per_cu;
+}
+
+int copy_stamped_grid(size_t bytes, int max_blocks) {
+  const size_t per_block = static_cast<size_t>(kCopyThreads) * kCopyUnroll * 16;
+  const size_t want = std::max<size_t>(1, (bytes + per_block - 1) / per_block);
+  return static_cast<int>(std::min<size_t>(static_cast<size_t>(std::max(1, max_blocks)), want));
+}
+
+void copy_stamped(void* dst, const void* src, size_t bytes, uint64_t* begin_slot, uint64_t* end_slot, uint64_t* gate,
+                  const uint64_t* iter, uint32_t tag, uint32_t* done, int blocks, void* stream) {
+  DLNB_REQUIRE(done != nullptr && blocks > 0 && (bytes == 0 || (dst != nullptr && src != nullptr)),
+               "copy_stamped: bad arguments");
+  if (gate) {
+    DLNB_REQUIRE(tag > 0 && reinterpret_cast<uintptr_t>(gate) % 16 == 0, "copy_stamped: bad gate/tag");
+    const long k = g_gate_signals.fetch_add(1);
+    const long f = g_gate_fault.load();
+    if (f >= 0 && k == f) {
+      std::fprintf(stderr, "[dlnb] fault injection: gate signal %ld of this process is not raised\n", k);
+      std::fflush(stderr);
+      gate = nullptr;
+    }
+  }
+  const uintptr_t rel = reinterpret_cast<uintptr_t>(dst) ^ reinterpret_cast<uintptr_t>(src);
+  int vec_log2 = 4;
+  while (vec_log2 > 0 && (rel & ((uintptr_t(1) << vec_log2) - 1)) != 0) --vec_log2;
+  hipLaunchKernelGGL(copy_stamped_kernel, blocks, kCopyThreads, 0, S(stream), static_cast<char*>(dst),
+                     static_cast<const char*>(src), bytes, vec_log2, begin_slot, end_slot, gate, iter, tag, done);
   DLNB_HIP_CHECK(hipGetLastError());
 }
 
diff --git a/csrc/src/capi.cpp b/csrc/src/capi.cpp
--- a/csrc/src/capi.cpp
+++ b/csrc/src/capi.cpp
@@ -118,6 +118,15 @@
 int dlnb_gate_signal_iter(void* gate, const void* iter, unsigned tag, void* stream) {
   return guard([&] {
     dlnb::kernels::gate_signal(static_cast<uint64_t*>(gate), static_cast<const uint64_t*>(iter), tag, stream);
+  });
+}
+
+int dlnb_copy_stamped(void* dst, const void* src, size_t bytes, void* begin, void* end, void* gate, const void* iter,
+                      unsigned tag, void* done, int blocks, void* stream) {
+  return guard([&] {
+    dlnb::kernels::copy_stamped(dst, src, bytes, static_cast<uint64_t*>(begin), static_cast<uint64_t*>(end),
+                                static_cast<uint64_t*>(gate), static_cast<const uint64_t*>(iter), tag,
+                                static_cast<uint32_t*>(done), blocks, stream);
   });
 }
 
diff --git a/csrc/src/comm_rccl.cpp b/csrc/src/comm_rccl.cpp
--- a/csrc/src/comm_rccl.cpp
+++ b/csrc/src/comm_rccl.cpp
@@ -4,10 +4,13 @@
 #include <dlfcn.h>
 
 #include <cstring>
+#include <deque>
+#include <map>
 #include <sstream>
 
 #include "dlnb/comm.hpp"
 #include "dlnb/json.hpp"
+#include "dlnb/kernels.hpp"
 
 #define DLNB_NCCL_CHECK(expr)                                                            \
   do {                                                                                   \
@@ -35,7 +38,7 @@
 class RcclComm : public Communicator {
  public:
   RcclComm(const std::string& name, const std::vector<int>& members, int my_world_rank, HostGroup& world,
-           int max_ctas) {
+           int max_ctas, int device) {
     name_ = name;
     members_ = members;
     size_ = static_cast<int>(members.size());
@@ -60,28 +63,69 @@
     if (max_ctas > 0) cfg.maxCTAs = max_ctas;
     cfg.commName = name_.c_str();
     DLNB_NCCL_CHECK(ncclCommInitRankConfig(&comm_, size_, id, rank_, &cfg));
+    if (size_ == 1) {
+      (void)max_ctas;
+      copy_blocks_ = kernels::num_cus(device);
+      if (hipMalloc(reinterpret_cast<void**>(&done_), kDoneWords * kDoneStride * sizeof(uint32_t)) != hipSuccess ||
+          hipMemset(done_, 0, kDoneWords * kDoneStride * sizeof(uint32_t)) != hipSuccess ||
+          hipStreamSynchronize(nullptr) != hipSuccess)
+        DLNB_THROW("RCCL communicator " << name << ": no memory for the copy kernel's counters");
+    }
   }
   ~RcclComm() override {
     if (comm_) (void)ncclCommDestroy(comm_);
+    if (done_) (void)hipFree(done_);
   }
   std::string backend_name() const override { return "RCCL"; }
 
   void all_reduce(const void* send, void* recv, size_t count, DType t, Stream& s) override {
+    if (size_ == 1) return local_copy(send, recv, count * dtype_size(t), s, CollHooks(), false);
     DLNB_NCCL_CHECK(ncclAllReduce(send, recv, count, to_nccl(t), ncclSum, comm_, hs(s)));
   }
   void all_gather(const void* send, void* recv, size_t send_count, DType t, Stream& s) override {
+    if (size_ == 1) return local_copy(send, recv, send_count * dtype_size(t), s, CollHooks(), false);
     DLNB_NCCL_CHECK(ncclAllGather(send, recv, send_count, to_nccl(t), comm_, hs(s)));
   }
   void reduce_scatter(const void* send, void* recv, size_t recv_count, DType t, Stream& s) override {
+    if (size_ == 1) return local_copy(send, recv, recv_count * dtype_size(t), s, CollHooks(), false);
     DLNB_NCCL_CHECK(ncclReduceScatter(send, recv, recv_count, to_nccl(t), ncclSum, comm_, hs(s)));
   }
   void all_to_all(const void* send, void* recv, size_t count, DType t, Stream& s) override {
+    if (size_ == 1) return local_copy(send, recv, count * dtype_size(t), s, CollHooks(), false);
     DLNB_NCCL_CHECK(ncclAllToAll(send, recv, count, to_nccl(t), comm_, hs(s)));
   }
+  bool collective_hooked(CollKind kind, const void* send, void* recv, size_t count, DType t, Stream& s,
+                         const CollHooks& h) override {
+    if (size_ != 1 || kind == CollKind::SendRecv) return false;
+    local_copy(send, recv, count * dtype_size(t), s, h, true);
+    return true;
+  }
   void send(const void* buf, size_t count, DType t, int peer, Stream& s) override {
+    if (size_ == 1) {
+      DLNB_REQUIRE(peer == 0, "send to rank " << peer << " of the one-rank group " << name_);
+      if (recvs_.empty()) {
+        sends_.push_back({const_cast<void*>(buf), count * dtype_size(t)});
+        return;
+      }
+      const Self r = recvs_.front();
+      recvs_.pop_front();
+      DLNB_REQUIRE(r.bytes == count * dtype_size(t), "send/recv to self: sizes differ in group " << name_);
+      return local_copy(buf, r.buf, r.bytes, s, CollHooks(), false);
+    }
     DLNB_NCCL_CHECK(ncclSend(buf, count, to_nccl(t), peer, comm_, hs(s)));
   }
   void recv(void* buf, size_t count, DType t, int peer, Stream& s) override {
+    if (size_ == 1) {
+      DLNB_REQUIRE(peer == 0, "recv from rank " << peer << " of the one-rank group " << name_);
+      if (sends_.empty()) {
+        recvs_.push_back({buf, count * dtype_size(t)});
+        return;
+      }
+      const Self m = sends_.front();
+      sends_.pop_front();
+      DLNB_REQUIRE(m.bytes == count * dtype_size(t), "send/recv to self: sizes differ in group " << name_);
+      return local_copy(m.buf, buf, m.bytes, s, CollHooks(), false);
+    }
     DLNB_NCCL_CHECK(ncclRecv(buf, count, to_nccl(t), peer, comm_, hs(s)));
   }
   void group_start() override { DLNB_NCCL_CHECK(ncclGroupStart()); }
@@ -105,7 +149,32 @@
   }
 
  private:
+  void local_copy(const void* src, void* dst, size_t bytes, Stream& s, const CollHooks& h, bool stamps_only) {
+    if (src == dst || bytes == 0) {
+      if (!stamps_only) return;
+      bytes = 0;
+    }
+    kernels::copy_stamped(dst, src, bytes, h.begin_slot, h.end_slot, h.gate, h.iter, h.tag, done_word(hs(s)),
+                          kernels::copy_stamped_grid(bytes, copy_blocks_), hs(s));
+  }
+  uint32_t* done_word(hipStream_t s) {
+    auto it = done_of_.find(s);
+    if (it == done_of_.end()) {
+      DLNB_REQUIRE(done_of_.size() < kDoneWords, "communicator " << name_ << " is used on more than " << kDoneWords << " streams");
+      it = done_of_.emplace(s, done_ + done_of_.size() * kDoneStride).first;
+    }
+    return it->second;
+  }
+  static constexpr size_t kDoneWords = 64, kDoneStride = 16;
+  struct Self {
+    void* buf;
+    size_t bytes;
+  };
   ncclComm_t comm_ = nullptr;
+  int copy_blocks_ = 0;
+  uint32_t* done_ = nullptr;
+  std::map<hipStream_t, uint32_t*> done_of_;
+  std::deque<Self> sends_, recvs_;
 };
 
 class RcclFactory : public CommFactory {
@@ -117,7 +186,7 @@
   std::unique_ptr<Communicator> create(const std::string& name, const std::vector<int>& members, size_t,
                                        bool, int max_ctas) override {
     (void)hipSetDevice(dev_.index());
-    return std::unique_ptr<Communicator>(new RcclComm(name, members, world_.rank(), world_, max_ctas));
+    return std::unique_ptr<Communicator>(new RcclComm(name, members, world_.rank(), world_, max_ctas, dev_.index()));
   }
 
  private:
diff --git a/csrc/src/compute.cpp b/csrc/src/compute.cpp
--- a/csrc/src/compute.cpp
+++ b/csrc/src/compute.cpp
@@ -280,9 +280,16 @@
   }
 
   void signal(Stream& s, int gate) override {
+    uint64_t* words = nullptr;
+    uint32_t tag = 0;
+    arm_signal(gate, &words, &tag);
+    kernels::gate_signal(words, dev_.iter_word(), tag, s.native());
+  }
+  void arm_signal(int gate, uint64_t** words, uint32_t* tag_out) override {
     uint32_t& tag = gate_tag_.at(gate);
     tag = tag == 0xffffffffu ? 1u : tag + 1;
-    kernels::gate_signal(gates_.at(gate), dev_.iter_word(), tag, s.native());
+    *words = gates_.at(gate);
+    *tag_out = tag;
   }
   void wait_gate(Stream& s, int gate, double timeout_us) override {
     const uint32_t tag = gate_tag_.at(gate);
diff --git a/csrc/src/device_gpu.cpp b/csrc/src/device_gpu.cpp
--- a/csrc/src/device_gpu.cpp
+++ b/csrc/src/device_gpu.cpp
@@ -300,6 +300,8 @@
   void set_gate_timeout(double s) override { gate_timeout_s_ = s; }
   double gate_timeout_s_ = 0.0;
   void gate_mark(GpuEvent& e, hipStream_t s) {
+    DLNB_REQUIRE(e.tag == 0 || e.gen != gen_ || e.on == s,
+                 "a gate event is recorded on two streams within one capture (its raises could land out of tag order)");
     if (!e.gate) e.gate = alloc_gate();
     e.tag = e.tag == 0xffffffffu ? 1u : e.tag + 1;
     e.on = s;
diff --git a/csrc/src/runner.cpp b/csrc/src/runner.cpp
--- a/csrc/src/runner.cpp
+++ b/csrc/src/runner.cpp
@@ -121,6 +121,31 @@
       std::this_thread::sleep_for(std::chrono::microseconds(5));
     }
   }
+}
+
+const uint64_t* hooked_collective(Context& ctx, TimerSet& timers, Communicator& comm, CollKind kind, const void* send,
+                                  void* recv, size_t count, DType t, Stream& s, const std::string& timer,
+                                  uint64_t* gate, uint32_t tag) {
+  CollHooks h;
+  const int tk = timers.begin_slot(s, &h.begin_slot);
+  const uint64_t* end = timers.end_slot(tk, s, timer, &h.end_slot);
+  if (gate) {
+    h.gate = gate;
+    h.iter = ctx.dev->iter_word();
+    h.tag = tag;
+  }
+  if (comm.collective_hooked(kind, send, recv, count, t, s, h)) return end;
+  timers.stamp(s, h.begin_slot);
+  switch (kind) {
+    case CollKind::AllReduce: comm.all_reduce(send, recv, count, t, s); break;
+    case CollKind::AllGather: comm.all_gather(send, recv, count, t, s); break;
+    case CollKind::ReduceScatter: comm.reduce_scatter(send, recv, count, t, s); break;
+    case CollKind::AllToAll: comm.all_to_all(send, recv, count, t, s); break;
+    case CollKind::SendRecv: DLNB_THROW("hooked_collective: not a collective");
+  }
+  timers.stamp(s, h.end_slot);
+  if (gate) ctx.dev->signal_gate(s, gate, tag);
+  return end;
 }
 
 Json comm_stats_json(const std::vector<CommStat>& stats, const TimerSet& t) {
diff --git a/csrc/src/strategy_dp.cpp b/csrc/src/strategy_dp.cpp
--- a/csrc/src/strategy_dp.cpp
+++ b/csrc/src/strategy_dp.cpp
@@ -133,14 +133,12 @@
       comm_stream_->wait(*ready_[i]);
       const uint64_t n = shard_[i] * W_;
       if (zero_ == 2) {
-        int t = timers_->begin(*comm_stream_);
-        comm_->reduce_scatter(grads_[i].data(), sums_[i].data(), shard_[i], ctx.wire, *comm_stream_);
-        timers_->end(t, *comm_stream_, "reduce_scatter_time");
+        hooked_collective(ctx, *timers_, *comm_, CollKind::ReduceScatter, grads_[i].data(), sums_[i].data(), shard_[i],
+                          ctx.wire, *comm_stream_, "reduce_scatter_time");
       } else {
-        int t = timers_->begin(*comm_stream_);
         void* out = in_place_ ? grads_[i].data() : sums_[i].data();
-        comm_->all_reduce(grads_[i].data(), out, n, ctx.wire, *comm_stream_);
-        timers_->end(t, *comm_stream_, "allreduce_time");
+        hooked_collective(ctx, *timers_, *comm_, CollKind::AllReduce, grads_[i].data(), out, n, ctx.wire,
+                          *comm_stream_, "allreduce_time");
       }
     }
     if (prog) ce.end_program(*compute_, false);
@@ -159,9 +157,8 @@
       }
       compute_->record(*opt_done_[i]);
       comm_stream_->wait(*opt_done_[i]);
-      int t = timers_->begin(*comm_stream_);
-      comm_->all_gather(pshard_[i].data(), pfull_[i].data(), shard_[i], ctx.wire, *comm_stream_);
-      ag_end = timers_->end(t, *comm_stream_, "param_allgather_time");
+      ag_end = hooked_collective(ctx, *timers_, *comm_, CollKind::AllGather, pshard_[i].data(), pfull_[i].data(),
+                                 shard_[i], ctx.wire, *comm_stream_, "param_allgather_time");
     }
     const uint64_t* opt_mark = opt_end ? opt_end : timers_->mark(*compute_);
     comm_stream_->record(*ag_done_);
@@ -194,10 +191,9 @@
       } else {
         comm_stream_->wait(*ready_[i]);
       }
-      int t = timers_->begin(*comm_stream_);
       void* out = in_place_ ? grads_[i].data() : sums_[i].data();
-      comm_->all_reduce(grads_[i].data(), out, sizes_[i], ctx.wire, *comm_stream_);
-      const uint64_t* e = timers_->end(t, *comm_stream_, "allreduce_time");
+      const uint64_t* e = hooked_collective(ctx, *timers_, *comm_, CollKind::AllReduce, grads_[i].data(), out,
+                                            sizes_[i], ctx.wire, *comm_stream_, "allreduce_time");
       if (e) tail_end = e;
     }
     const bool tail_gap = last.slot && tail_end && !ctx.opt.optimizer;
diff --git a/csrc/src/strategy_fsdp.cpp b/csrc/src/strategy_fsdp.cpp
--- a/csrc/src/strategy_fsdp.cpp
+++ b/csrc/src/strategy_fsdp.cpp
@@ -146,10 +146,11 @@
     const bool lane = gated_ && ctx.dev->gate_events();
     const bool prog = lane && ce.begin_program(*compute_);
     auto gather = [&](int u, Event& done, bool first, int gate) {
-      int tk = timers_->begin(*ag_stream_);
-      ag_comm_->all_gather(params_[u].data(), gathered_[u & 1].data(), shard_[u], t, *ag_stream_);
-      timers_->end(tk, *ag_stream_, first ? "allgather" : "allgather_time");
-      if (gated_) ce.signal(*ag_stream_, gate);
+      uint64_t* words = nullptr;
+      uint32_t tag = 0;
+      if (gated_) ce.arm_signal(gate, &words, &tag);
+      hooked_collective(ctx, *timers_, *ag_comm_, CollKind::AllGather, params_[u].data(), gathered_[u & 1].data(),
+                        shard_[u], t, *ag_stream_, first ? "allgather" : "allgather_time", words, tag);
       if (!lane) ag_stream_->record(done);
     };
 
@@ -196,11 +197,16 @@
       }
 
       rs_stream_->wait(*bwd_done_[u]);
-      int tk = timers_->begin(*rs_stream_);
-      rs_comm_->reduce_scatter(full_grad_[u & 1].data(), grads_[u].data(), shard_[u], t, *rs_stream_);
-      tail_end_ = timers_->end(tk, *rs_stream_, "reduce_scatter");
-      if (gated_ && u >= 2) ce.signal(*rs_stream_, g_rs_[u]);
-      if (!lane || R_ > 1 || u == 0) rs_stream_->record(*rs_done_[u]);
+      uint64_t* words = nullptr;
+      uint32_t tag = 0;
+      bool record = !lane || R_ > 1 || u == 0;
+      if (gated_ && u >= 2)
+        ce.arm_signal(g_rs_[u], &words, &tag);
+      else if (record && ctx.dev->arm_gate_record(*rs_done_[u], *rs_stream_, &words, &tag))
+        record = false;
+      tail_end_ = hooked_collective(ctx, *timers_, *rs_comm_, CollKind::ReduceScatter, full_grad_[u & 1].data(),
+                                    grads_[u].data(), shard_[u], t, *rs_stream_, "reduce_scatter", words, tag);
+      if (record) rs_stream_->record(*rs_done_[u]);
       if (reference_) compute_->wait(*rs_done_[u]);
       if (R_ > 1) {
         ar_stream_->wait(*rs_done_[u]);
diff --git a/csrc/src/timeline.cpp b/csrc/src/timeline.cpp
--- a/csrc/src/timeline.cpp
+++ b/csrc/src/timeline.cpp
@@ -400,6 +400,7 @@
   bool gates_task(double us) const override { return in_->gates_task(us); }
   int make_gate() override { return in_->make_gate(); }
   void signal(Stream& s, int gate) override { in_->signal(s, gate); }
+  void arm_signal(int gate, uint64_t** words, uint32_t* tag) override { in_->arm_signal(gate, words, tag); }
   void wait_gate(Stream& s, int gate, double timeout_us) override { in_->wait_gate(s, gate, timeout_us); }
   void run_gated(Stream& s, double us, double flops, const std::vector<int>& gates, uint64_t* start,
                  bool chain, Event* done) override {
diff --git a/csrc/src/timers.cpp b/csrc/src/timers.cpp
--- a/csrc/src/timers.cpp
+++ b/csrc/src/timers.cpp
@@ -15,10 +15,29 @@
 }
 
 int TimerSet::begin(Stream& s) {
+  uint64_t* slot = nullptr;
+  const int idx = begin_slot(s, &slot);
+  if (slot) dev_.stamp(s, slot);
+  return idx;
+}
+
+const uint64_t* TimerSet::end(int token, Stream& s, const std::string& name) {
+  uint64_t* slot = nullptr;
+  const uint64_t* e = end_slot(token, s, name, &slot);
+  if (slot) dev_.stamp(s, slot);
+  return e;
+}
+
+void TimerSet::stamp(Stream& s, uint64_t* slot) {
+  if (slot) dev_.stamp(s, slot);
+}
+
+int TimerSet::begin_slot(Stream& s, uint64_t** slot) {
+  *slot = nullptr;
   if (!enabled_) return -1;
   DLNB_REQUIRE(next_ < cap_, "too many timer stamps in one iteration");
   int idx = static_cast<int>(next_++);
-  dev_.stamp(s, stamps_ + idx);
+  *slot = stamps_ + idx;
   if (task_stamps()) {
     auto it = clocks_.find(&s);
     if (it != clocks_.end() && !it->second.pending.empty()) close_pending(it->second, stamps_ + idx);
@@ -26,11 +45,12 @@
   return idx;
 }
 
-const uint64_t* TimerSet::end(int token, Stream& s, const std::string& name) {
+const uint64_t* TimerSet::end_slot(int token, Stream& s, const std::string& name, uint64_t** slot) {
+  *slot = nullptr;
   if (!enabled_ || token < 0) return nullptr;
   DLNB_REQUIRE(next_ < cap_, "too many timer stamps in one iteration");
   int idx = static_cast<int>(next_++);
-  dev_.stamp(s, stamps_ + idx);
+  *slot = stamps_ + idx;
   pending_.push_back(Pending{token, idx, name});
   if (task_stamps()) {
     auto it = clocks_.find(&s);
diff --git a/dlnetbench_amd/_native.py b/dlnetbench_amd/_native.py
--- a/dlnetbench_amd/_native.py
+++ b/dlnetbench_amd/_native.py
@@ -54,6 +54,7 @@
                                         ctypes.c_uint, c_dbl, c_vp, ctypes.c_uint, c_vp, ctypes.c_uint, c_vp, c_vp]
     L.dlnb_gate_signal.argtypes = [c_vp, ctypes.c_uint, c_vp]
     L.dlnb_gate_signal_iter.argtypes = [c_vp, c_vp, ctypes.c_uint, c_vp]
+    L.dlnb_copy_stamped.argtypes = [c_vp, c_vp, c_size, c_vp, c_vp, c_vp, c_vp, ctypes.c_uint, c_vp, c_int, c_vp]
     L.dlnb_task_size.restype = c_int
     L.dlnb_gemm_program.argtypes = [c_vp, c_vp, c_vp, c_int, c_int, c_int, c_int, ctypes.POINTER(TaskDesc), c_int,
                                     c_vp, c_vp, c_vp, c_dbl, c_int, c_vp, c_vp, c_int, c_vp, ctypes.c_uint]
diff --git a/dlnetbench_amd/ops/gemm.py b/dlnetbench_amd/ops/gemm.py
--- a/dlnetbench_amd/ops/gemm.py
+++ b/dlnetbench_amd/ops/gemm.py
@@ -120,6 +120,17 @@
     return gate
 
 
+def copy_stamped_(dst, src, nbytes: int, done, blocks: int, begin=None, end=None, gate=None, tag: int = 0,
+                  iter_word=None, dst_offset: int = 0, src_offset: int = 0):
+    def word(x, words):
+        return ptr(x[0], x[1] * words, words) if x is not None else None
+    _native.check(_native.lib().dlnb_copy_stamped(
+        dst.data_ptr() + dst_offset, src.data_ptr() + src_offset, nbytes, word(begin, 1), word(end, 1),
+        word(gate, 2), iter_word.data_ptr() if iter_word is not None else None, tag, done.data_ptr(), blocks,
+        _stream(dst)))
+    return dst
+
+
 def task_size() -> int:
     return int(_native.lib().dlnb_task_size())
 
```

After: 2815. No clear change (+0.0%).
